# fuxiAIlab/RL4RS

Hardware: AMD Instinct MI355X
Metric: env-steps/s (batch=4096, 9-slot slate) (higher is better)
Workload: dtype f32 (scorer matrix operands as fp16 hi+lo pairs, three f16 MFMAs per product, fp32 accumulate)

## Files before the change

### include/rl4rs_hip.h

```cpp
#ifndef RL4RS_HIP_H
#define RL4RS_HIP_H

#include <stdint.h>

#ifdef __cplusplus
extern "C" {
#endif

#define RL4RS_ABI_VERSION 1

enum {
    RL4RS_OK = 0,
    RL4RS_EINVAL = -1,
    RL4RS_EHIP = -2,
    RL4RS_ESTATE = -3,
    RL4RS_ENOMEM = -4
};

const char* rl4rs_last_error(void);
int rl4rs_abi_version(void);
int rl4rs_device_count(void);

int rl4rs_copy_d2d(void* dst_dev, const void* src_dev, int64_t n_bytes, void* stream);

// ... 182 lines not shown
int rl4rs_dien_head_prob(rl4rs_dien* net, int32_t R, const float* obs_dev, float* prob_dev, void* stream);

enum {
    RL4RS_DIEN_ALL_FEATURE = 0,
    RL4RS_DIEN_SCORES = 1,
    RL4RS_DIEN_QUERY = 2,
    RL4RS_DIEN_H1 = 3,
    RL4RS_DIEN_N_ACTIVE = 4,
    RL4RS_DIEN_ROW_REP = 5,
    RL4RS_DIEN_ROW_ACTIVE = 6,
    RL4RS_DIEN_H1_FRAG = 7,
    RL4RS_DIEN_LEAD = 8
};
int rl4rs_dien_buffer(rl4rs_dien* net, int which, void** dev_ptr, int64_t* n_bytes);

int rl4rs_dien_set_row_order(rl4rs_dien* net, const int32_t* order_dev, int32_t n_groups);

int rl4rs_dien_set_profiling(rl4rs_dien* net, int enable);
int rl4rs_dien_kernel_count(void);
const char* rl4rs_dien_kernel_name(int which);
int rl4rs_dien_kernel_label(rl4rs_dien* net, int which, char* buf, int32_t cap);
int rl4rs_dien_profile_read(rl4rs_dien* net, int which, double* ms_total, int64_t* launches);
int rl4rs_dien_profile_reset(rl4rs_dien* net);

typedef struct rl4rs_simnet rl4rs_simnet;
enum { RL4RS_SIMNET_DNN = 1, RL4RS_SIMNET_WIDEDEEP = 2, RL4RS_SIMNET_LSTM = 3,
       RL4RS_SIMNET_ADVERSARIAL = 4  };

typedef struct rl4rs_simnet_cfg {
    int32_t algo;
    int32_t maxlen;
    int32_t emb_size;
    int32_t hidden_units;
    int32_t dense_feature_num;
    int32_t category_feature_num;
    int32_t category_hash_size;
    int32_t seq_num;
    int32_t class_num;
    int32_t max_rows;
    int32_t max_slots;
} rl4rs_simnet_cfg;

typedef struct rl4rs_simnet_weights {
    const float* cat_emb;
    const float* seq_emb;
    const float* dense_w1; const float* dense_b1;
    const float* dense_w2; const float* dense_b2;
    const float* fc_w; const float* fc_b;
    const float* obs_w; const float* obs_b;
    const float* out_w; const float* out_b;
    const float* cat_gru_kernel; const float* cat_gru_recurrent; const float* cat_gru_bias;
    const float* seq_gru_kernel[4]; const float* seq_gru_recurrent[4]; const float* seq_gru_bias[4];
} rl4rs_simnet_weights;

int rl4rs_simnet_create(const rl4rs_simnet_cfg* cfg, const rl4rs_simnet_weights* w, void* stream,
                        rl4rs_simnet** out);
int rl4rs_simnet_destroy(rl4rs_simnet* net);
int rl4rs_simnet_obs_dim(rl4rs_simnet* net, int32_t* dim);
int rl4rs_simnet_encode(rl4rs_simnet* net, int32_t s, const int32_t* ids_dev, int32_t n, int32_t slot_base,
                        void* stream);
int rl4rs_simnet_forward(rl4rs_simnet* net, int32_t R, int32_t group, const float* dense_dev,
                         const int32_t* cat_dev, const int32_t* slot_dev, float* obs_dev, float* prob_dev,
                         void* stream);
int rl4rs_simnet_head_prob(rl4rs_simnet* net, int32_t R, const float* obs_dev, float* prob_dev, void* stream);

typedef struct rl4rs_stepper rl4rs_stepper;
int rl4rs_env_attach_scorer(rl4rs_env* env, rl4rs_dien* net, const int32_t* slots_dev, int32_t seq_num,
                            rl4rs_stepper** out);
int rl4rs_env_attach_simnet(rl4rs_env* env, rl4rs_simnet* net, const int32_t* slots_dev, int32_t seq_num,
                            rl4rs_stepper** out);
int rl4rs_stepper_destroy(rl4rs_stepper* s);
int rl4rs_env_step_discrete(rl4rs_stepper* s, const int32_t* actions_dev, float* obs_dev, double* reward_dev,
                            uint8_t* done_dev, uint32_t* mask_bits_dev, void* stream);
int rl4rs_stepper_set_act_tail(rl4rs_stepper* s, int32_t on);
int rl4rs_stepper_set_obs_fold(rl4rs_stepper* s, int32_t on);
int rl4rs_stepper_set_distinct_hint(rl4rs_stepper* s, int32_t n_distinct);
int rl4rs_stepper_set_partition_carry(rl4rs_stepper* s, int32_t on);
int rl4rs_stepper_set_step_overlap(rl4rs_stepper* s, int32_t on);
int rl4rs_stepper_lane_stats(const rl4rs_stepper* s, int64_t* lane0, int64_t* lane1, int64_t* joins);
int rl4rs_stepper_observe(rl4rs_stepper* s, float* obs_dev, int32_t* taken, void* stream);
int rl4rs_stepper_set_reset_lane(rl4rs_stepper* s, int32_t on);
int rl4rs_stepper_set_reward_lane(rl4rs_stepper* s, int32_t on);
int rl4rs_stepper_lane_stats_ex(const rl4rs_stepper* s, int64_t* reset_runs, int64_t* reward_runs);
int rl4rs_stepper_click_probs(rl4rs_stepper* s, float* out_dev, void* stream);
int rl4rs_stepper_reward_rows(const rl4rs_stepper* s);
int rl4rs_stepper_next_offline_action(rl4rs_stepper* s, const int32_t** ids_dev, int32_t* step);
int rl4rs_env_step_conti(rl4rs_stepper* s, const void* actions_dev, int is_f64, int32_t* chosen_dev, float* obs_dev,
                         double* reward_dev, uint8_t* done_dev, uint32_t* mask_bits_dev, void* stream);

enum {
    RL4RS_STEP_WANT_MASK_I64 = 1, RL4RS_STEP_WANT_MASK_BITS = 2, RL4RS_STEP_WANT_D3RL_OBS = 4, RL4RS_STEP_WANT_CLICK_P = 8,
    RL4RS_STEP_WANT_OFFLINE_ACTION = 16, RL4RS_STEP_WANT_ALL = 31
};
typedef struct rl4rs_step_record {
    int64_t status, reward, done, chosen, obs, obs_d3rl, mask_i64, mask_bits, click_p, offline_action;
    int64_t host_bytes, total_bytes;
    int32_t obs_dim, d3rl_cols;
} rl4rs_step_record;
int rl4rs_stepper_record_layout(rl4rs_stepper* s, uint32_t want, int32_t conti, rl4rs_step_record* out);
int rl4rs_env_step_record(rl4rs_stepper* s, const void* actions_dev, int32_t action_kind, uint32_t want, void* record_dev,
                          void* stream);
int rl4rs_env_step_record_host(rl4rs_stepper* s, const void* actions_dev, int32_t action_kind, uint32_t want, void* record_dev,
                               void* record_host, void* stream);
int rl4rs_env_observe_record_host(rl4rs_stepper* s, int32_t conti, uint32_t want, void* record_dev, void* record_host,
                                  void* stream);
int rl4rs_set_host_mirror(int32_t on);

typedef struct rl4rs_policy rl4rs_policy;

int rl4rs_policy_param_count(int32_t obs_dim, int32_t hidden, int32_t action_size);
int rl4rs_policy_create(int32_t obs_dim, int32_t hidden, int32_t action_size, int32_t max_rows,
                        const float* params_host, void* stream, rl4rs_policy** out);
int rl4rs_policy_destroy(rl4rs_policy* pol);
int rl4rs_policy_params(rl4rs_policy* pol, float** params_dev, int32_t* count);

int rl4rs_policy_act(rl4rs_policy* pol, int32_t N, const float* obs_dev, const uint32_t* mask_bits_dev,
                     uint32_t seed, uint32_t step, int32_t* actions_dev, float* logp_dev, float* value_dev,
                     float* entropy_dev, float* logits_dev, void* stream);
int rl4rs_policy_evaluate(rl4rs_policy* pol, int32_t N, const float* obs_dev, const uint32_t* mask_bits_dev,
                          const int32_t* actions_dev, float* logp_dev, float* value_dev, float* entropy_dev,
                          float* logits_dev, void* stream);

int rl4rs_policy_loss_grad(rl4rs_policy* pol, int32_t algo, int32_t N, const float* obs_dev,
                           const uint32_t* mask_bits_dev, const int32_t* actions_dev, const float* adv_dev,
                           const float* ret_dev, const float* old_logp_dev, const float* old_value_dev,
                           const float* old_logits_dev, float vf_coeff, float ent_coeff, float clip,
                           float vf_clip, float kl_coeff, float* grad_dev, float* stats_dev, void* stream);
int rl4rs_policy_adam_step(rl4rs_policy* pol, const float* grad_dev, float lr, float beta1, float beta2,
                           float eps, float grad_clip, void* stream);
int rl4rs_policy_ppo_epoch(rl4rs_policy* pol, int32_t N, int32_t minibatch, const float* obs_dev,
                           const uint32_t* mask_bits_dev, const int32_t* actions_dev, const float* adv_dev,
                           const float* ret_dev, const float* old_logp_dev, const float* old_value_dev,
                           const float* old_logits_dev, float vf_coeff, float ent_coeff, float clip, float vf_clip,
                           float kl_coeff, float lr, float beta1, float beta2, float eps, float grad_clip,
                           float* grad_dev, float* stats_dev, void* stream);
int rl4rs_policy_ppo_minibatch_grad(rl4rs_policy* pol, int32_t N, int32_t minibatch, int32_t mb_index,
                                    const float* obs_dev, const uint32_t* mask_bits_dev, const int32_t* actions_dev,
                                    const float* adv_dev, const float* ret_dev, const float* old_logp_dev,
                                    const float* old_value_dev, const float* old_logits_dev, float vf_coeff,
                                    float ent_coeff, float clip, float vf_clip, float kl_coeff, float* grad_dev,
                                    float* stats_dev, void* stream);
enum { RL4RS_POLICY_STATUS_PASS_TIMEOUT = 1 };
int rl4rs_policy_status(rl4rs_policy* pol, int32_t* flags, void* stream);
int rl4rs_policy_status_words(rl4rs_policy* pol, uint32_t** words_dev);
enum { RL4RS_POLICY_OPT_TILE = 0, RL4RS_POLICY_OPT_PPO_FUSED = 1, RL4RS_POLICY_OPT_PPO_ROWS = 2, RL4RS_POLICY_OPT_RESIDENT_WGS = 3,
       RL4RS_POLICY_OPT_PPO_STD = 4 };
int rl4rs_policy_set_option(rl4rs_policy* pol, int32_t which, int32_t value);
int rl4rs_policy_adam_state(rl4rs_policy* pol, float** m_dev, float** v_dev, int64_t* step);
int rl4rs_policy_set_adam_step(rl4rs_policy* pol, int64_t step);

typedef struct rl4rs_replay rl4rs_replay;

int rl4rs_replay_create(int32_t obs_dim, int32_t action_size, int32_t max_steps, int32_t batch_size, int64_t buffer_size,
                        double alpha, rl4rs_replay** out);
int rl4rs_replay_destroy(rl4rs_replay* h);
int rl4rs_replay_rows(rl4rs_replay* h, int32_t* rows, int32_t* capacity_rows, int64_t* pushes);
enum { RL4RS_REPLAY_BUF_OBS = 0, RL4RS_REPLAY_BUF_MASK = 1, RL4RS_REPLAY_BUF_ACTION = 2, RL4RS_REPLAY_BUF_REWARD = 3,
       RL4RS_REPLAY_BUF_DONE = 4, RL4RS_REPLAY_BUF_PRIORITY = 5, RL4RS_REPLAY_BUF_MAX_PRIORITY = 6,
       RL4RS_REPLAY_BUF_ACTION_F32 = 7  };
int rl4rs_replay_buffer(rl4rs_replay* h, int32_t which, void** dev_out, int64_t* count_out);
int rl4rs_replay_push(rl4rs_replay* h, const float* obs_dev, const uint32_t* mask_bits_dev, const int32_t* action_dev,
                      const double* reward_dev, void* stream);
int rl4rs_replay_sample(rl4rs_replay* h, int32_t M, int32_t prioritized, double beta, uint32_t seed, uint32_t step,
                        float* obs_out, float* next_obs_out, uint32_t* next_mask_out, int32_t* action_out, float* reward_out,
                        int32_t* done_out, int32_t* idx_out, float* weight_out, float* u_out, void* stream);
int rl4rs_replay_update_priorities(rl4rs_replay* h, int32_t M, const int32_t* idx_dev, const float* td_dev, void* stream);
// ... 508 lines not shown
```

### rl4rs_amd/_lib.py

```python
import ctypes as C
import os

_HERE = os.path.dirname(os.path.abspath(__file__))
LIB_PATH = os.path.join(_HERE, 'csrc', 'librl4rs_hip.so')

OK = 0


class Rl4rsHipError(RuntimeError):
    pass


class EnvCfg(C.Structure):
    _fields_ = [(n, C.c_int32) for n in (
        'batch_size', 'max_steps', 'action_size', 'action_emb_size', 'page_items', 'item_dim',
        'user_dense_dim', 'user_cat_dim', 'maxlen', 'dense_feature_num', 'category_feature_num',
        'log_steps', 'is_seq', 'violation_zeroes_reward')]


class DienCfg(C.Structure):
    _fields_ = [(n, C.c_int32) for n in (
        'maxlen', 'emb_size', 'hidden_units', 'dense_feature_num', 'category_feature_num',
        'category_hash_size', 'seq_num', 'class_num', 'max_rows', 'max_slots', 'scorer_mode')] + [('kernel_opts', C.c_uint32)]

# ... 179 lines not shown
    'rl4rs_dien_kernel_count': (_I, []),
    'rl4rs_dien_kernel_name': (C.c_char_p, [_I]),
    'rl4rs_dien_kernel_label': (_I, [_P, _I, C.c_char_p, _I32]),
    'rl4rs_dien_profile_read': (_I, [_P, _I, C.POINTER(C.c_double), C.POINTER(_I64)]),
    'rl4rs_dien_profile_reset': (_I, [_P]),
    'rl4rs_policy_param_count': (_I, [_I32, _I32, _I32]),
    'rl4rs_policy_create': (_I, [_I32, _I32, _I32, _I32, _P, _P, C.POINTER(_P)]),
    'rl4rs_policy_destroy': (_I, [_P]),
    'rl4rs_policy_params': (_I, [_P, C.POINTER(_P), C.POINTER(_I32)]),
    'rl4rs_policy_act': (_I, [_P, _I32, _P, _P, C.c_uint32, C.c_uint32, _P, _P, _P, _P, _P, _P]),
    'rl4rs_policy_evaluate': (_I, [_P, _I32, _P, _P, _P, _P, _P, _P, _P, _P]),
    'rl4rs_policy_loss_grad': (_I, [_P, _I32, _I32, _P, _P, _P, _P, _P, _P, _P, _P, C.c_float, C.c_float, C.c_float,
                                    C.c_float, C.c_float, _P, _P, _P]),
    'rl4rs_policy_adam_step': (_I, [_P, _P, C.c_float, C.c_float, C.c_float, C.c_float, C.c_float, _P]),
    'rl4rs_simtrain_create': (_I, [C.POINTER(SimnetCfg), C.POINTER(SimnetWeights), _I32, _P, C.POINTER(_P)]),
    'rl4rs_simtrain_create_head': (_I, [C.POINTER(SimnetCfg), C.POINTER(SimnetWeights), _I32, _I32, _P, C.POINTER(_P)]),
    'rl4rs_simtrain_adam_state': (_I, [_P, C.POINTER(_P), C.POINTER(_P), C.POINTER(_I64)]),
    'rl4rs_simtrain_eval': (_I, [_P, _I32, _P, _P, C.POINTER(_P), _P, _P, _P, _P]),
    'rl4rs_simtrain_destroy': (_I, [_P]),
    'rl4rs_simtrain_params': (_I, [_P, C.POINTER(_P), C.POINTER(_P), C.POINTER(_I64)]),
    'rl4rs_simtrain_masks': (_I, [_P, C.POINTER(_P), C.POINTER(_P)]),
    'rl4rs_simtrain_grad': (_I, [_P, _I32, _P, _P, C.POINTER(_P), _P, C.c_float, C.c_uint32, C.c_uint32, _P, _P]),
    'rl4rs_simtrain_step': (_I, [_P, _I32, _P, _P, C.POINTER(_P), _P, C.c_float, C.c_float, C.c_float, C.c_float, C.c_float,
                                 C.c_uint32, C.c_uint32, _P, _P]),
    'rl4rs_recur_train_set_rows': (_I, [_I32]),
    'rl4rs_dientrain_create': (_I, [C.POINTER(DienCfg), C.POINTER(DienWeights), _I32, _P, C.POINTER(_P)]),
    'rl4rs_dientrain_create_head': (_I, [C.POINTER(DienCfg), C.POINTER(DienWeights), _I32, _I32, _P, C.POINTER(_P)]),
    'rl4rs_dientrain_adam_state': (_I, [_P, C.POINTER(_P), C.POINTER(_P), C.POINTER(_I64)]),
    'rl4rs_dientrain_eval': (_I, [_P, _I32, _P, _P, C.POINTER(_P), _P, _P, _P, _P]),
    'rl4rs_dientrain_destroy': (_I, [_P]),
    'rl4rs_clfmetrics_create': (_I, [_I32, _FP, _P, C.POINTER(_P)]),
    'rl4rs_clfmetrics_destroy': (_I, [_P]),
    'rl4rs_clfmetrics_reset': (_I, [_P, _P]),
    'rl4rs_clfmetrics_update_binary': (_I, [_P, _I64, _P, _P, _P]),
    'rl4rs_clfmetrics_update_multiclass': (_I, [_P, _I64, _I32, _P, _P, _P]),
    'rl4rs_clfmetrics_read': (_I, [_P, C.POINTER(_I64), _P]),
    'rl4rs_dientrain_set_fork': (_I, [_I32]),
    'rl4rs_dientrain_params': (_I, [_P, C.POINTER(_P), C.POINTER(_P), C.POINTER(_I64)]),
    'rl4rs_dientrain_masks': (_I, [_P, C.POINTER(_P), C.POINTER(_P)]),
    'rl4rs_dientrain_grad': (_I, [_P, _I32, _P, _P, C.POINTER(_P), _P, C.c_float, C.c_uint32, C.c_uint32, _P, _P]),
    'rl4rs_dientrain_step': (_I, [_P, _I32, _P, _P, C.POINTER(_P), _P, C.c_float, C.c_float, C.c_float, C.c_float, C.c_float,
                                  C.c_uint32, C.c_uint32, _P, _P]),
    'rl4rs_rawpolicy_create': (_I, [C.POINTER(RawPolicyCfg), C.POINTER(RawPolicyWeights), _P, C.POINTER(_P)]),
    'rl4rs_rawpolicy_destroy': (_I, [_P]),
    'rl4rs_rawpolicy_act': (_I, [_P, _I32, _P, _P, C.POINTER(_P), _P, C.c_uint32, C.c_uint32, _P, _P, _P, _P, _P, _P]),
    'rl4rs_rawpolicy_evaluate': (_I, [_P, _I32, _P, _P, C.POINTER(_P), _P, _P, _P, _P, _P, _P, _P]),
    'rl4rs_rawtrain_create': (_I, [C.POINTER(RawPolicyCfg), C.POINTER(RawPolicyWeights), _P, C.POINTER(_P)]),
    'rl4rs_rawtrain_destroy': (_I, [_P]),
    'rl4rs_rawtrain_params': (_I, [_P, C.POINTER(_P), C.POINTER(_P), C.POINTER(_I64)]),
    'rl4rs_rawtrain_act': (_I, [_P, _I32, _P, _P, C.POINTER(_P), _P, C.c_uint32, C.c_uint32, _P, _P, _P, _P, _P, _P]),
    'rl4rs_rawtrain_evaluate': (_I, [_P, _I32, _P, _P, C.POINTER(_P), _P, _P, _P, _P, _P, _P, _P]),
    'rl4rs_rawtrain_loss_grad': (_I, [_P, _I32, _I32, _P, _P, C.POINTER(_P), _P, _P, _P, _P, _P, _P, _P, C.c_float, C.c_float,
                                      C.c_float, C.c_float, C.c_float, _P, _P]),
    'rl4rs_rawtrain_adam_step': (_I, [_P, C.c_float, C.c_float, C.c_float, C.c_float, C.c_float, _P]),
    'rl4rs_policy_ppo_epoch': (_I, [_P, _I32, _I32, _P, _P, _P, _P, _P, _P, _P, _P] + [C.c_float] * 10 + [_P, _P, _P]),
    'rl4rs_dien_set_row_order': (_I, [_P, _P, _I32]),
    'rl4rs_dien_set_obs_last': (_I, [_P, _P]),
    'rl4rs_dien_set_row_partition': (_I, [_P, _P, _P, _P, _I32]),
    'rl4rs_dien_dedup_counts': (_I, [_P, C.POINTER(_I64), C.POINTER(_I64)]),
    'rl4rs_dien_set_augru_rows': (_I, [_P, _I32]),
    'rl4rs_dien_set_distinct_hint': (_I, [_P, _I32]),
    'rl4rs_dien_status_word': (_I, [_P, C.POINTER(_P)]),
    'rl4rs_stepper_record_layout': (_I, [_P, C.c_uint32, _I32, C.POINTER(StepRecord)]),
    'rl4rs_env_step_record': (_I, [_P, _P, _I32, C.c_uint32, _P, _P]),
    'rl4rs_env_step_record_host': (_I, [_P, _P, _I32, C.c_uint32, _P, _P, _P]),
    'rl4rs_env_observe_record_host': (_I, [_P, _I32, C.c_uint32, _P, _P, _P]),
    'rl4rs_set_host_mirror': (_I, [_I32]),
    'rl4rs_env_set_option': (_I, [_P, _I32, _I32]),
    'rl4rs_policy_set_option': (_I, [_P, _I32, _I32]),
    'rl4rs_env_get_cfg': (_I, [_P, _P]),
    'rl4rs_env_attach_scorer': (_I, [_P, _P, _P, _I32, _P]),
    'rl4rs_env_attach_simnet': (_I, [_P, _P, _P, _I32, _P]),
    'rl4rs_stepper_destroy': (_I, [_P]),
    'rl4rs_stepper_set_act_tail': (_I, [_P, _I32]),
    'rl4rs_stepper_set_obs_fold': (_I, [_P, _I32]),
    'rl4rs_stepper_set_partition_carry': (_I, [_P, _I32]),
    'rl4rs_stepper_set_distinct_hint': (_I, [_P, _I32]),
    'rl4rs_stepper_set_step_overlap': (_I, [_P, _I32]),
    'rl4rs_stepper_lane_stats': (_I, [_P, _P, _P, _P]),
    'rl4rs_stepper_observe': (_I, [_P, _P, _P, _P]),
    'rl4rs_stepper_set_reset_lane': (_I, [_P, _I32]),
    'rl4rs_stepper_set_reward_lane': (_I, [_P, _I32]),
    'rl4rs_stepper_lane_stats_ex': (_I, [_P, _P, _P]),
    'rl4rs_stepper_click_probs': (_I, [_P, _P, _P]),
    'rl4rs_stepper_reward_rows': (_I, [_P]),
    'rl4rs_stepper_next_offline_action': (_I, [_P, _P, _P]),
    'rl4rs_env_step_discrete': (_I, [_P, _P, _P, _P, _P, _P, _P]),
    'rl4rs_env_step_conti': (_I, [_P, _P, _I, _P, _P, _P, _P, _P, _P]),
    'rl4rs_policy_ppo_minibatch_grad': (_I, [_P, _I32, _I32, _I32, _P, _P, _P, _P, _P, _P, _P, _P] + [C.c_float] * 5 + [_P, _P, _P]),
    'rl4rs_policy_status': (_I, [_P, _P, _P]),
    'rl4rs_policy_status_words': (_I, [_P, _P]),
    'rl4rs_policy_adam_state': (_I, [_P, _P, _P, _P]),
    'rl4rs_policy_set_adam_step': (_I, [_P, C.c_int64]),
    'rl4rs_qnet_create': (_I, [_P, _FP, _P, _P, _P, _P]),
    'rl4rs_qnet_destroy': (_I, [_P]),
    'rl4rs_qnet_params': (_I, [_P, _P, _P, _P]),
    'rl4rs_qnet_copy_params': (_I, [_P, _P, _P]),
    'rl4rs_qnet_adam_state': (_I, [_P, _P, _P, _P]),
    'rl4rs_qnet_set_adam_step': (_I, [_P, _I64]),
    'rl4rs_qnet_status': (_I, [_P, C.POINTER(_I32), _P]),
    'rl4rs_qnet_forward': (_I, [_P, _I32, _P, _P, _P]),
    'rl4rs_qnet_backward': (_I, [_P, _I32, _P, _P, _P]),
    'rl4rs_qnet_adam_step': (_I, [_P, C.c_float, C.c_float, C.c_float, C.c_float, _P]),
    'rl4rs_q_best_action': (_I, [_I32, _I32, _P, _P, C.c_float, _P, _P]),
    'rl4rs_qloss_imitation': (_I, [_P, _I32, _P, _P, C.c_float, _P, _P, _P, _P]),
    'rl4rs_qloss_dqn': (_I, [_P, _I32, _P, _P, _P, _P, _P, _P, _P, C.c_float, C.c_float, C.c_float, _P, _P, _P, _P, _P]),
    'rl4rs_amlp_create': (_I, [_P, _FP, _P, _P]),
    'rl4rs_amlp_destroy': (_I, [_P]),
    'rl4rs_amlp_params': (_I, [_P, _P, _P, _P]),
    'rl4rs_amlp_copy_params': (_I, [_P, _P, _P]),
    'rl4rs_amlp_adam_state': (_I, [_P, _P, _P, _P]),
    'rl4rs_amlp_set_adam_step': (_I, [_P, _I64]),
    'rl4rs_amlp_soft_update': (_I, [_P, _P, C.c_float, _P]),
    'rl4rs_amlp_forward': (_I, [_P, _I32, _I32, _P, _P, _P, _P]),
    'rl4rs_amlp_h16_ok': (_I, [_P]),
    'rl4rs_pack_h16_selftest': (_I, [_P, _I64, _I32, _I32, _P, _P]),
    'rl4rs_amlp_forward_h16': (_I, [_P, _I32, _I32, _P, _P, _P, _P]),
    'rl4rs_amlp_backward': (_I, [_P, _I32, _I32, _P, _P, _P, _P, _I32, _P]),
    'rl4rs_amlp_adam_step': (_I, [_P, C.c_float, C.c_float, C.c_float, C.c_float, _P]),
    'rl4rs_amlp_adam_multi': (_I, [_I32, C.POINTER(_P), C.POINTER(C.c_float), C.POINTER(_I32), C.POINTER(_P), C.c_float, C.c_float, C.c_float,
                                   C.c_float, _P]),
    'rl4rs_amlp_set_fused': (_I, [_I32]),
    'rl4rs_cql_workspace_floats': (_I64, [_I32, _I32, _I32]),
    'rl4rs_cql_update': (_I, [C.POINTER(CqlStep), _P]),
    'rl4rs_bcq_workspace_floats': (_I64, [_I32, _I32, _I32, _I32]),
    'rl4rs_amlp_grad_stash': (_I, [_I32, _P, _P, _I32, _P]),
    'rl4rs_combo_critic_loss': (_I, [_I32, _I32, _I32, _P, _P, _P, _P, _P, _P, _P, _P, _P, _P, _P, _P, _P, _P]),
    'rl4rs_combo_workspace_floats': (_I64, [_I32, _I32, _I32, _I32]),
    'rl4rs_combo_workspace_offset': (_I64, [_I32, _I32, _I32, _I32, _I32]),
    'rl4rs_combo_update': (_I, [C.POINTER(ComboStep), _P]),
    'rl4rs_bcq_update': (_I, [C.POINTER(BcqStep), _P]),
    'rl4rs_amlp_forward_multi': (_I, [_I32, C.POINTER(_P), _I32, _P, _P, C.POINTER(_P), _P]),
    'rl4rs_amlp_backward_multi': (_I, [_I32, C.POINTER(_P), _I32, _P, _P, C.POINTER(_P), C.POINTER(_P), _I32, _P]),
    'rl4rs_cvae_sample': (_I, [_I32, _I32, _P, _P, C.c_float, C.c_float, _P, _P]),
    'rl4rs_cvae_loss': (_I, [_I32, _I32, _I32, _P, _P, _P, C.c_float, C.c_float, _P, _P, _P, _P]),
    'rl4rs_cvae_encoder_grad': (_I, [_I32, _I32, _P, _P, _P, C.c_float, C.c_float, C.c_float, _P, _P]),
    'rl4rs_residual_action': (_I, [_I32, _I32, _P, _P, C.c_float, _P, _P]),
    'rl4rs_residual_grad': (_I, [_I32, _I32, _P, _P, C.c_float, _P, _P, _P]),
    'rl4rs_bcq_target': (_I, [_I32, _I32, _P, _P, C.c_float, _P, _P, C.c_float, _P, _P, _P]),
    'rl4rs_pick_rows': (_I, [_I32, _I32, _I32, _P, _P, _P, _P]),
    'rl4rs_critic_mse': (_I, [_I32, _P, _P, _P, _P, _P, _P, _P]),
    'rl4rs_squashed_sample': (_I, [_I32, _I32, _I32, _P, _P, C.c_float, C.c_float, _I32, _I32, _P, _P, _P]),
    'rl4rs_sac_actor_grad': (_I, [_I32, _I32, _P, _P, _P, _P, _P, C.c_float, C.c_float, _P, _P]),
    'rl4rs_twin_min': (_I, [_I32, _P, _P, _P, _P, _P, _P]),
    'rl4rs_cql_critic_loss': (_I, [_I32, _I32, _P, _P, _P, _P, _P, _P, _P, _P, _P, _P]),
    'rl4rs_gemm_f32_packed': (_I, [_P, _I64, _P, _I64, _P, _P, _I64, _I32, _I32, _I32, _I, _P]),
    'rl4rs_gemm_h16_packed': (_I, [_P, _I64, _P, _I64, _P, _P, _I64, _I32, _I32, _I32, _I, _P]),
    'rl4rs_gemm_f32': (_I, [_P, _I64, _P, _I64, _P, _P, _I64, _I32, _I32, _I32, _I, _P]),
    'rl4rs_student_t_ppf': (C.c_double, [C.c_double, C.c_double]),
    'rl4rs_ope_create': (_I, [_I32, _I32, C.POINTER(_P)]),
    'rl4rs_ope_destroy': (_I, [_P]),
    'rl4rs_ope_begin': (_I, [_P, _I32, _I32]),
    'rl4rs_ope_record_policy': (_I, [_P, _I32, _P, _I32, _I64, _P, _I32, _P]),
    'rl4rs_ope_record_behavior': (_I, [_P, _I32, _P, _I32, _I64, _I32, _I32, _P, _I32, _P]),
    'rl4rs_ope_record_column': (_I, [_P, _I32, _I32, _P, _I32, _P]),
    'rl4rs_ope_record_q': (_I, [_P, _I32, _P, _I32, _I64, _P, _P]),
    'rl4rs_ope_log': (_I, [_P, _I32, C.POINTER(_P), C.POINTER(_I64)]),
    'rl4rs_ope_mark_recorded': (_I, [_P, _I32, _I32]),
    'rl4rs_ope_estimate': (_I, [_P, C.c_double, C.POINTER(C.c_double), _P]),
    'rl4rs_ope_episode_stats': (_I, [_I32, _P, _P, _P, _P, _P, C.POINTER(C.c_double), _P]),
    'rl4rs_ope_step_stats': (_I, [_I32, _I32, _P, _P, _P, _P, _P, C.c_double, C.POINTER(C.c_double), _P]),
    'rl4rs_replay_create': (_I, [_I32, _I32, _I32, _I32, _I64, C.c_double, C.POINTER(_P)]),
    'rl4rs_replay_destroy': (_I, [_P]),
    'rl4rs_replay_rows': (_I, [_P, C.POINTER(_I32), C.POINTER(_I32), C.POINTER(_I64)]),
    'rl4rs_replay_buffer': (_I, [_P, _I32, C.POINTER(_P), C.POINTER(_I64)]),
    'rl4rs_replay_push': (_I, [_P, _P, _P, _P, _P, _P]),
# ... 136 lines not shown
```

### rl4rs_amd/csrc/common.hpp

```cpp
#pragma once
#include <hip/hip_runtime.h>
#include <cmath>
#include <cstdarg>
#include <cstdint>
#include <cstdio>
#include <cstring>
#include <string>
#include <vector>

#include "../../include/rl4rs_hip.h"
#include "step_lanes.hpp"

namespace rl4rs {

void set_error(const char* fmt, ...);

#define RL4RS_HIP_TRY(expr)                                                              \
    do {                                                                                 \
        hipError_t _e = (expr);                                                          \
        if (_e != hipSuccess) {                                                          \
            ::rl4rs::set_error("%s failed: %s (%s:%d)", #expr, hipGetErrorString(_e),    \
                               __FILE__, __LINE__);                                      \
            return RL4RS_EHIP;                                                           \
        }                                                                                \
// ... 29 lines not shown
    uint32_t h = mix32(seed ^ mix32(step * 0x9E3779B9U + 0x85EBCA6BU) ^ mix32(row * 0xC2B2AE35U + a * 0x27D4EB2FU + 1U));
    h = mix32(h + a);
    return ((float)(h >> 9) + 0.5f) * (1.0f / 8388608.0f);
}
__device__ __forceinline__ float normal01(uint32_t seed, uint32_t step, uint32_t row, uint32_t col) {
    const float u1 = uniform01(seed, step, row, 2u * col);
    const float u2 = uniform01(seed, step, row, 2u * col + 1u);
    return sqrtf(-2.f * logf(u1)) * cosf(6.28318530717958647692f * u2);
}

inline int ceil_div(int a, int b) { return (a + b - 1) / b; }

enum { ACT_NONE = 0, ACT_ELU = 1, ACT_SIGMOID = 2, ACT_TANH = 3, ACT_RELU = 4 };

int launch_gemm_f32(const float* a, int64_t lda, const float* w, int64_t ldw, const float* bias,
                    float* c, int64_t ldc, int M, int N, int K, int act, hipStream_t st, const float* addend = nullptr,
                    int64_t ldadd = 0, int add_div = 1);

int launch_gemm_small(const float* a, int64_t lda, const float* w, int64_t ldw, int K, const float* a2, int64_t lda2, const float* w2,
                      int64_t ldw2, int K2, const float* bias, float* c, int64_t ldc, int M, int N, int act, hipStream_t st,
                      const float* addend = nullptr, int64_t ldadd = 0, int add_div = 1);
int launch_gemm_nt(const float* dy, int64_t ldy, const float* w, int64_t ldw, float* dx, int64_t ldx, int M, int Kin, int Nout,
                   hipStream_t st, const float* relu_of = nullptr, int64_t ldr = 0);

int launch_gemm_tn(const float* A, int lda, int M, const float* B, int ldb, int Nc, int Ns, int chunk, float* part, float* part_b,
                   float* dW, float* db, hipStream_t st);

int launch_gemm_packed(const float* a, int64_t lda, const float* wp, const float* bias, float* c, int64_t ldc,
                       int M, int N, int K, int act, hipStream_t st, const float* addend = nullptr, int64_t ldadd = 0);
std::vector<float> pack_gemm_weight(const float* w, int64_t ldw, int K, int N);
struct G16RowMap { const int32_t* active; const int32_t* n_active; int group; };
int launch_gemm_h16(const float* a, int64_t lda, const float* wp16, const float* bias, float* c, int64_t ldc,
                    int M, int N, int K, int act, hipStream_t st, const float* addend = nullptr, int64_t ldadd = 0,
                    float* mirror = nullptr, int64_t ldm = 0, const G16RowMap* map = nullptr);
int launch_gemm_h16_gather(const float* a, int64_t lda, const float* wp16, float* c, int64_t ldc, int M, int N, int K, int act,
                           hipStream_t st, const float* addend, int64_t ldadd, const int32_t* rep);
std::vector<float> pack_gemm_weight_h16(const float* w, int64_t ldw, int K, int N);
int launch_gemm_h16_chain(const float* a, int64_t lda, const float* wp1, const float* bias1, int N1, int K1, int act1,
                          const float* wp2, const float* bias2, float* c2, int64_t ldc2, int N2, int act2, int M, hipStream_t st,
                          const G16RowMap* map = nullptr);
struct GemmH16Desc {
    const float* a; int64_t lda; const float* wp; const float* bias; float* c; int64_t ldc; int M, N, K, act;
    const float* addend; int64_t ldadd;
    const float* wp2; const float* bias2; float* c2; int64_t ldc2; int N2, act2;
};
int launch_gemm_h16_pair(const GemmH16Desc& x, const GemmH16Desc& y, hipStream_t st, const G16RowMap* map = nullptr);

struct PackH16Desc { const float* w; float* out; int ldw, K, N; };
struct PackH16Args { PackH16Desc d[4]; };
int launch_pack_h16_dev(const PackH16Desc* d, int n, hipStream_t st);
struct AmlpFwdH16 {
    const float* act; const float* proj; const char* w1p; const char* w2p; const char* w3p;
    const float* b2; const float* b3; float* out;
    int N, E, rep, K3, head_act;
};
int launch_amlp_fwd_h16(const AmlpFwdH16& a, hipStream_t st);

int raise_dyn_smem(const void* fn, size_t bytes);
int current_device();

struct ActTail {
    uint8_t* done; uint8_t done_v;
    double* zero_reward;
    int32_t* next_action; int next_cur;
};
struct RowRefineArgs;
int env_act_discrete_tail(rl4rs_env* e, const int32_t* actions, const ActTail& tail, void* stream, const RowRefineArgs* rf = nullptr);
int env_act_conti_refine(rl4rs_env* e, const void* actions, int is_f64, int32_t* chosen, void* stream, const RowRefineArgs* rf);
bool env_refine_fits(const rl4rs_env* e);
uint64_t next_stamp();
uint64_t env_rows_stamp(const rl4rs_env* e);
struct DienPartition {
    uint64_t stamp;
    int n_groups, group;
    const float* dense; const int32_t* cat; const int32_t* slots; const int32_t* order;
    const int32_t* rep; const int32_t* active; const int32_t* n_active;
};
void dien_last_partition(const rl4rs_dien* n, DienPartition* out);
bool dien_takes_partition(const rl4rs_dien* n);
const int32_t* dien_row_order(const rl4rs_dien* n, int n_groups);

void dien_set_obs_mirror(rl4rs_dien* n, float* host_visible);
bool dien_obs_mirror_used(const rl4rs_dien* n);
void dien_drop_pending_expand(rl4rs_dien* n);
int64_t dien_augru_rounds(const rl4rs_dien* n, int B, int live, int group);
bool dien_augru_rows64(const rl4rs_dien* n, int B, int group);

const LaneHook** env_lane_slot(rl4rs_env* e);
const LaneHook** dien_lane_slot(rl4rs_dien* n);
void env_flip_rows(rl4rs_env* e);
void env_rows_current(const rl4rs_env* e, const float** dense, const int32_t** cat);
int dien_reserve_lane_scratch(rl4rs_dien* n, int rows);
int dien_forward_lane(rl4rs_dien* n, int set, int32_t R, const float* dense, const int32_t* cat, const int32_t* slots, float* obs,
                      void* stream, void* home);
int dien_forward_lane_full(rl4rs_dien* n, int set, int32_t R, int32_t group, const float* dense, const int32_t* cat, const int32_t* slots,
                           float* obs, float* prob, void* stream, void* home, void* after_dedup, void* before_augru);
int env_build_complete_rows_lane(rl4rs_env* e, int32_t rows_per_env, void* stream);
int env_reward_split_lane(rl4rs_env* e, const float* probs, const float* p_last, double* reward, void* stream);
bool dien_lane_path(const rl4rs_dien* n, int rows);
int dien_n_cu(const rl4rs_dien* n);

struct RecurTrainFwd {
    int N, L, S, Hd;
    const int32_t* iota;
    const float* a1[4];
    const float* wg[4]; const float* wc[4];
    const float* att[4];
    float *R[4], *U[4], *C[4], *H[4], *RH[4];
    int hard;
    int xblk[3];
};
struct RecurTrainBwd {
    int N, L, S, Hd;
    const float *R[4], *U[4], *C[4], *H[4];
    const float* att[4];
    const float* up_last[4]; int64_t ld_up;
    const float* up_all[4];
    const float* wcT[4]; const float* wgT[4];
    float *dr[4], *du[4], *dc[4];
    int64_t ld_g, ld_c;
    float* d_score[4];
    int hard;
};
int launch_recur_train_fwd(const RecurTrainFwd& f, hipStream_t st);
int launch_recur_train_bwd(const RecurTrainBwd& b, hipStream_t st);
int launch_pack_frag(const float* w, int64_t ld, int k_off, int K, int N, int transpose, float* out, hipStream_t st);
int launch_pack_frag_slice(const float* w, int64_t ld, int k_off, int K, int N, int transpose, float* out, int K_total, int k_dst,
                           hipStream_t st);

inline float pow2_prescale(float maxabs) {
    if (!(maxabs > 0.f) || !(maxabs < 3.0e38f)) return 1.f;
    int e = 0;
    (void)frexpf(maxabs, &e);
    int k = 14 - e;
#ifndef RL4RS_PRESCALE_UP
    if (e <= 14 && e > -6) k = 0;
#endif
    if (k > 100) k = 100;
    if (k < -100) k = -100;
    return ldexpf(1.f, k);
}

inline uint16_t f32_to_f16(float f) {
    uint32_t x;
    memcpy(&x, &f, 4);
    const uint32_t sign = (x >> 16) & 0x8000u;
    x &= 0x7fffffffu;
    if (x >= 0x7f800000u) return (uint16_t)(sign | 0x7c00u | (x > 0x7f800000u ? 0x200u : 0));
    if (x >= 0x477ff000u) return (uint16_t)(sign | 0x7c00u);
    if (x < 0x38800000u) {
        if (x < 0x33000000u) return (uint16_t)sign;
        const int e = (int)(x >> 23);
        uint32_t m = (x & 0x7fffffu) | 0x800000u;
        const int shift = 126 - e;
        uint32_t r = m >> shift;
        const uint32_t rem = m & ((1u << shift) - 1), halfway = 1u << (shift - 1);
        if (rem > halfway || (rem == halfway && (r & 1))) ++r;
        return (uint16_t)(sign | r);
    }
    uint32_t r = ((x - 0x38000000u) >> 13);
    const uint32_t rem = x & 0x1fffu;
    if (rem > 0x1000u || (rem == 0x1000u && (r & 1))) ++r;
    return (uint16_t)(sign | r);
}
inline float f16_to_f32(uint16_t h) {
    const uint32_t sign = (uint32_t)(h & 0x8000u) << 16;
    uint32_t e = (h >> 10) & 0x1f, m = h & 0x3ffu, x;
    if (e == 0) {
        if (m == 0) x = sign;
        else { int s = 0; while (!(m & 0x400u)) { m <<= 1; ++s; } m &= 0x3ffu; x = sign | ((uint32_t)(113 - s) << 23) | (m << 13); }
    } else if (e == 31) x = sign | 0x7f800000u | (m << 13);
    else x = sign | ((e + 112) << 23) | (m << 13);
    float f;
    memcpy(&f, &x, 4);
    return f;
}

}
```

### rl4rs_amd/csrc/dien.hip

```cpp
#include <cstdlib>
#include <vector>

#include "common.hpp"
#include "recur_args.hpp"
#include "cat_attn2_row.hpp"
#include "dien_plan.hpp"
#include "augru_xs.hpp"

namespace rl4rs {


__device__ __forceinline__ float sigmoidf_(float x) { return 1.f / (1.f + expf(-x)); }
__device__ __forceinline__ float eluf_(float x) { return x > 0.f ? x : expm1f(x); }



#ifndef RL4RS_AUGRU_U
#define RL4RS_AUGRU_U 2
#endif
constexpr int AUGRU_U = RL4RS_AUGRU_U, GRU_U = 2;
#ifndef RL4RS_H16_NLDS
#define RL4RS_H16_NLDS 5
#endif
#ifndef RL4RS_H16_NRES
// ... 1354 lines not shown
        int id = min(max(crowp[j], 0), H - 1);
        const float4 v = reinterpret_cast<const float4*>(ptab + ((size_t)j * H + id) * OBS_DIM)[lane];
        acc.x += v.x; acc.y += v.y; acc.z += v.z; acc.w += v.w;
    }
    acc.x = eluf_(acc.x); acc.y = eluf_(acc.y); acc.z = eluf_(acc.z); acc.w = eluf_(acc.w);
    *o = acc;
}

}

using namespace rl4rs;

namespace {
enum { KID_CAT = 0, KID_DENSE, KID_DIN, KID_AUGRU, KID_HEAD, KID_PROB, KID_GRU1, KID_PROJ, KID_DEDUP, KID_COUNT };
const char* kKernelNames[KID_COUNT] = {"k_cat_attn", "k_gemm_f32(dense tower)", "k_din_scores",
                                       "augru", "k_gemm_f32(simulator_obs)", "k_head_prob",
                                       "k_recur<128,gru>", "k_gemm_f32(seq projections)", "k_row_dedup"};
struct EvPair { int id; hipEvent_t a, b; };
}

static size_t augru_h16_smem(int mt, int nh2, int L) {
    return (size_t)4 * mt * 32 * (nh2 + 8) * 2 + (size_t)(mt * 32 * (L + 1) + mt * 32) * 4 + (size_t)8 * RL4RS_H16_NLDS * 2048;
}

struct rl4rs_dien {
    rl4rs_dien_cfg c;
    DienTraits t;
    int n_cu;
    int E, U, L, S, Cn, Dn, H, K, F, PLD, NH2;
    int Fld;
    float *cat_emb, *seq_emb, *dense_w1, *dense_b1, *dense_w2, *dense_b2, *obs_w, *obs_b, *out_w, *out_b;
    float* ptab;
    float* embw1[4];
    float* gru_wg[4];
    float* gru_wc[4];
    float* wproj[4];
    float* bproj[4];
    float* w1ac[4];
    float* w1ac_all;
    float* qa;
    float* w1d[4];
    float* w1d16[4];
    float *att_w2[4], *att_b2[4], *att_w3[4], *att_b3[4];
    float* augru_wg16[4];
    float* augru_wc16[4];
    float* gru_wg16[4];
    float* gru_pad[4];
    int32_t* lead[4];
    float* gru_wc16[4];
    bool gru16, gru16_attr;
    bool gru_roles;
    int augru_rows;
    float augru_s[4][3][8];
    float* tsum;
    hipStream_t side_stream; hipEvent_t ev_fork, ev_join;
    int* range_flag;
    const int32_t* row_order; int row_order_n;
    DienPlan last_plan;
    int distinct_hint;
    int32_t *dd_dstart, *dd_dlist, *dd_dcur;
    int32_t* dd_rep;
    int32_t* dd_active;
    int32_t* dd_nact;
    const int32_t* part_rep; const int32_t* part_active; const int32_t* part_nact; int part_groups;
    const int32_t* last_rep; const int32_t* last_active; const int32_t* last_nact; int last_groups;
    DienPartition dd_info;
    int64_t dedup_launched, dedup_carried;
    struct LazyExpand { bool pending; hipStream_t st; int R, group, n_groups, ncol; const int32_t* rep; const int32_t* nact; int set; } lazy;
    float* augru_wg[4];
    float* augru_wc[4];
    float* h1[4];
    float* h1f[4];
    float* proj[4];
    float *allf, *dh, *q, *scores, *obs_tmp;
    int srows;
    struct ScratchSet { float *allf, *dh, *q, *scores, *qa, *tsum; int rows; } alt;
    int last_set;
    int last_rows;
    hipStream_t last_home;
    const LaneHook* lanes;
    float* obs_mirror;
    bool obs_mirror_used;
    float* obs_last;
    std::vector<void*> owned;
    int profiling;
    std::vector<EvPair> pending;
    std::vector<hipEvent_t> pool;
    double ms_total[KID_COUNT];
    long launches[KID_COUNT];
};

namespace {

int upload(rl4rs_dien* n, float** dst, const float* src, size_t count, hipStream_t st) {
    int rc = dev_alloc(dst, count);
    if (rc) return rc;
    n->owned.push_back(*dst);
    RL4RS_HIP_TRY(hipMemcpyAsync(*dst, src, count * 4, hipMemcpyHostToDevice, st));
    return RL4RS_OK;
}
int alloc_f(rl4rs_dien* n, float** dst, size_t count) {
    int rc = dev_alloc(dst, count);
    if (rc) return rc;
    n->owned.push_back(*dst);
    return RL4RS_OK;
}

int launch_gru16(rl4rs_dien* n, const RecurArgs& a, hipStream_t st) {
    const size_t smem_v1 = (((size_t)4 * 32 * (128 + 8) * 2 + (size_t)32 * (a.L + 1) * 4 + 15) & ~(size_t)15) + (size_t)4 * 8 * 2048;
    const size_t smem = n->gru_roles ? gru_h16r_smem(a.L) : smem_v1;
    const void* fn = n->gru_roles ? reinterpret_cast<const void*>(&k_gru_h16r) : reinterpret_cast<const void*>(&k_gru_h16);
    if (!n->gru16_attr) {
        const int rc = raise_dyn_smem(fn, smem);
        if (rc) return rc;
        n->gru16_attr = true;
    }
    if (n->gru_roles) hipLaunchKernelGGL(k_gru_h16r, dim3((a.n_rows + 31) / 32, 1), dim3(512), smem, st, a);
    else hipLaunchKernelGGL(k_gru_h16, dim3((a.n_rows + 31) / 32, 1), dim3(256), smem, st, a);
    return RL4RS_OK;
}

std::vector<float> pack_frag(const float* w, int ld, int k_off, int K, int N) {
    const int KB = K / 8, NT = N / 32;
    std::vector<float> out((size_t)K * N);
    for (int nt = 0; nt < NT; ++nt)
        for (int kb = 0; kb < KB; ++kb)
            for (int lane = 0; lane < 64; ++lane)
                for (int i = 0; i < 4; ++i) {
                    int k = kb * 8 + (lane >> 5) * 4 + i;
                    int j = nt * 32 + (lane & 31);
                    out[(((size_t)nt * KB + kb) * 64 + lane) * 4 + i] = w[(size_t)(k_off + k) * ld + j];
                }
    return out;
}

std::vector<float> pack_frag_h16(const float* w, int ld, int k_off, int K, int N) {
    const int KB = K / 16, NT = N / 32;
    std::vector<uint16_t> out((size_t)NT * KB * 2 * 64 * 8);
    for (int nt = 0; nt < NT; ++nt)
        for (int kb = 0; kb < KB; ++kb)
            for (int lane = 0; lane < 64; ++lane)
                for (int i = 0; i < 8; ++i) {
                    const float v = w[(size_t)(k_off + kb * 16 + (lane >> 5) * 8 + i) * ld + nt * 32 + (lane & 31)];
                    const uint16_t hi = f32_to_f16(v);
                    const uint16_t lo = f32_to_f16(v - f16_to_f32(hi));
                    const size_t base = (((size_t)nt * KB + kb) * 2) * 512 + (size_t)lane * 8 + i;
                    out[base] = hi;
                    out[base + 512] = lo;
                }
    std::vector<float> f(out.size() / 2);
    memcpy(f.data(), out.data(), out.size() * 2);
    return f;
}

static int scorer_gemm(rl4rs_dien* n, const float* a, int64_t lda, const float* wp, const float* bias, float* c, int64_t ldc,
                       int M, int N, int K, int act, hipStream_t st) {
    return n->t.gemm16 ? launch_gemm_h16(a, lda, wp, bias, c, ldc, M, N, K, act, st)
                     : launch_gemm_packed(a, lda, wp, bias, c, ldc, M, N, K, act, st);
}

struct Prof {
    rl4rs_dien* n; int id; hipStream_t st; hipEvent_t a, b; bool on;
    Prof(rl4rs_dien* n_, int id_, hipStream_t st_) : n(n_), id(id_), st(st_), on(n_->profiling == 1 || (n_->profiling == 2 && id_ == KID_AUGRU)) {
        if (!on) return;
        auto get = [&]() {
            hipEvent_t e;
// ... 684 lines not shown
            augru_xs_launch(S, f.st, a, sh);
            break;
        }
        case PlanAugru::X32: augru_x_launch(32, S, f.st, a); break;
        case PlanAugru::X64: augru_x_launch(64, S, f.st, a); break;
        default: hipLaunchKernelGGL((k_augru_h16<1, RL4RS_H16_RING1, RL4RS_H16_NRES>), grid, block, augru_h16_smem(1, NH2, L), f.st, a); break;
    }
    RL4RS_LAUNCH_CHECK();
    return RL4RS_OK;
}

static int stage_expand(rl4rs_dien* n, const DienPlan& p, const DienFwd& f) {
    Prof pr(n, KID_DEDUP, f.st);
    if (p.expand == PlanExpand::Lazy) {
        n->lazy = rl4rs_dien::LazyExpand{true, f.home, f.R, f.group, f.n_groups, p.expand_ncol, f.rep, f.nact, f.set};
        return RL4RS_OK;
    }
    RowExpandArgs a;
    memset(&a, 0, sizeof(a));
    a.R = f.R; a.group = f.group; a.n_groups = f.n_groups; a.S = n->S; a.L = n->L; a.ncol = p.expand_ncol;
    a.rep = f.rep; a.n_active = f.nact;
    a.allf = n->allf; a.ld = n->Fld; a.scores = n->scores; a.scores_stride = (int64_t)n->srows * n->L;
    if (p.expand == PlanExpand::Behind) { a.q = n->q; a.E = n->E; a.obs = f.obs_out; a.obs_dim = OBS_DIM; }
    hipLaunchKernelGGL(k_row_expand, dim3((f.R + 3) / 4), dim3(256), 0, f.st, a);
    RL4RS_LAUNCH_CHECK();
    return RL4RS_OK;
}

static int stage_head(rl4rs_dien* n, const DienPlan& p, const DienFwd& f) {
    Prof pr(n, KID_HEAD, f.st);
    const int F = n->Fld, R = f.R, Kh = n->S * n->NH2 + n->U + n->E;
    int rc;
    switch (p.head) {
        case PlanHead::TsumH16:
        case PlanHead::TsumH16Mirror: {
            if (p.expand == PlanExpand::Lazy && f.group == 1)
                return launch_gemm_h16_gather(n->allf, F, n->obs_w, f.obs_out, OBS_DIM, R, OBS_DIM, Kh, 1, f.st, n->tsum, OBS_DIM, f.rep);
            float* const mirror = p.head == PlanHead::TsumH16Mirror ? n->obs_mirror : nullptr;
            rc = launch_gemm_h16(n->allf, F, n->obs_w, nullptr, f.obs_out, OBS_DIM, R, OBS_DIM, Kh, 1, f.st, n->tsum, OBS_DIM, mirror, OBS_DIM, f.map2);
            n->obs_mirror_used = mirror != nullptr;
            return rc;
        }
        case PlanHead::TsumPacked:
            return launch_gemm_packed(n->allf, F, n->obs_w, nullptr, f.obs_out, OBS_DIM, R, OBS_DIM, Kh, 1, f.st, n->tsum, OBS_DIM);
        case PlanHead::TablesFinish:
            if ((rc = scorer_gemm(n, n->allf, F, n->obs_w, nullptr, f.obs_out, OBS_DIM, R, OBS_DIM, Kh, 0, f.st))) return rc;
            hipLaunchKernelGGL(k_head_finish, dim3((R + 3) / 4), dim3(256), 0, f.st, f.obs_out, R, f.cat, n->Cn, n->H, n->ptab, n->obs_b);
            RL4RS_LAUNCH_CHECK();
            return RL4RS_OK;
        case PlanHead::Plain: break;
    }
    return scorer_gemm(n, n->allf, F, n->obs_w, n->obs_b, f.obs_out, OBS_DIM, R, OBS_DIM, n->F, 1, f.st);
}

static int stage_prob(rl4rs_dien* n, const DienPlan& p, const DienFwd& f) {
    Prof pr(n, KID_PROB, f.st);
    if (p.expand == PlanExpand::Lazy && f.group > 1)
        hipLaunchKernelGGL(k_head_prob_rep, dim3((f.R + 3) / 4), dim3(256), 0, f.st, f.obs_out, f.R, OBS_DIM, n->K, n->out_w, n->out_b, f.prob, f.group,
                           n->obs_last, f.rep);
    else
        hipLaunchKernelGGL(k_head_prob, dim3((f.R + 3) / 4), dim3(256), 0, f.st, f.obs_out, f.R, OBS_DIM, n->K, n->out_w, n->out_b, f.prob, f.group, n->obs_last);
    RL4RS_LAUNCH_CHECK();
    return RL4RS_OK;
}

static void swap_scratch(rl4rs_dien* n) {
    rl4rs_dien::ScratchSet& a = n->alt;
    std::swap(n->allf, a.allf); std::swap(n->dh, a.dh); std::swap(n->q, a.q); std::swap(n->scores, a.scores);
    std::swap(n->qa, a.qa); std::swap(n->tsum, a.tsum); std::swap(n->srows, a.rows);
}

static int dien_forward_on(rl4rs_dien* n, int set, hipStream_t home, int32_t R, int32_t group, const float* dense, const int32_t* cat,
                           const int32_t* slots, float* obs, float* prob, void* stream, hipEvent_t after_dedup = nullptr,
                           hipEvent_t before_augru = nullptr) {
    RL4RS_REQUIRE(n && dense && cat && slots, "dien_forward: null argument");
    RL4RS_REQUIRE(R > 0 && R <= n->c.max_rows, "dien_forward: R=%d exceeds max_rows=%d", R, n->c.max_rows);
    RL4RS_REQUIRE(group >= 1 && R % group == 0, "dien_forward: R=%d is not a multiple of group=%d", R, group);
    const int ngroups = R / group;
    n->obs_mirror_used = false;
    n->lazy.pending = false;
    struct SetGuard { rl4rs_dien* n; bool on; ~SetGuard() { if (on) swap_scratch(n); } } set_guard{n, set == 1};
    if (set == 1) swap_scratch(n);
    n->last_set = set; n->last_rows = R; n->last_home = home;
    struct MirrorOnce { rl4rs_dien* n; ~MirrorOnce() { n->obs_mirror = nullptr; n->obs_last = nullptr; n->part_rep = nullptr; } } mirror_once{n};
    DienCall c{};
    c.R = R; c.group = group; c.obs = obs != nullptr; c.prob = prob != nullptr;
    c.mirror = n->obs_mirror != nullptr; c.obs_last = n->obs_last != nullptr;
    c.carried = n->part_rep != nullptr; c.part_groups = n->part_groups;
    c.row_order = n->row_order && n->row_order_n == ngroups;
    c.augru_rows = n->augru_rows; c.distinct_hint = n->distinct_hint;
    c.dense_vec = (n->Dn & 3) == 0 && (reinterpret_cast<uintptr_t>(dense) & 15) == 0;
    RL4RS_REQUIRE(!c.carried || (dien_takes_partition(n) && c.part_groups == ngroups),
                  "dien_forward: the row partition set for this forward is for %d groups with the row dedup on (forward: %d groups)", n->part_groups, ngroups);
    RL4RS_REQUIRE(!c.obs_last || c.prob, "dien_forward: rl4rs_dien_set_obs_last needs a forward that returns probabilities");
    const DienPlan p = dien_plan(n->t, c);
    DienFwd f;
    f.R = R; f.group = group; f.n_groups = ngroups; f.dense = dense; f.cat = cat; f.slots = slots;
    f.obs_out = obs ? obs : n->obs_tmp; f.prob = prob; f.st = (hipStream_t)stream;
    f.set = set; f.home = home;
    f.order_in = c.row_order ? n->row_order : nullptr;
    f.rep = c.carried ? n->part_rep : n->dd_rep;
    f.active = c.carried ? n->part_active : n->dd_active;
    f.nact = c.carried ? n->part_nact : n->dd_nact;
    f.rmap = G16RowMap{f.active, f.nact, group};
    f.map2 = p.tier2 ? &f.rmap : nullptr;
    int rc;
    if (p.dense_side && (rc = stage_dense_fork(n, p, f))) return rc;
    if ((rc = stage_dedup(n, p, f))) return rc;
    if (after_dedup) RL4RS_HIP_TRY(hipEventRecord(after_dedup, f.st));
    n->last_plan = p;
    if ((rc = stage_cat(n, p, f))) return rc;
    if ((rc = stage_dense(n, p, f))) return rc;
    if ((rc = stage_din(n, p, f))) return rc;
    if (before_augru) RL4RS_HIP_TRY(hipStreamWaitEvent(f.st, before_augru, 0));
    if ((rc = stage_augru(n, p, f))) return rc;
    if (p.expand == PlanExpand::Front && (rc = stage_expand(n, p, f))) return rc;
    if (p.dense_side) RL4RS_HIP_TRY(hipStreamWaitEvent(f.st, n->ev_join, 0));
    if ((rc = stage_head(n, p, f))) return rc;
    if ((p.expand == PlanExpand::Behind || p.expand == PlanExpand::Lazy) && (rc = stage_expand(n, p, f))) return rc;
    if (p.prob && (rc = stage_prob(n, p, f))) return rc;
    return RL4RS_OK;
}

int rl4rs_dien_forward(rl4rs_dien* n, int32_t R, int32_t group, const float* dense, const int32_t* cat,
                       const int32_t* slots, float* obs, float* prob, void* stream) {
    RL4RS_REQUIRE(n, "dien_forward: null argument");
    const int rc = lanes_join(n->lanes, stream);
    if (rc) return rc;
    return dien_forward_on(n, 0, (hipStream_t)stream, R, group, dense, cat, slots, obs, prob, stream);
}

int rl4rs_dien_head_prob(rl4rs_dien* n, int32_t R, const float* obs, float* prob, void* stream) {
    RL4RS_REQUIRE(n && obs && prob && R > 0, "dien_head_prob: bad argument");
    hipStream_t st = (hipStream_t)stream;
    Prof p(n, KID_PROB, st);
    hipLaunchKernelGGL(k_head_prob, dim3((R + 3) / 4), dim3(256), 0, st, obs, R, OBS_DIM, n->K, n->out_w, n->out_b, prob, 1, nullptr);
    RL4RS_LAUNCH_CHECK();
    return RL4RS_OK;
}

static int dien_settle_set(rl4rs_dien* n) {
    if (n->last_set != 1) return RL4RS_OK;
    n->last_set = 0;
    const rl4rs_dien::ScratchSet& a = n->alt;
    const size_t R = (size_t)n->last_rows;
    hipStream_t st = n->last_home;
    RL4RS_HIP_TRY(hipMemcpyAsync(n->allf, a.allf, R * n->Fld * 4, hipMemcpyDeviceToDevice, st));
    RL4RS_HIP_TRY(hipMemcpyAsync(n->q, a.q, R * n->E * 4, hipMemcpyDeviceToDevice, st));
    for (int s = 0; s < n->S; ++s)
        RL4RS_HIP_TRY(hipMemcpyAsync(n->scores + (size_t)s * n->srows * n->L, a.scores + (size_t)s * a.rows * n->L, R * n->L * 4,
                                     hipMemcpyDeviceToDevice, st));
    return RL4RS_OK;
}

static int dien_settle_expand(rl4rs_dien* n) {
    if (!n->lazy.pending) return RL4RS_OK;
    n->lazy.pending = false;
    const rl4rs_dien::LazyExpand& z = n->lazy;
    struct SetGuard { rl4rs_dien* n; bool on; ~SetGuard() { if (on) swap_scratch(n); } } set_guard{n, z.set == 1};
    if (z.set == 1) swap_scratch(n);
    RowExpandArgs a;
    memset(&a, 0, sizeof(a));
    a.R = z.R; a.group = z.group; a.n_groups = z.n_groups; a.S = n->S; a.L = n->L; a.ncol = z.ncol;
    a.rep = z.rep; a.n_active = z.nact;
    a.allf = n->allf; a.ld = n->Fld; a.scores = n->scores; a.scores_stride = (int64_t)n->srows * n->L;
    a.q = n->q; a.E = n->E;
    hipLaunchKernelGGL(k_row_expand, dim3((z.R + 3) / 4), dim3(256), 0, z.st, a);
    RL4RS_LAUNCH_CHECK();
    return RL4RS_OK;
}

int rl4rs_dien_buffer(rl4rs_dien* n, int which, void** p, int64_t* bytes) {
    RL4RS_REQUIRE(n && p, "dien_buffer: null argument");
    {
        const int rc = lanes_join(n->lanes, nullptr, false);
        if (rc) return rc;
    }
    if (which == RL4RS_DIEN_ALL_FEATURE || which == RL4RS_DIEN_SCORES || which == RL4RS_DIEN_QUERY) {
        int rc = dien_settle_expand(n);
        if (rc) return rc;
        if ((rc = dien_settle_set(n))) return rc;
// ... 10 lines not shown
            ptr = n->h1f[0]; b = ((int64_t)n->c.max_slots + 1) * ((n->L + 31) / 32) * 32 * n->E * 4; break;
        case RL4RS_DIEN_LEAD:
            if (!n->lead[0]) { set_error("dien_buffer: this handle keeps no pad table (no lead[])"); return RL4RS_EINVAL; }
            ptr = n->lead[0]; b = ((int64_t)n->c.max_slots + 1) * 4; break;
        case RL4RS_DIEN_N_ACTIVE:
        case RL4RS_DIEN_ROW_REP:
        case RL4RS_DIEN_ROW_ACTIVE: {
            if (!n->t.row_dedup) { set_error("dien_buffer: row dedup is off on this handle"); return RL4RS_EINVAL; }
            const int64_t groups = n->last_rep ? n->last_groups : n->c.max_rows;
            if (which == RL4RS_DIEN_N_ACTIVE) { ptr = const_cast<int32_t*>(n->last_rep ? n->last_nact : n->dd_nact); b = 4; }
            else if (which == RL4RS_DIEN_ROW_REP) { ptr = const_cast<int32_t*>(n->last_rep ? n->last_rep : n->dd_rep); b = groups * 4; }
            else { ptr = const_cast<int32_t*>(n->last_rep ? n->last_active : n->dd_active); b = groups * 4; }
            break;
        }
        default: set_error("dien_buffer: unknown buffer id %d", which); return RL4RS_EINVAL;
    }
    *p = ptr;
    if (bytes) *bytes = b;
    return RL4RS_OK;
}

int rl4rs_dien_set_row_order(rl4rs_dien* n, const int32_t* order_dev, int32_t n_groups) {
    RL4RS_REQUIRE(n && n_groups >= 0, "dien_set_row_order: bad argument");
    n->row_order = order_dev;
    n->row_order_n = order_dev ? n_groups : 0;
    return RL4RS_OK;
}

int rl4rs_dien_set_augru_rows(rl4rs_dien* n, int32_t rows) {
    RL4RS_REQUIRE(n && (rows == 0 || rows == 32 || rows == 64), "dien_set_augru_rows: rows must be 0, 32 or 64");
    n->augru_rows = rows;
    return RL4RS_OK;
}

int rl4rs_dien_set_distinct_hint(rl4rs_dien* n, int32_t n_groups) {
    RL4RS_REQUIRE(n && n_groups >= 0, "dien_set_distinct_hint: bad argument");
    n->distinct_hint = n_groups;
    return RL4RS_OK;
}

static_assert(rl4rs::ROW_REFINE_CAP == rl4rs::ROW_DEDUP_CAP, "the carried partition's search window is k_row_dedup's");
int rl4rs_dien_set_row_partition(rl4rs_dien* n, const int32_t* rep_dev, const int32_t* active_dev, const int32_t* n_active_dev, int32_t n_groups) {
    RL4RS_REQUIRE(n, "dien_set_row_partition: null handle");
    if (!rep_dev) { n->part_rep = nullptr; return RL4RS_OK; }
    RL4RS_REQUIRE(active_dev && n_active_dev && n_groups > 0 && n_groups <= n->c.max_rows, "dien_set_row_partition: bad argument");
    RL4RS_REQUIRE(n->t.row_dedup && !n->t.dup_store, "dien_set_row_partition: this handle's forward does not take a partition (row dedup off, or dup_store)");
    n->part_rep = rep_dev; n->part_active = active_dev; n->part_nact = n_active_dev; n->part_groups = n_groups;
    return RL4RS_OK;
}

int rl4rs_dien_set_obs_last(rl4rs_dien* n, float* obs_last_dev) {
    RL4RS_REQUIRE(n, "dien_set_obs_last: null handle");
    n->obs_last = obs_last_dev;
    return RL4RS_OK;
}

int rl4rs_dien_set_profiling(rl4rs_dien* n, int enable) {
    RL4RS_REQUIRE(n, "dien_set_profiling: null handle");
    n->profiling = enable == 2 ? 2 : (enable != 0 ? 1 : 0);
    return RL4RS_OK;
}
int rl4rs_dien_scorer_mode(rl4rs_dien* n, int32_t* mode) {
    RL4RS_REQUIRE(n && mode, "dien_scorer_mode: null argument");
    *mode = n->t.fp16x2 ? RL4RS_SCORER_FP16X2 : RL4RS_SCORER_FP32;
    return RL4RS_OK;
}
int rl4rs_dien_status(rl4rs_dien* n, int32_t* flags, void* stream) {
    RL4RS_REQUIRE(n && flags, "dien_status: null argument");
    hipStream_t st = (hipStream_t)stream;
    int v = 0;
    {
        const int rc = lanes_join(n->lanes, stream);
        if (rc) return rc;
    }
    RL4RS_HIP_TRY(hipMemcpyAsync(&v, n->range_flag, 4, hipMemcpyDeviceToHost, st));
    RL4RS_HIP_TRY(hipStreamSynchronize(st));
    if (v) RL4RS_HIP_TRY(hipMemsetAsync(n->range_flag, 0, 4, st));
    *flags = v ? RL4RS_DIEN_STATUS_FP16_RANGE : 0;
    return RL4RS_OK;
}
}
namespace rl4rs {
void dien_set_obs_mirror(rl4rs_dien* n, float* host_visible) { if (n) n->obs_mirror = host_visible; }
void dien_last_partition(const rl4rs_dien* n, DienPartition* out) { *out = n->dd_info; }
bool dien_takes_partition(const rl4rs_dien* n) { return n && n->t.row_dedup && !n->t.dup_store; }
const int32_t* dien_row_order(const rl4rs_dien* n, int n_groups) { return (n->row_order && n->row_order_n == n_groups) ? n->row_order : nullptr; }
bool dien_obs_mirror_used(const rl4rs_dien* n) { return n && n->obs_mirror_used; }
void dien_drop_pending_expand(rl4rs_dien* n) { if (n) n->lazy.pending = false; }
const LaneHook** dien_lane_slot(rl4rs_dien* n) { return &n->lanes; }
int dien_n_cu(const rl4rs_dien* n) { return n ? n->n_cu : 0; }
bool dien_lane_path(const rl4rs_dien* n, int rows) {
    return n && n->t.fp16x2 && n->t.augru_x && n->t.row_dedup && n->alt.allf && n->alt.rows >= rows;
}
int dien_reserve_lane_scratch(rl4rs_dien* n, int rows) {
    RL4RS_REQUIRE(n && rows > 0 && rows <= n->c.max_rows, "dien_reserve_lane_scratch: bad argument");
    if (n->alt.allf && n->alt.rows >= rows) return RL4RS_OK;
    rl4rs_dien::ScratchSet a;
    memset(&a, 0, sizeof(a));
    const int padded = (rows + 63) / 64 * 64 + 64;
    const size_t R = (size_t)padded;
    int rc;
    if ((rc = alloc_f(n, &a.allf, R * n->Fld)) || (rc = alloc_f(n, &a.dh, R * n->U)) || (rc = alloc_f(n, &a.q, R * n->E)) ||
        (rc = alloc_f(n, &a.qa, (size_t)n->S * R * ATT_H1)) || (rc = alloc_f(n, &a.scores, (size_t)n->S * R * n->L))) return rc;
    if (n->tsum && (rc = alloc_f(n, &a.tsum, R * OBS_DIM))) return rc;
    a.rows = padded;
    n->alt = a;
    return RL4RS_OK;
}
int dien_forward_lane(rl4rs_dien* n, int set, int32_t R, const float* dense, const int32_t* cat, const int32_t* slots, float* obs,
                      void* stream, void* home) {
    RL4RS_REQUIRE(n && (set == 0 || (set == 1 && n->alt.allf && R <= n->alt.rows)), "dien_forward_lane: no second scratch set of %d rows", R);
    return dien_forward_on(n, set, (hipStream_t)home, R, 1, dense, cat, slots, obs, nullptr, stream);
}
int dien_forward_lane_full(rl4rs_dien* n, int set, int32_t R, int32_t group, const float* dense, const int32_t* cat, const int32_t* slots,
                           float* obs, float* prob, void* stream, void* home, void* after_dedup, void* before_augru) {
    RL4RS_REQUIRE(n && (set == 0 || (set == 1 && n->alt.allf && R <= n->alt.rows)), "dien_forward_lane: no second scratch set of %d rows", R);
    return dien_forward_on(n, set, (hipStream_t)home, R, group, dense, cat, slots, obs, prob, stream, (hipEvent_t)after_dedup, (hipEvent_t)before_augru);
}
bool dien_augru_rows64(const rl4rs_dien* n, int B, int group) {
    return n && n->t.fp16x2 && n->t.augru_x && (int64_t)B * group <= n->c.max_rows && augru_rows64(n->augru_rows, B * group, group, n->S, n->n_cu);
}
int64_t dien_augru_rounds(const rl4rs_dien* n, int B, int live, int group) {
    if (!n || !n->t.fp16x2 || !n->t.augru_x || (int64_t)B * group > n->c.max_rows) return -1;
    const int64_t G = n->t.row_dedup ? (live < B ? live : B) : B;
    const int64_t tiles = augru_tiles(augru_rows64(n->augru_rows, B * group, group, n->S, n->n_cu), G * group, group);
    return (tiles * n->S + n->n_cu - 1) / n->n_cu;
}
}
extern "C" {
int rl4rs_dien_status_word(rl4rs_dien* n, int32_t** word_dev) {
    RL4RS_REQUIRE(n && word_dev, "dien_status_word: null argument");
    *word_dev = n->range_flag;
    return RL4RS_OK;
}
int rl4rs_dien_last_plan(rl4rs_dien* n, char* buf, int32_t cap) {
    RL4RS_REQUIRE(n && buf && cap > 0, "dien_last_plan: bad argument");
    buf[0] = 0;
    if (n->last_plan.din_waves) dien_plan_str(n->last_plan, buf, (size_t)cap);
    return RL4RS_OK;
}
int rl4rs_dien_kernel_count(void) { return KID_COUNT; }
int rl4rs_dien_kernel_label(rl4rs_dien* n, int which, char* buf, int32_t cap) {
    RL4RS_REQUIRE(n && buf && cap > 0 && which >= 0 && which < KID_COUNT, "dien_kernel_label: bad argument");
    const char* gemm = n->t.gemm16 ? "k_gemm_h16" : "k_gemm_pk";
    const DienTraits& t = n->t;
    std::string s;
    switch (which) {
        case KID_CAT: s = t.cat_v2_shape() ? (t.cat_group ? "k_cat_attn2 / k_cat_attn2g (grouped rows)" : "k_cat_attn2") : "k_cat_attn"; break;
        case KID_DENSE:
            s = t.dense_grouped() ? "k_gemm_h16_pair(dense tower, both layers + q-side term of the DIN scores)"
                : t.dense_chained() ? "k_gemm_h16<chain>(dense tower, both layers)" : std::string(gemm) + " x2 (dense tower)";
            break;
        case KID_DIN:
            s = std::string(t.din_x_selected() ? "k_din_x" : (t.din_h16() ? "k_din_scores<h16>" : "k_din_scores"));
            if (!t.dense_grouped()) s += std::string(" + ") + gemm + "(q-side term)";
            break;
        case KID_AUGRU:
            s = !t.fp16x2 ? "k_recur<256,augru>" : (t.augru_x ? "k_augru_x" : "k_augru_h16");
            if (n->last_plan.shadow) s = "k_augru_xs (last forward: category branch and dense tower in the shadow plane)";
            break;
        case KID_HEAD:
            s = std::string(gemm) + "(simulator_obs)" + ((n->ptab && !n->tsum) ? " + k_head_finish" : "");
            break;
        case KID_PROB: s = "k_head_prob"; break;
        case KID_GRU1:
            s = n->gru16 ? (n->gru_roles ? "k_gru_h16r" : "k_gru_h16") : "k_recur<128,gru>";
            if (n->h1f[0] && !(n->gru16 && n->gru_roles)) s += " + k_h1_frag";
            break;
        case KID_DEDUP: s = n->t.row_dedup ? "k_row_dedup + k_row_expand" : "k_row_dedup (off)"; break;
        case KID_PROJ: s = n->t.gemm16 ? "k_gemm_h16 / k_gemm_h16_wres(seq projections)" : "k_gemm_pk(seq projections)"; break;
    }
    snprintf(buf, (size_t)cap, "%s", s.c_str());
    return RL4RS_OK;
}
const char* rl4rs_dien_kernel_name(int which) {
    return (which >= 0 && which < KID_COUNT) ? kKernelNames[which] : "";
}
int rl4rs_dien_profile_read(rl4rs_dien* n, int which, double* ms_total, int64_t* launches) {
    RL4RS_REQUIRE(n && which >= 0 && which < KID_COUNT, "dien_profile_read: bad argument");
    {
        const int rc = lanes_join(n->lanes, nullptr, false);
        if (rc) return rc;
    }
    for (auto& e : n->pending) {
        RL4RS_HIP_TRY(hipEventSynchronize(e.b));
        float ms = 0.f;
        RL4RS_HIP_TRY(hipEventElapsedTime(&ms, e.a, e.b));
        n->ms_total[e.id] += ms;
        n->launches[e.id] += 1;
        n->pool.push_back(e.a);
        n->pool.push_back(e.b);
    }
    n->pending.clear();
    if (ms_total) *ms_total = n->ms_total[which];
    if (launches) *launches = n->launches[which];
    return RL4RS_OK;
}
int rl4rs_dien_profile_reset(rl4rs_dien* n) {
    RL4RS_REQUIRE(n, "dien_profile_reset: null handle");
    double d; int64_t l;
    int rc = rl4rs_dien_profile_read(n, 0, &d, &l);
    for (int i = 0; i < KID_COUNT; ++i) { n->ms_total[i] = 0; n->launches[i] = 0; }
    n->dedup_launched = n->dedup_carried = 0;
// ... 14 lines not shown
```

### rl4rs_amd/csrc/dien_plan.hpp

```cpp
#pragma once
#include <stdint.h>
#include <stdio.h>

namespace rl4rs {

inline int64_t augru_tiles(bool rows64, int64_t rows, int group) {
    if (!rows64) return (rows + 31) / 32;
    return group == 9 ? (rows / 9 + 6) / 7 : (rows + 63) / 64;
}
inline bool augru_rows64(int pin, int R, int group, int S, int n_cu) {
    if (pin == 32 || !(group == 9 || (group % 8 == 0 && R % 64 == 0))) return false;
    return pin == 64 || augru_tiles(true, R, group) * S >= 2 * (int64_t)n_cu;
}
inline bool augru_shadow_room(int hint, int n_groups, int S, int n_cu) {
    const int g = hint > 0 && hint < n_groups ? hint : n_groups;
    return augru_tiles(false, g, 1) * (S + 1) <= n_cu;
}
inline bool g16_shadow_fits(int R, int Dn, int F, int U) {
    return ((int64_t)R - 1) * Dn + Dn < ((int64_t)1 << 29) && ((int64_t)R - 1) * F + U < ((int64_t)1 << 29);
}
inline bool g16_gather_fits(int R, int F, int Kh) {
    return ((int64_t)R - 1) * F + Kh < ((int64_t)1 << 29) && (int64_t)R * 256 < ((int64_t)1 << 29);
}

struct DienTraits {
    bool fp16x2;
    bool gemm16;
    bool din16;
    bool cat16;
    bool augru_x;
    bool din_x;
    bool din_rows_auto;
    bool cat_v2;
    bool cat_group;
    bool dense_chain;
    bool gemm_group;
    bool dense_fork;
    bool row_dedup;
    bool dup_store;
    bool tier2_rows;
    bool augru_shadow;
    bool h1f;
    bool lazy_expand;
    bool ptab, tsum;
    int E, U, L, S, Cn, Dn, Fld, NH2, n_cu, max_rows;

    bool dense_chained() const { return gemm16 && dense_chain && U <= 128 && U % 16 == 0; }
    bool dense_grouped() const { return fp16x2 && dense_chained() && gemm_group && !dense_fork; }
    bool din_h16() const { return fp16x2 && din16; }
    bool din_x_selected() const { return din_h16() && h1f; }
    bool cat_v2_shape() const { return cat_v2 && E == 128 && Cn <= 24; }
    bool head_tsum() const { return ptab && tsum; }
};

struct DienCall {
    int R, group;
    bool obs, prob;
    bool mirror, obs_last;
    bool carried;
    int part_groups;
    bool row_order;
    int augru_rows;
    int distinct_hint;
    bool dense_vec;
};

enum class PlanDedup { None, Launch, Carried };
enum class PlanCat { Shadow, V1, V2_21, V2_24, G8, G9 };
enum class PlanDense { Shadow, Pair, Chain, TwoGemm };
enum class PlanQside { InPair, InDinXq, MappedH16, ScorerGemm };
enum class PlanDin { Xq, XAuto, X16, Scores };
enum class PlanAugru { Xs, X32, X64, H16, Recur32 };
enum class PlanExpand { None, Front, Behind, Lazy };
enum class PlanHead { TsumH16, TsumH16Mirror, TsumPacked, TablesFinish, Plain };

struct DienPlan {
    bool tier2;
    bool shadow;
    PlanDedup dedup;
    bool dup_lists;
    PlanCat cat;
    bool cat_h16;
    PlanDense dense;
    bool dense_side;
    bool dense_vec;
    PlanQside qside;
    PlanDin din;
    bool din_stage, din_h16; int din_waves;
    PlanAugru augru;
    PlanExpand expand; int expand_ncol;
    PlanHead head;
    bool prob;
};

inline DienPlan dien_plan(const DienTraits& t, const DienCall& c) {
    DienPlan p{};
    const int n_groups = c.R / c.group;
    const bool rows64 = augru_rows64(c.augru_rows, c.R, c.group, t.S, t.n_cu);
    p.dedup = !t.row_dedup ? PlanDedup::None : (c.carried ? PlanDedup::Carried : PlanDedup::Launch);
    p.dup_lists = t.dup_store;
    p.tier2 = t.row_dedup && t.tier2_rows && !t.dup_store && !t.dense_fork && !(c.obs && c.mirror) && t.gemm16 && t.head_tsum() &&
              t.cat_v2_shape() && t.dense_chained();
    p.shadow = p.tier2 && t.augru_shadow && c.group == 1 && t.Cn == 21 && t.S <= 2 && t.din_rows_auto && t.dense_grouped() && !rows64 &&
               c.augru_rows != 64 && augru_shadow_room(c.distinct_hint, n_groups, t.S, t.n_cu) && g16_shadow_fits(c.R, t.Dn, t.Fld, t.U);
    p.cat_h16 = t.fp16x2 && t.cat16;
    if (p.shadow) p.cat = PlanCat::Shadow;
    else if (t.cat_v2_shape() && t.cat_group && t.Cn >= 11 && (c.group == 8 || c.group == 9)) p.cat = c.group == 8 ? PlanCat::G8 : PlanCat::G9;
    else if (t.cat_v2_shape()) p.cat = t.Cn == 21 ? PlanCat::V2_21 : PlanCat::V2_24;
    else p.cat = PlanCat::V1;
    p.dense_side = t.dense_fork;
    p.dense_vec = c.dense_vec;
    if (p.shadow) p.dense = PlanDense::Shadow;
    else if (t.dense_grouped()) p.dense = PlanDense::Pair;
    else p.dense = t.dense_chained() ? PlanDense::Chain : PlanDense::TwoGemm;
    if (p.shadow) p.qside = PlanQside::InDinXq;
    else if (p.dense == PlanDense::Pair) p.qside = PlanQside::InPair;
    else p.qside = p.tier2 ? PlanQside::MappedH16 : PlanQside::ScorerGemm;
    p.din_h16 = t.din_h16();
    p.din_stage = c.group != 1;
    p.din_waves = c.group == 1 ? 4 : (c.group % 4 == 0 ? 4 : (c.group % 3 == 0 ? 3 : (c.group % 2 == 0 ? 2 : (c.group < 4 ? c.group : 4))));
    if (p.shadow) p.din = PlanDin::Xq;
    else if (t.din_x_selected()) p.din = (c.group == 1 && t.din_rows_auto) ? PlanDin::XAuto : PlanDin::X16;
    else p.din = PlanDin::Scores;
    if (!t.fp16x2) p.augru = PlanAugru::Recur32;
    else if (p.shadow) p.augru = PlanAugru::Xs;
    else if (t.augru_x) p.augru = rows64 ? PlanAugru::X64 : PlanAugru::X32;
    else p.augru = PlanAugru::H16;
    if (p.dedup == PlanDedup::None || t.dup_store) p.expand = PlanExpand::None;
    else p.expand = p.tier2 ? PlanExpand::Behind : PlanExpand::Front;
    p.expand_ncol = p.expand == PlanExpand::None ? 0 : (p.tier2 ? t.S * t.NH2 + t.U + t.E : t.S * t.NH2);
    if (p.expand == PlanExpand::Behind && t.lazy_expand &&
        (c.group == 1 ? g16_gather_fits(c.R, t.Fld, p.expand_ncol) : !c.obs))
        p.expand = PlanExpand::Lazy;
    if (t.head_tsum()) p.head = !t.gemm16 ? PlanHead::TsumPacked : ((c.obs && c.mirror) ? PlanHead::TsumH16Mirror : PlanHead::TsumH16);
    else p.head = t.ptab ? PlanHead::TablesFinish : PlanHead::Plain;
    p.prob = c.prob;
    return p;
}

inline int dien_plan_str(const DienPlan& p, char* buf, size_t cap) {
    static const char* const dd[] = {"none", "k_row_dedup", "carried"};
    static const char* const ct[] = {"shadow", "k_cat_attn", "k_cat_attn2<21,true>", "k_cat_attn2<24,false>", "k_cat_attn2g<8,8>", "k_cat_attn2g<9>"};
    static const char* const dn[] = {"shadow", "pair", "chain", "two_gemms"};
    static const char* const qs[] = {"in_pair", "in_k_din_xq", "mapped_k_gemm_h16", "scorer_gemm"};
    static const char* const di[] = {"k_din_xq", "k_din_x_auto", "k_din_x_16", "k_din_scores"};
    static const char* const au[] = {"k_augru_xs", "k_augru_x_32", "k_augru_x_64", "k_augru_h16", "k_recur_fp32"};
    static const char* const ex[] = {"none", "front", "behind", "lazy"};
    static const char* const hd[] = {"tsum+k_gemm_h16", "tsum+k_gemm_h16+mirror", "tsum+packed", "tables+k_head_finish", "plain"};
    char din[48];
    if (p.din == PlanDin::Scores) snprintf(din, sizeof(din), "k_din_scores<%d,%d>x%d", (int)p.din_stage, (int)p.din_h16, p.din_waves);
    else snprintf(din, sizeof(din), "%s", di[(int)p.din]);
    return snprintf(buf, cap, "tier2=%d shadow=%d dedup=%s%s cat=%s dense=%s%s qside=%s din=%s augru=%s expand=%s:%d head=%s prob=%d",
                    (int)p.tier2, (int)p.shadow, dd[(int)p.dedup], p.dup_lists ? "+dup_lists" : "", ct[(int)p.cat], dn[(int)p.dense],
                    p.dense_side ? "@side" : "", qs[(int)p.qside], din, au[(int)p.augru], ex[(int)p.expand], p.expand_ncol,
                    hd[(int)p.head], (int)p.prob);
}

}
```

### rl4rs_amd/csrc/env.hip

```cpp
#include <atomic>
#include <cstdlib>
#include <mutex>

#include "common.hpp"
#include "row_refine.hpp"

namespace rl4rs {

static thread_local std::string g_err;
void set_error(const char* fmt, ...) {
    char buf[1024];
    va_list ap;
    va_start(ap, fmt);
    vsnprintf(buf, sizeof(buf), fmt, ap);
    va_end(ap);
    g_err = buf;
}

struct EnvDev {
    int B, T, A, W, E, P, D, UD, UC, L, Dn, Cn, logT, is_seq;
    const float* item_vec;
    const double* price;
    const double* action_emb;
    const uint32_t* special_bits;
// ... 43 lines not shown
                if (j < npage) id = s_prev[page_init + j];
                else if (j == npage) id = a;
                if (id >= 0) v = *reinterpret_cast<const float4*>(s_item + id * D + d);
                else v = make_float4(0.f, 0.f, 0.f, 0.f);
            }
            out4[q] = v;
        }
    } else {
        for (int x = lane; x < e.Dn; x += 64) {
            float v = 0.f;
            if (x < UD) {
                v = e.ud[(size_t)b * UD + x];
            } else {
                int r = x - UD;
                int j = r / D;
                int d = r - j * D;
                int id = -1;
                if (j < npage) id = s_prev[page_init + j];
                else if (j == npage) id = a;
                if (id >= 0) v = s_item[id * D + d];
            }
            drow[x] = v;
        }
    }
    for (int c = lane; c < e.Cn; c += 64) {
        int v = 0;
        if (c < e.UC) v = e.ucat[(size_t)b * e.UC + c];
        else if (c == e.UC) v = seq_id;
        else {
            int j = c - e.UC - 1;
            if (j < npage) v = s_prev[page_init + j];
            else if (j == npage) v = a;
        }
        crow[c] = v;
    }
}

__device__ __forceinline__ void stage_items(const EnvDev& e, float* s_item) {
    const int n = e.A * e.D;
    if ((n & 3) == 0) {
        const float4* src = reinterpret_cast<const float4*>(e.item_vec);
        float4* dst = reinterpret_cast<float4*>(s_item);
        for (int i = threadIdx.x; i < (n >> 2); i += blockDim.x) dst[i] = src[i];
    } else {
        for (int i = threadIdx.x; i < n; i += blockDim.x) s_item[i] = e.item_vec[i];
    }
}

#ifndef RL4RS_ROWS_PER_ENV
#define RL4RS_ROWS_PER_ENV 1
#endif

__device__ __forceinline__ int offline_action_id(const EnvDev& e, int b, int cur) {
    return (cur < e.T && cur < e.logT) ? e.exposed[(size_t)b * e.logT + cur] : 0;
}

#define ENV_ROWS_BEGIN(b)
#define ENV_ROWS_ACTED(b, a, lane)
#define ENV_ROWS_BUILT(b, a, lane)
#define ENV_ROWS_DONE(smem)
template <int MODE, bool USE_LDS>
__global__ __launch_bounds__(1024) void k_env_rows(EnvDev e, const int32_t* __restrict__ actions,
                                                   int cur, int n_complete, int j_base, ActTail tail) {
#include "env_rows_body.inc"
}
#undef ENV_ROWS_BEGIN
#undef ENV_ROWS_ACTED
#undef ENV_ROWS_BUILT
#undef ENV_ROWS_DONE
#define ENV_ROWS_BEGIN(b) const int rf_r = rf.rep_prev[b]; int rf_ar = 0
#define ENV_ROWS_ACTED(b, a, lane) rf_ar = row_refine_key(actions, e.A, rf_r)
#define ENV_ROWS_BUILT(b, a, lane) row_refine_env(rf, b, a, rf_r, rf_ar, lane)
#define ENV_ROWS_DONE(smem) row_refine_finish(rf, actions, e.A, smem)
template <bool USE_LDS>
__global__ __launch_bounds__(1024) void k_env_rows_refine(EnvDev e, const int32_t* __restrict__ actions, int cur, ActTail tail, RowRefineArgs rf) {
    constexpr int MODE = 1;
    const int n_complete = 0, j_base = 0;
#include "env_rows_body.inc"
}
#undef ENV_ROWS_BEGIN
#undef ENV_ROWS_ACTED
#undef ENV_ROWS_BUILT
#undef ENV_ROWS_DONE

template <typename TA>
__global__ __launch_bounds__(256) void k_knn(const TA* __restrict__ actions, int n, const double* __restrict__ emb,
                                             int A, int E, const uint32_t* __restrict__ amask,
                                             const uint32_t* __restrict__ smask, const uint32_t* __restrict__ loc,
                                             int W, const uint8_t* __restrict__ dense_mask,
                                             int32_t* __restrict__ out) {
    extern __shared__ __attribute__((aligned(16))) char smem[];
    double* s_act = reinterpret_cast<double*>(smem);
    const int wave = threadIdx.x >> 6, lane = threadIdx.x & 63, nw = blockDim.x >> 6;
    double* my = s_act + wave * E;
    const int b = blockIdx.x * nw + wave;
    if (b < n)
        for (int j = lane; j < E; j += 64) my[j] = (double)actions[(size_t)b * E + j];
    __syncthreads();
    if (b >= n) return;
    double best = -1.0e308;
    int best_k = 0x7fffffff;
    for (int k = lane; k < A; k += 64) {
        double s = 0.0;
        const double* row = emb + (size_t)k * E;
        for (int j = 0; j < E; ++j) s = __dadd_rn(s, __dmul_rn(my[j], row[j]));
        if (amask) {
            uint32_t m = amask[(size_t)b * W + (k >> 5)] & smask[(size_t)b * W + (k >> 5)] & loc[k >> 5];
            if (!((m >> (k & 31)) & 1u)) s = -2147483648.0;
        }
        if (dense_mask && !dense_mask[(size_t)b * A + k]) s = -2147483648.0;
        if (best_k == 0x7fffffff || s > best) { best = s; best_k = k; }
    }
    for (int off = 32; off > 0; off >>= 1) {
        double os = __shfl_xor(best, off);
        int ok = __shfl_xor(best_k, off);
        if (ok != 0x7fffffff && (best_k == 0x7fffffff || os > best || (os == best && ok < best_k))) {
            best = os;
            best_k = ok;
        }
    }
    if (lane == 0) out[b] = best_k;
}

template <typename TA>
__global__ __launch_bounds__(1024) void k_knn_lds(const TA* __restrict__ actions, int n, const double* __restrict__ emb,
                                                  int A, int E, const uint32_t* __restrict__ amask,
                                                  const uint32_t* __restrict__ smask, const uint32_t* __restrict__ loc,
                                                  int W, const uint8_t* __restrict__ dense_mask,
                                                  int32_t* __restrict__ out) {
    extern __shared__ __attribute__((aligned(16))) char smem[];
    const int LDE = E + 1;
    double* s_emb = reinterpret_cast<double*>(smem);
    double* s_act = s_emb + (size_t)A * LDE;
    const int wave = threadIdx.x >> 6, lane = threadIdx.x & 63, nw = blockDim.x >> 6;
    for (int i = threadIdx.x; i < A * E; i += blockDim.x) s_emb[(i / E) * LDE + (i % E)] = emb[i];
    double* my = s_act + wave * E;
    const int b = blockIdx.x * nw + wave;
    if (b < n)
        for (int j = lane; j < E; j += 64) my[j] = (double)actions[(size_t)b * E + j];
    __syncthreads();
    if (b >= n) return;
    double best = -1.0e308;
    int best_k = 0x7fffffff;
    for (int k = lane; k < A; k += 64) {
        double s = 0.0;
        const double* row = s_emb + (size_t)k * LDE;
        for (int j = 0; j < E; ++j) s = __dadd_rn(s, __dmul_rn(my[j], row[j]));
        if (amask) {
            uint32_t m = amask[(size_t)b * W + (k >> 5)] & smask[(size_t)b * W + (k >> 5)] & loc[k >> 5];
            if (!((m >> (k & 31)) & 1u)) s = -2147483648.0;
        }
        if (dense_mask && !dense_mask[(size_t)b * A + k]) s = -2147483648.0;
        if (best_k == 0x7fffffff || s > best) { best = s; best_k = k; }
    }
    for (int off = 32; off > 0; off >>= 1) {
        double os = __shfl_xor(best, off);
        int ok = __shfl_xor(best_k, off);
        if (ok != 0x7fffffff && (best_k == 0x7fffffff || os > best || (os == best && ok < best_k))) {
            best = os;
            best_k = ok;
        }
    }
    if (lane == 0) out[b] = best_k;
}

__global__ __launch_bounds__(256) void k_predict_with_mask(EnvDev e, int N, const float* __restrict__ scores,
// ... 538 lines not shown
    }
    dim3 grid((n + 3) / 4), block(256);
    size_t smem = (size_t)4 * E * sizeof(double);
    if (is_f64)
        hipLaunchKernelGGL(k_knn<double>, grid, block, smem, st, (const double*)actions, n, emb, A, E, amask, smask, loc, W, dense_mask, out);
    else
        hipLaunchKernelGGL(k_knn<float>, grid, block, smem, st, (const float*)actions, n, emb, A, E, amask, smask, loc, W, dense_mask, out);
    RL4RS_LAUNCH_CHECK();
    return RL4RS_OK;
}

int rl4rs_env_act_conti(rl4rs_env* e, const void* actions, int is_f64, int32_t* chosen, void* stream) {
    RL4RS_REQUIRE(e, "act_conti: null argument");
    ENV_JOIN(e, stream);
    return rl4rs::env_act_conti_refine(e, actions, is_f64, chosen, stream, nullptr);
}
}
int rl4rs::env_act_conti_refine(rl4rs_env* e, const void* actions, int is_f64, int32_t* chosen, void* stream, const RowRefineArgs* rf) {
    RL4RS_REQUIRE(e && actions, "act_conti: null argument");
    if (e->cur_steps >= e->d.T) {
        set_error("act at cur_steps=%d >= max_steps=%d", e->cur_steps, e->d.T);
        return RL4RS_ESTATE;
    }
    hipStream_t st = (hipStream_t)stream;
    const EnvDev& d = e->d;
    int layer = d.is_seq ? (e->cur_steps % d.P) / 3 : e->cur_steps / 3;
    RL4RS_REQUIRE(layer < 4, "location layer %d out of range (cur_steps=%d)", layer, e->cur_steps);
    int rc = knn_launch(actions, is_f64, d.B, d.action_emb, d.A, d.E, d.amask, d.smask, d.loc_bits + layer * d.W,
                        d.W, nullptr, e->knn_tmp, st);
    if (rc) return rc;
    if (chosen) RL4RS_HIP_TRY(hipMemcpyAsync(chosen, e->knn_tmp, (size_t)d.B * 4, hipMemcpyDeviceToDevice, st));
    return rl4rs::env_act_discrete_tail(e, e->knn_tmp, ActTail(), stream, rf);
}
extern "C" {

int rl4rs_knn(const void* actions, int is_f64, int32_t n, const double* emb, int32_t A, int32_t E,
              const uint8_t* mask, int32_t* out, void* stream) {
    RL4RS_REQUIRE(actions && emb && out && n > 0 && A > 0 && E > 0, "rl4rs_knn: bad argument");
    return knn_launch(actions, is_f64, n, emb, A, E, nullptr, nullptr, nullptr, 0, mask, out, (hipStream_t)stream);
}

int rl4rs_env_get_cfg(const rl4rs_env* e, rl4rs_env_cfg* out) {
    RL4RS_REQUIRE(e && out, "env_get_cfg: null argument");
    *out = e->cfg;
    return RL4RS_OK;
}
int rl4rs_env_complete_rows(const rl4rs_env* e) { return e ? e->n_complete : RL4RS_EINVAL; }
int rl4rs_env_cur_steps(const rl4rs_env* e) { return e ? e->cur_steps : RL4RS_EINVAL; }
int rl4rs_env_is_reward_step(const rl4rs_env* e) {
    if (!e) return RL4RS_EINVAL;
    if (e->d.is_seq) return (e->cur_steps % e->d.P == 0) ? 1 : 0;
    return (e->cur_steps >= e->d.T) ? 1 : 0;
}

static int complete_base(const rl4rs_env* e) {
    return e->d.is_seq ? e->cur_steps - e->d.P : 0;
}

int rl4rs_env_build_complete_rows(rl4rs_env* e, int32_t rows_per_env, void* stream);
int rl4rs_env_build_complete(rl4rs_env* e, void* stream) {
    RL4RS_REQUIRE(e, "build_complete: null env");
    return rl4rs_env_build_complete_rows(e, e->n_complete, stream);
}

int rl4rs_env_build_complete_rows(rl4rs_env* e, int32_t rows_per_env, void* stream) {
    RL4RS_REQUIRE(e, "build_complete: null env");
    ENV_JOIN(e, stream);
    return rl4rs::env_build_complete_rows_lane(e, rows_per_env, stream);
}
}
int rl4rs::env_build_complete_rows_lane(rl4rs_env* e, int32_t rows_per_env, void* stream) {
    RL4RS_REQUIRE(e, "build_complete: null env");
    RL4RS_REQUIRE(rows_per_env >= 1 && rows_per_env <= e->n_complete, "build_complete: rows_per_env=%d not in 1..%d",
                  rows_per_env, e->n_complete);
    int jb = complete_base(e);
    if (jb < 0 || jb + e->n_complete > e->d.T) {
        set_error("build_complete: cur_steps=%d has no complete page", e->cur_steps);
        return RL4RS_ESTATE;
    }
    hipStream_t st = (hipStream_t)stream;
    int R = e->d.B * rows_per_env;
    return launch_rows<2>(e, R, nullptr, e->cur_steps, rows_per_env, jb, st);
}
extern "C" {

int rl4rs_env_reward_split(rl4rs_env* e, const float* probs, const float* p_last, double* reward, void* stream);
int rl4rs_env_reward(rl4rs_env* e, const float* probs, double* reward, void* stream) {
    return rl4rs_env_reward_split(e, probs, nullptr, reward, stream);
}

int rl4rs_env_reward_split(rl4rs_env* e, const float* probs, const float* p_last, double* reward, void* stream) {
    RL4RS_REQUIRE(e && probs && reward, "reward: null argument");
    ENV_JOIN(e, stream);
    return rl4rs::env_reward_split_lane(e, probs, p_last, reward, stream);
}
}
int rl4rs::env_reward_split_lane(rl4rs_env* e, const float* probs, const float* p_last, double* reward, void* stream) {
    RL4RS_REQUIRE(e && probs && reward, "reward: null argument");
    int jb = complete_base(e);
    if (jb < 0 || jb + e->n_complete > e->d.T) {
        set_error("reward: cur_steps=%d has no complete page", e->cur_steps);
        return RL4RS_ESTATE;
    }
    hipLaunchKernelGGL(k_reward, dim3((e->d.B + 127) / 128), dim3(128), 0, (hipStream_t)stream, e->d,
                       e->cur_steps, e->n_complete, jb, e->cfg.violation_zeroes_reward, probs, p_last, reward);
    RL4RS_LAUNCH_CHECK();
    return RL4RS_OK;
}
extern "C" {

int rl4rs_env_violation(rl4rs_env* e, int32_t* out, void* stream) {
    RL4RS_REQUIRE(e && out, "violation: null argument");
    ENV_JOIN(e, stream);
    hipLaunchKernelGGL(k_violation, dim3((e->d.B + 127) / 128), dim3(128), 0, (hipStream_t)stream, e->d,
                       e->cur_steps, out);
    RL4RS_LAUNCH_CHECK();
    return RL4RS_OK;
}

int rl4rs_env_obs_mask(rl4rs_env* e, void* out, int dtype, void* stream) {
    RL4RS_REQUIRE(e && out && dtype >= 0 && dtype <= 4, "obs_mask: bad argument");
    ENV_JOIN(e, stream);
    const EnvDev& d = e->d;
    int layer = d.is_seq ? (e->cur_steps % d.P) / 3 : e->cur_steps / 3;
    RL4RS_REQUIRE(layer < 4, "location layer %d out of range (cur_steps=%d)", layer, e->cur_steps);
    if (dtype == 4) {
        hipLaunchKernelGGL(k_obs_mask_bits, dim3((unsigned)((d.B * d.W + 255) / 256)), dim3(256), 0, (hipStream_t)stream, e->d, layer,
                           reinterpret_cast<uint32_t*>(out));
        RL4RS_LAUNCH_CHECK();
        return RL4RS_OK;
    }
    size_t total = (size_t)d.B * d.A;
    hipLaunchKernelGGL(k_obs_mask, dim3((unsigned)((total + 255) / 256)), dim3(256), 0, (hipStream_t)stream, e->d,
                       layer, out, dtype);
    RL4RS_LAUNCH_CHECK();
    return RL4RS_OK;
}

int rl4rs_env_offline_action(rl4rs_env* e, int32_t* ids, double* emb, void* stream) {
    RL4RS_REQUIRE(e && (ids || emb), "offline_action: null argument");
    ENV_JOIN(e, stream);
    hipLaunchKernelGGL(k_offline_action, dim3((e->d.B + 127) / 128), dim3(128), 0, (hipStream_t)stream, e->d,
                       e->cur_steps, ids, emb);
    RL4RS_LAUNCH_CHECK();
    return RL4RS_OK;
}

int rl4rs_env_offline_reward(rl4rs_env* e, double* out, void* stream) {
    RL4RS_REQUIRE(e && out, "offline_reward: null argument");
    ENV_JOIN(e, stream);
    hipLaunchKernelGGL(k_offline_reward, dim3((e->d.B + 127) / 128), dim3(128), 0, (hipStream_t)stream, e->d,
                       e->cur_steps, out);
    RL4RS_LAUNCH_CHECK();
    return RL4RS_OK;
}

int rl4rs_env_predict_with_mask(rl4rs_env* e, int32_t N, const float* scores, const int32_t* prev, int32_t prev_cols,
                                const int32_t* cur_step, int32_t* out, void* stream) {
    RL4RS_REQUIRE(e && scores && prev && cur_step && out && N > 0 && prev_cols > 0, "predict_with_mask: bad argument");
    ENV_JOIN(e, stream);
    if (!e->catalog_set) {
        set_error("predict_with_mask: catalogue not loaded");
        return RL4RS_ESTATE;
    }
    hipLaunchKernelGGL(k_predict_with_mask, dim3((N + 3) / 4), dim3(256), 0, (hipStream_t)stream, e->d, N, scores, prev,
                       prev_cols, cur_step, out);
// ... 33 lines not shown
```

### rl4rs_amd/csrc/step.hip

```cpp
#include "common.hpp"
#include "row_refine.hpp"
#include "step_lanes.hpp"

using namespace rl4rs;

struct StepLane {
    hipStream_t st;
    hipEvent_t act_done;
    hipEvent_t done;
    hipEvent_t handed;
    float* obs;
    double* reward;
};

struct rl4rs_stepper {
    rl4rs_env* env;
    rl4rs_dien* dien;
    rl4rs_simnet* simnet;
    const int32_t* slots;
    int32_t seq_num;
    rl4rs_env_cfg cfg;
    int n_complete;
    float* probs;
    float* p_last;
    const float* dense; const int32_t* cat; const int32_t* seq1; const float* c_dense; const int32_t* c_cat;
    bool act_tail;
    bool obs_fold;
    int distinct_hint;
    int probs_rows;
    int32_t* next_off;
    int next_off_cur;
    bool carry;
    bool part_valid;
    bool part_now;
    int part_cur;
    int32_t* part_rep[2];
    int32_t* part_active;
    int32_t* part_cnt;
    const int32_t* part_order;
    uint64_t part_stamp;
    bool overlap;
    bool reset_lane;
    bool reward_lane;
    bool lanes_made;
    StepLane lane[2];
    hipEvent_t ev_entry;
    LaneState lstate;
    LaneHook hook;
    LaneLinks links;
    int32_t* part_active_alt;
    int32_t* part_cnt_alt;
    hipStream_t copy_stream;
    hipEvent_t ev_ready, ev_copied;
};

namespace {

int scorer_forward(rl4rs_stepper* s, int R, int group, const float* dense, const int32_t* cat, float* obs, float* prob, void* stream) {
    if (s->part_now && s->dien) {
        int rc = rl4rs_dien_set_row_partition(s->dien, s->part_rep[s->part_cur], s->part_active, s->part_cnt, s->cfg.batch_size);
        if (rc) return rc;
    }
    return s->dien ? rl4rs_dien_forward(s->dien, R, group, dense, cat, s->slots, obs, prob, stream)
                   : rl4rs_simnet_forward(s->simnet, R, group, dense, cat, s->slots, obs, prob, stream);
}
int scorer_head_prob(rl4rs_stepper* s, int R, const float* obs, float* prob, void* stream) {
    return s->dien ? rl4rs_dien_head_prob(s->dien, R, obs, prob, stream) : rl4rs_simnet_head_prob(s->simnet, R, obs, prob, stream);
}
int scorer_encode(rl4rs_stepper* s, int q, const int32_t* ids, int n, void* stream) {
    return s->dien ? rl4rs_dien_encode(s->dien, q, ids, n, 0, stream) : rl4rs_simnet_encode(s->simnet, q, ids, n, 0, stream);
}

int g_host_mirror = 0;

int ensure_copy_stream(rl4rs_stepper* s) {
    if (!s->copy_stream) {
        RL4RS_HIP_TRY(hipStreamCreateWithFlags(&s->copy_stream, hipStreamNonBlocking));
        RL4RS_HIP_TRY(hipEventCreateWithFlags(&s->ev_ready, hipEventDisableTiming));
        RL4RS_HIP_TRY(hipEventCreateWithFlags(&s->ev_copied, hipEventDisableTiming));
    }
    return RL4RS_OK;
}

__global__ void k_step_tail(uint8_t* done, uint8_t v, double* zero_reward, int n) {
    const int i = blockIdx.x * blockDim.x + threadIdx.x;
    if (i < n) {
        if (done) done[i] = v;
        if (zero_reward) zero_reward[i] = 0.0;
    }
}

__global__ void k_lane_handout(const float* __restrict__ obs_src, float* __restrict__ obs_dst, int64_t n_obs,
                               const double* __restrict__ reward_src, double* __restrict__ reward_dst, int B) {
    const int64_t i = (int64_t)blockIdx.x * blockDim.x + threadIdx.x;
    if (i < n_obs) obs_dst[i] = obs_src[i];
    if (reward_dst && i < B) reward_dst[i] = reward_src[i];
}

int lanes_wait(rl4rs_stepper* s, void* stream, int have_stream) {
    const bool used[2] = {s->lstate.used[0], s->lstate.used[1]};
    if (!lane_join(s->lstate)) return RL4RS_OK;
    for (int i = 0; i < 2; ++i) {
        if (!used[i]) continue;
        if (have_stream) RL4RS_HIP_TRY(hipStreamWaitEvent((hipStream_t)stream, s->lane[i].done, 0));
        else RL4RS_HIP_TRY(hipStreamSynchronize(s->lane[i].st));
    }
    return RL4RS_OK;
}
int hook_join(void* ctx, void* stream, int have_stream) { return lanes_wait(reinterpret_cast<rl4rs_stepper*>(ctx), stream, have_stream); }
void hook_gone(void* ctx, int which) {
    rl4rs_stepper* s = reinterpret_cast<rl4rs_stepper*>(ctx);
    lane_links_gone(s->links, which);
    s->overlap = false;
}

int make_lanes(rl4rs_stepper* s) {
    const size_t B = (size_t)s->cfg.batch_size;
    RL4RS_HIP_TRY(hipEventCreateWithFlags(&s->ev_entry, hipEventDisableTiming));
    for (int i = 0; i < 2; ++i) {
        StepLane& l = s->lane[i];
        RL4RS_HIP_TRY(hipStreamCreateWithFlags(&l.st, hipStreamNonBlocking));
        RL4RS_HIP_TRY(hipEventCreateWithFlags(&l.act_done, hipEventDisableTiming));
        RL4RS_HIP_TRY(hipEventCreateWithFlags(&l.done, hipEventDisableTiming));
        RL4RS_HIP_TRY(hipEventCreateWithFlags(&l.handed, hipEventDisableTiming));
        int rc;
        if ((rc = dev_alloc(&l.obs, B * 256)) || (rc = dev_alloc(&l.reward, B))) return rc;
    }
    s->lanes_made = true;
    return RL4RS_OK;
}

struct NoHook { int operator()() const { return RL4RS_OK; } };

bool plan_refine(rl4rs_stepper* s, int cur, RowRefineArgs* rf) {
    s->part_now = false;
    env_rows_current(s->env, &s->dense, &s->cat);
    const int B = s->cfg.batch_size;
    const bool was_valid = s->part_valid;
    s->part_valid = false;
    if (!s->carry || !s->dien || !s->part_cnt || !dien_takes_partition(s->dien) || !env_refine_fits(s->env)) return false;
    if (s->cfg.is_seq && cur > 0 && cur % s->cfg.page_items == 0) return false;
    const int32_t* order = dien_row_order(s->dien, B);
    memset(rf, 0, sizeof(*rf));
    if (was_valid && s->part_stamp == env_rows_stamp(s->env) && s->part_order == order) {
        rf->rep_prev = s->part_rep[s->part_cur];
    } else {
        DienPartition d;
        dien_last_partition(s->dien, &d);
        if (!(d.stamp > env_rows_stamp(s->env) && d.n_groups == B && d.group == 1 && d.dense == s->dense && d.cat == s->cat &&
              d.slots == s->slots && d.order == order)) return false;
        rf->rep_prev = d.rep;
        rf->active_src = d.active;
        rf->n_active_src = d.n_active;
    }
    dien_drop_pending_expand(s->dien);
    rf->n = B;
    rf->rep = s->part_rep[s->part_cur ^ 1];
    rf->active = s->part_active;
    rf->cnt = s->part_cnt;
    rf->order = order;
    return true;
}
void refined(rl4rs_stepper* s) {
    s->part_cur ^= 1;
    s->part_order = dien_row_order(s->dien, s->cfg.batch_size);
    s->part_stamp = env_rows_stamp(s->env);
    s->part_valid = s->part_now = true;
}

bool fold_obs(const rl4rs_stepper* s) {
    const int n = s->n_complete, B = s->cfg.batch_size;
    if (!s->obs_fold || !s->dien || n < 2) return false;
    if (!rl4rs::dien_augru_rows64(s->dien, B, n)) return false;
    const int64_t with = rl4rs::dien_augru_rounds(s->dien, B, s->distinct_hint, n);
    const int64_t without = rl4rs::dien_augru_rounds(s->dien, B, s->distinct_hint, n - 1);
    return with > 0 && without > 0 && with <= without;
}

template <typename Hook = NoHook>
int after_act(rl4rs_stepper* s, int cur_before, float* obs, double* reward, uint8_t* done, uint32_t* mask_bits, void* stream,
              Hook on_obs = Hook(), bool tail_done = false, bool may_fold = false) {
    hipStream_t st = (hipStream_t)stream;
// ... 49 lines not shown
__global__ void k_record_d3rl(const float* obs, int obs_dim, const int32_t* prev, int T, int c0, int ncols, int cur, double* out, int B) {
    const int w = obs_dim + ncols + 1;
    const int64_t i = (int64_t)blockIdx.x * blockDim.x + threadIdx.x;
    if (i >= (int64_t)B * w) return;
    const int b = (int)(i / w), c = (int)(i - (int64_t)b * w);
    double v;
    if (c < obs_dim) v = (double)obs[(size_t)b * obs_dim + c];
    else if (c < obs_dim + ncols) v = (double)prev[(size_t)b * T + c0 + (c - obs_dim)];
    else v = (double)cur;
    out[i] = v;
}
__global__ void k_record_click(const float* probs, const float* p_last, int m, float* out, int B) {
    const int i = blockIdx.x * blockDim.x + threadIdx.x;
    if (i >= B * (m + 1)) return;
    const int b = i / (m + 1), j = i - b * (m + 1);
    out[i] = j < m ? probs[(size_t)b * m + j] : p_last[b];
}
__global__ void k_record_status(const int32_t* env_err, int32_t* range_flag, int32_t* out) {
    if (threadIdx.x == 0 && blockIdx.x == 0) {
        out[0] = env_err ? *env_err : 0;
        out[1] = range_flag ? atomicExch(range_flag, 0) : 0;
    }
}

int lane_transition(rl4rs_stepper* s, const LanePlan& lp, const LaneState& before, int cur, RowRefineArgs* rf, const int32_t* actions_dev, float* obs_dev,
                    double* reward_dev, void* stream) {
    hipStream_t home = (hipStream_t)stream;
    StepLane& l = s->lane[lp.on];
    const int B = s->cfg.batch_size;
    if (lp.wait_entry) {
        RL4RS_HIP_TRY(hipEventRecord(s->ev_entry, home));
        RL4RS_HIP_TRY(hipStreamWaitEvent(l.st, s->ev_entry, 0));
    }
    if (lp.wait_act) RL4RS_HIP_TRY(hipStreamWaitEvent(l.st, s->lane[lp.on ^ 1].act_done, 0));
    if (lp.wait_handout) RL4RS_HIP_TRY(hipStreamWaitEvent(l.st, l.handed, 0));
    if (!rf->active_src) { rf->active_src = s->part_active; rf->n_active_src = s->part_cnt; }
    rf->active = s->part_active_alt;
    rf->cnt = s->part_cnt_alt;
    env_flip_rows(s->env);
    ActTail tail;
    tail.done = nullptr; tail.done_v = 0;
    tail.zero_reward = (reward_dev && !lp.reward) ? l.reward : nullptr;
    tail.next_action = s->next_off + (size_t)(cur + 1) * B;
    tail.next_cur = cur + 1;
    int rc = rl4rs::env_act_discrete_tail(s->env, actions_dev, tail, l.st, rf);
    if (rc) {
        env_flip_rows(s->env);
        env_rows_current(s->env, &s->dense, &s->cat);
        lane_undo(s->lstate, before);
        return rc;
    }
    std::swap(s->part_active, s->part_active_alt);
    std::swap(s->part_cnt, s->part_cnt_alt);
    env_rows_current(s->env, &s->dense, &s->cat);
    refined(s);
    s->next_off_cur = cur + 1;
    RL4RS_HIP_TRY(hipEventRecord(l.act_done, l.st));
    if (lp.reward) {
        const int n = s->n_complete;
        if ((rc = rl4rs::env_build_complete_rows_lane(s->env, n, l.st)) ||
            (rc = rl4rs_dien_set_obs_last(s->dien, l.obs)) ||
            (rc = rl4rs_dien_set_row_partition(s->dien, s->part_rep[s->part_cur], s->part_active, s->part_cnt, B)) ||
            (rc = dien_forward_lane_full(s->dien, 0, B * n, n, s->c_dense, s->c_cat, s->slots, nullptr, s->probs, l.st, stream, nullptr,
                                         s->lane[1].done)) ||
            (rc = rl4rs::env_reward_split_lane(s->env, s->probs, nullptr, l.reward, l.st))) {
            (void)hipEventRecord(l.done, l.st);
            return rc;
        }
        s->probs_rows = n;
    } else if ((rc = rl4rs_dien_set_row_partition(s->dien, s->part_rep[s->part_cur], s->part_active, s->part_cnt, B)) ||
        (rc = dien_forward_lane(s->dien, lp.on, B, s->dense, s->cat, s->slots, l.obs, l.st, stream))) {
        (void)hipEventRecord(l.done, l.st);
        return rc;
    }
    RL4RS_HIP_TRY(hipEventRecord(l.done, l.st));
    RL4RS_HIP_TRY(hipStreamWaitEvent(home, l.done, 0));
    const int64_t n_obs = (int64_t)B * 256;
    hipLaunchKernelGGL(k_lane_handout, dim3((unsigned)((n_obs + 255) / 256)), dim3(256), 0, home, l.obs, obs_dev, n_obs, l.reward, reward_dev, B);
    RL4RS_LAUNCH_CHECK();
    RL4RS_HIP_TRY(hipEventRecord(l.handed, home));
    return RL4RS_OK;
}

int reward_act(const rl4rs_stepper* s, int cur) {
    const int T = s->cfg.max_steps;
    if (!s->cfg.is_seq) return T - 1;
    const int d = cur / s->cfg.page_items * s->cfg.page_items + s->cfg.page_items - 1;
    return d < T - 1 ? d : T - 1;
}

int attach(rl4rs_env* env, rl4rs_dien* dien, rl4rs_simnet* simnet, const int32_t* slots_dev, int32_t seq_num, rl4rs_stepper** out) {
    RL4RS_REQUIRE(env && (dien || simnet) && slots_dev && out && seq_num >= 1 && seq_num <= 4, "env_attach_scorer: bad argument");
    rl4rs_stepper* s = new rl4rs_stepper();
    memset(s, 0, sizeof(*s));
    s->env = env; s->dien = dien; s->simnet = simnet; s->slots = slots_dev; s->seq_num = seq_num;
    int rc = rl4rs_env_get_cfg(env, &s->cfg);
    if (rc) { delete s; return rc; }
    s->n_complete = rl4rs_env_complete_rows(env);
    const size_t B = (size_t)s->cfg.batch_size;
    float* ring = nullptr;
    if ((rc = dev_alloc(&s->probs, B * (size_t)s->n_complete)) || (rc = dev_alloc(&s->p_last, B)) ||
        (rc = dev_alloc(&ring, B * (size_t)(s->cfg.max_steps + 1)))) {
        if (s->probs) (void)hipFree(s->probs);
        if (s->p_last) (void)hipFree(s->p_last);
        delete s;
        return rc;
    }
    s->next_off = reinterpret_cast<int32_t*>(ring);
    s->next_off_cur = -1;
    if (dien) {
        float* part = nullptr;
        if ((rc = dev_alloc(&part, 4 * B + 8))) { rl4rs_stepper_destroy(s); return rc; }
        s->part_rep[0] = reinterpret_cast<int32_t*>(part);
        s->part_rep[1] = s->part_rep[0] + B;
        s->part_active = s->part_rep[1] + B;
        s->part_active_alt = s->part_active + B;
        s->part_cnt = s->part_active_alt + B;
        s->part_cnt_alt = s->part_cnt + 4;
        if (hipMemset(s->part_cnt, 0, 32) != hipSuccess) { rl4rs_stepper_destroy(s); set_error("env_attach_scorer: hipMemset failed"); return RL4RS_EHIP; }
        s->carry = true;
    }
    s->hook.ctx = s;
    s->hook.join = hook_join;
    s->hook.gone = hook_gone;
    lane_links_attach(s->links, LANE_LINK_ENV, env_lane_slot(env), &s->hook);
    if (dien) {
        lane_links_attach(s->links, LANE_LINK_SCORER, dien_lane_slot(dien), &s->hook);
        if (dien_takes_partition(dien) && ((rc = make_lanes(s)) || (rc = dien_reserve_lane_scratch(dien, s->cfg.batch_size)))) {
            rl4rs_stepper_destroy(s);
            return rc;
        }
        s->overlap = s->reset_lane = s->reward_lane = s->lanes_made;
    }
    s->act_tail = true;
    s->obs_fold = true;
    s->distinct_hint = s->cfg.batch_size;
    void* p;
    int64_t nb;
#define BUF(which, field, type) if ((rc = rl4rs_env_buffer(env, which, &p, &nb))) { rl4rs_stepper_destroy(s); return rc; } s->field = reinterpret_cast<type>(p)
    BUF(RL4RS_BUF_DENSE, dense, const float*);
    BUF(RL4RS_BUF_CATEGORY, cat, const int32_t*);
    BUF(RL4RS_BUF_SEQ1, seq1, const int32_t*);
    BUF(RL4RS_BUF_C_DENSE, c_dense, const float*);
    BUF(RL4RS_BUF_C_CATEGORY, c_cat, const int32_t*);
#undef BUF
    *out = s;
    return RL4RS_OK;
}

}

extern "C" {

int rl4rs_env_attach_scorer(rl4rs_env* env, rl4rs_dien* net, const int32_t* slots_dev, int32_t seq_num, rl4rs_stepper** out) {
    return attach(env, net, nullptr, slots_dev, seq_num, out);
}
int rl4rs_env_attach_simnet(rl4rs_env* env, rl4rs_simnet* net, const int32_t* slots_dev, int32_t seq_num, rl4rs_stepper** out) {
    return attach(env, nullptr, net, slots_dev, seq_num, out);
}

int rl4rs_stepper_destroy(rl4rs_stepper* s) {
    if (!s) return RL4RS_OK;
    (void)lanes_wait(s, nullptr, 0);
    lane_links_release(s->links, &s->hook);
    if (s->lanes_made || s->ev_entry) {
        if (s->ev_entry) (void)hipEventDestroy(s->ev_entry);
        for (int i = 0; i < 2; ++i) {
            StepLane& l = s->lane[i];
            if (l.st) { (void)hipStreamSynchronize(l.st); (void)hipStreamDestroy(l.st); }
            if (l.act_done) (void)hipEventDestroy(l.act_done);
            if (l.done) (void)hipEventDestroy(l.done);
            if (l.handed) (void)hipEventDestroy(l.handed);
            if (l.obs) (void)hipFree(l.obs);
            if (l.reward) (void)hipFree(l.reward);
        }
    }
    if (s->probs) (void)hipFree(s->probs);
    if (s->p_last) (void)hipFree(s->p_last);
    if (s->next_off) (void)hipFree(s->next_off);
    if (s->part_rep[0]) (void)hipFree(s->part_rep[0]);
    if (s->ev_ready) (void)hipEventDestroy(s->ev_ready);
    if (s->ev_copied) (void)hipEventDestroy(s->ev_copied);
    if (s->copy_stream) (void)hipStreamDestroy(s->copy_stream);
    delete s;
    return RL4RS_OK;
}

int rl4rs_env_step_discrete(rl4rs_stepper* s, const int32_t* actions_dev, float* obs_dev, double* reward_dev, uint8_t* done_dev,
                            uint32_t* mask_bits_dev, void* stream) {
    RL4RS_REQUIRE(s && actions_dev && obs_dev, "env_step_discrete: null argument");
    const int cur = rl4rs_env_cur_steps(s->env);
    const bool own_row = s->next_off_cur == cur && cur >= 0 && actions_dev == s->next_off + (size_t)cur * s->cfg.batch_size;
    s->next_off_cur = -1;
    RowRefineArgs rf;
    const bool refine = plan_refine(s, cur, &rf);
    {
        const int T = s->cfg.max_steps;
        LaneCall c;
        memset(&c, 0, sizeof(c));
        c.overlap = s->overlap && s->act_tail && cur < T && lane_links_mine(s->links, LANE_LINK_ENV, &s->hook) &&
                    lane_links_mine(s->links, LANE_LINK_SCORER, &s->hook);
        c.dien_x = s->dien && dien_lane_path(s->dien, s->cfg.batch_size);
        c.carried = refine;
        c.reward_due = s->cfg.is_seq ? (cur + 1) % s->cfg.page_items == 0 : cur + 1 >= T;
        c.extra_outputs = mask_bits_dev != nullptr || done_dev != nullptr;
        c.own_row = own_row;
        c.seq_num = s->seq_num; c.distinct_hint = s->distinct_hint; c.n_cu = s->dien ? dien_n_cu(s->dien) : 0;
        c.to_reward = (c.reward_due || !(s->reset_lane || s->reward_lane)) ? 0 : reward_act(s, cur) - cur;
        c.no_reward_lane = !s->reward_lane;
        c.reward_fold = c.reward_due && reward_dev && c.overlap && c.dien_x && refine && fold_obs(s);
        const LaneState before = s->lstate;
        const LanePlan lp = lane_decide(s->lstate, c);
        if (lp.lane) return lane_transition(s, lp, before, cur, &rf, actions_dev, obs_dev, reward_dev, stream);
        if (lp.join) {
            for (int i = 0; i < 2; ++i) RL4RS_HIP_TRY(hipStreamWaitEvent((hipStream_t)stream, s->lane[i].done, 0));
        }
    }
    if (!s->act_tail) {
        int rc = rl4rs::env_act_discrete_tail(s->env, actions_dev, ActTail(), stream, refine ? &rf : nullptr);
        if (rc) return rc;
        if (refine) refined(s);
        return after_act(s, cur, obs_dev, reward_dev, done_dev, mask_bits_dev, stream, NoHook(), false, true);
    }
    const int T = s->cfg.max_steps;
    const int due = s->cfg.is_seq ? ((cur + 1) % s->cfg.page_items == 0 ? 1 : 0) : (cur + 1 >= T ? 1 : 0);
    ActTail tail;
    tail.done = done_dev; tail.done_v = (uint8_t)(cur >= T - 1 ? 1 : 0);
    tail.zero_reward = (reward_dev && !due) ? reward_dev : nullptr;
    tail.next_action = (cur + 1 <= T) ? s->next_off + (size_t)(cur + 1) * s->cfg.batch_size : nullptr;
    tail.next_cur = cur + 1;
    int rc = rl4rs::env_act_discrete_tail(s->env, actions_dev, tail, stream, refine ? &rf : nullptr);
    if (rc) return rc;
    if (refine) refined(s);
    if (tail.next_action) s->next_off_cur = cur + 1;
    const bool covered = rl4rs_env_is_reward_step(s->env) == due;
    return after_act(s, cur, obs_dev, reward_dev, done_dev, mask_bits_dev, stream, NoHook(), covered, true);
}

int rl4rs_stepper_set_act_tail(rl4rs_stepper* s, int32_t on) {
    RL4RS_REQUIRE(s, "stepper_set_act_tail: null argument");
    s->act_tail = on != 0;
    s->next_off_cur = -1;
    return RL4RS_OK;
}

int rl4rs_stepper_set_obs_fold(rl4rs_stepper* s, int32_t on) {
    RL4RS_REQUIRE(s, "stepper_set_obs_fold: null argument");
    s->obs_fold = on != 0;
    return RL4RS_OK;
}

int rl4rs_stepper_set_partition_carry(rl4rs_stepper* s, int32_t on) {
    RL4RS_REQUIRE(s, "stepper_set_partition_carry: null argument");
    s->carry = on != 0 && s->part_cnt != nullptr;
    s->part_valid = s->part_now = false;
    return RL4RS_OK;
}

int rl4rs_stepper_set_step_overlap(rl4rs_stepper* s, int32_t on) {
    RL4RS_REQUIRE(s, "stepper_set_step_overlap: null argument");
    s->overlap = on != 0 && s->lanes_made;
    return RL4RS_OK;
}

int rl4rs_stepper_set_reset_lane(rl4rs_stepper* s, int32_t on) {
    RL4RS_REQUIRE(s, "stepper_set_reset_lane: null argument");
    s->reset_lane = on != 0 && s->lanes_made;
    return RL4RS_OK;
}

int rl4rs_stepper_set_reward_lane(rl4rs_stepper* s, int32_t on) {
    RL4RS_REQUIRE(s, "stepper_set_reward_lane: null argument");
    s->reward_lane = on != 0 && s->lanes_made;
    return RL4RS_OK;
}

int rl4rs_stepper_lane_stats_ex(const rl4rs_stepper* s, int64_t* reset_runs, int64_t* reward_runs) {
    RL4RS_REQUIRE(s, "stepper_lane_stats_ex: null argument");
    if (reset_runs) *reset_runs = s->lstate.ran_reset;
    if (reward_runs) *reward_runs = s->lstate.ran_reward;
    return RL4RS_OK;
}

int rl4rs_stepper_observe(rl4rs_stepper* s, float* obs_dev, int32_t* taken, void* stream) {
    RL4RS_REQUIRE(s && obs_dev && taken, "stepper_observe: null argument");
    *taken = 0;
    const int cur = rl4rs_env_cur_steps(s->env);
    const int B = s->cfg.batch_size;
    LaneCall c;
    memset(&c, 0, sizeof(c));
    c.overlap = s->overlap && s->act_tail && cur == 0 && lane_links_mine(s->links, LANE_LINK_ENV, &s->hook) &&
                lane_links_mine(s->links, LANE_LINK_SCORER, &s->hook);
    c.dien_x = s->dien && dien_lane_path(s->dien, B);
    c.seq_num = s->seq_num; c.distinct_hint = s->distinct_hint; c.n_cu = s->dien ? dien_n_cu(s->dien) : 0;
    c.observe = true;
    c.no_reset_lane = !s->reset_lane;
    c.to_reward = 1 + reward_act(s, cur) - cur;
    if (!lane_observe_eligible(c)) return RL4RS_OK;
    hipStream_t home = (hipStream_t)stream;
    int rc = lanes_wait(s, stream, 1);
    if (rc) return rc;
    s->next_off_cur = -1;
    if ((rc = rl4rs_env_offline_action(s->env, s->next_off, nullptr, stream))) return rc;
    const LanePlan lp = lane_decide(s->lstate, c);
    StepLane& l = s->lane[lp.on];
    s->part_now = false;
    env_rows_current(s->env, &s->dense, &s->cat);
    RL4RS_HIP_TRY(hipEventRecord(s->ev_entry, home));
    RL4RS_HIP_TRY(hipStreamWaitEvent(l.st, s->ev_entry, 0));
    if ((rc = dien_forward_lane_full(s->dien, lp.on, B, 1, s->dense, s->cat, s->slots, l.obs, nullptr, l.st, stream, l.act_done, nullptr))) {
        (void)hipEventRecord(l.act_done, l.st);
        (void)hipEventRecord(l.done, l.st);
        return rc;
    }
    RL4RS_HIP_TRY(hipEventRecord(l.done, l.st));
    RL4RS_HIP_TRY(hipStreamWaitEvent(home, l.done, 0));
    const int64_t n_obs = (int64_t)B * 256;
    hipLaunchKernelGGL(k_lane_handout, dim3((unsigned)((n_obs + 255) / 256)), dim3(256), 0, home, l.obs, obs_dev, n_obs, l.reward, (double*)nullptr, B);
    RL4RS_LAUNCH_CHECK();
    RL4RS_HIP_TRY(hipEventRecord(l.handed, home));
    s->next_off_cur = 0;
    *taken = 1;
    return RL4RS_OK;
}

int rl4rs_stepper_lane_stats(const rl4rs_stepper* s, int64_t* lane0, int64_t* lane1, int64_t* joins) {
    RL4RS_REQUIRE(s, "stepper_lane_stats: null argument");
    if (lane0) *lane0 = s->lstate.ran[0];
    if (lane1) *lane1 = s->lstate.ran[1];
    if (joins) *joins = s->lstate.joins;
    return RL4RS_OK;
}

int rl4rs_stepper_reward_rows(const rl4rs_stepper* s) { return s ? s->probs_rows : RL4RS_EINVAL; }

int rl4rs_stepper_click_probs(rl4rs_stepper* s, float* out_dev, void* stream) {
    RL4RS_REQUIRE(s && out_dev, "stepper_click_probs: null argument");
    { const int rcj = lanes_wait(s, stream, 1); if (rcj) return rcj; }
    RL4RS_REQUIRE(s->n_complete >= 2 && s->probs_rows > 0, "stepper_click_probs: no reward step yet");
    const int B = s->cfg.batch_size, n = s->n_complete;
    hipStream_t st = (hipStream_t)stream;
    if (s->probs_rows == n) {
        RL4RS_HIP_TRY(hipMemcpyAsync(out_dev, s->probs, (size_t)B * n * 4, hipMemcpyDeviceToDevice, st));
    } else {
        hipLaunchKernelGGL(k_record_click, dim3((B * n + 255) / 256), dim3(256), 0, st, s->probs, s->p_last, n - 1, out_dev, B);
        RL4RS_LAUNCH_CHECK();
    }
    return RL4RS_OK;
}

int rl4rs_stepper_set_distinct_hint(rl4rs_stepper* s, int32_t n_distinct) {
    RL4RS_REQUIRE(s && n_distinct >= 1, "stepper_set_distinct_hint: bad argument");
    s->distinct_hint = n_distinct < s->cfg.batch_size ? n_distinct : s->cfg.batch_size;
    if (s->dien) return rl4rs_dien_set_distinct_hint(s->dien, s->distinct_hint);
    return RL4RS_OK;
}
// ... 199 lines not shown
```

### rl4rs_amd/csrc/step_lanes.hpp

```cpp
#pragma once
#include <stdint.h>

namespace rl4rs {

inline int64_t lane_pair_workgroups(int seq_num, int distinct_hint) { return 2 * (int64_t)seq_num * ((distinct_hint + 31) / 32); }

struct LaneCall {
    bool overlap;
    bool dien_x;
    bool carried;
    bool reward_due;
    bool extra_outputs;
    bool own_row;
    int seq_num, distinct_hint, n_cu;
    bool observe;
    bool no_reset_lane;
    bool reward_fold;
    bool no_reward_lane;
    int to_reward;
};

inline bool lane_room(const LaneCall& c) {
    return c.overlap && c.dien_x && !c.extra_outputs && lane_pair_workgroups(c.seq_num, c.distinct_hint) <= c.n_cu;
}
// ... 30 lines not shown
}

inline void lane_undo(LaneState& s, const LaneState& before) { s = before; }

enum { LANE_LINK_ENV = 0, LANE_LINK_SCORER = 1 };
struct LaneHook {
    void* ctx;
    int (*join)(void* ctx, void* stream, int have_stream);
    void (*gone)(void* ctx, int which);
};
inline int lanes_join(const LaneHook* h, void* stream, bool have_stream = true) {
    return h ? h->join(h->ctx, stream, have_stream ? 1 : 0) : 0;
}
inline void lanes_gone(const LaneHook* h, int which) {
    if (h && h->gone) h->gone(h->ctx, which);
}
struct LaneLinks { const LaneHook** slot[2]; };
inline void lane_links_attach(LaneLinks& l, int which, const LaneHook** slot, const LaneHook* hook) {
    if (*slot && *slot != hook) {
        (void)lanes_join(*slot, nullptr, false);
        lanes_gone(*slot, which);
    }
    *slot = hook;
    l.slot[which] = slot;
}
inline void lane_links_gone(LaneLinks& l, int which) { l.slot[which] = nullptr; }
inline bool lane_links_mine(const LaneLinks& l, int which, const LaneHook* hook) { return l.slot[which] && *l.slot[which] == hook; }
inline void lane_links_release(LaneLinks& l, const LaneHook* hook) {
    for (int w = 0; w < 2; ++w) {
        if (lane_links_mine(l, w, hook)) *l.slot[w] = nullptr;
        l.slot[w] = nullptr;
    }
}

inline int lane_first(int to_reward) { return 1 ^ ((to_reward - 1) & 1); }

inline bool lane_reward_eligible(const LaneState& s, const LaneCall& c) {
    return lane_room(c) && !c.observe && c.carried && c.reward_due && c.reward_fold && !c.no_reward_lane && s.in_flight && s.last == 1;
}

inline LanePlan lane_decide(LaneState& s, const LaneCall& c) {
    LanePlan p = {};
    if (lane_reward_eligible(s, c)) {
        p.lane = p.reward = true;
        p.on = 0;
        p.wait_act = true;
        p.wait_entry = !c.own_row;
        p.wait_handout = !p.wait_entry && s.used[0];
        s.used[0] = true;
        s.last = 0;
        s.ran_reward += 1;
        s.next = 1;
        return p;
    }
    if (lane_observe_eligible(c)) {
        p.join = lane_join(s);
        p.lane = p.observe = true;
        p.on = c.to_reward > 0 ? lane_first(c.to_reward) : s.next;
        p.wait_entry = true;
        s.in_flight = true;
        s.used[p.on] = true;
        s.last = p.on;
        s.ran_reset += 1;
        s.next = p.on ^ 1;
        return p;
    }
    if (!lane_eligible(c)) {
        p.join = lane_join(s);
        return p;
    }
    p.lane = true;
    p.on = (!s.in_flight && c.to_reward > 0) ? lane_first(c.to_reward) : s.next;
    p.wait_act = s.in_flight;
    p.wait_entry = !s.in_flight || !c.own_row;
    p.wait_handout = !p.wait_entry && s.used[p.on];
    s.in_flight = true;
    s.used[p.on] = true;
    s.last = p.on;
    s.ran[p.on] += 1;
    s.next = p.on ^ 1;
    return p;
}

}
```

### rl4rs_amd/device.py

```python
import ctypes as C
import os

import numpy as np
import torch

from . import _lib
from ._lib import check

BUF_PREV_ACTIONS, BUF_ACTION_MASK, BUF_SPECIAL_MASK, BUF_DENSE, BUF_CATEGORY, BUF_SEQ0, BUF_SEQ1, \
    BUF_C_DENSE, BUF_C_CATEGORY, BUF_ERROR_FLAG = range(10)
DIEN_ALL_FEATURE, DIEN_SCORES, DIEN_QUERY, DIEN_H1, DIEN_N_ACTIVE, DIEN_ROW_REP, DIEN_ROW_ACTIVE = range(7)
DIEN_H1_FRAG, DIEN_LEAD = 7, 8

_MASK_DTYPES = {torch.uint8: 0, torch.int32: 1, torch.int64: 2, torch.float32: 3}


def _stream():
    return C.c_void_p(torch.cuda.current_stream().cuda_stream)


def _ptr(t):
    return C.c_void_p(t.data_ptr()) if t is not None else C.c_void_p(0)


# ... 116 lines not shown
        assert ex.shape == (self.B, self.log_steps) and fb.shape == ex.shape, (ex.shape, self.log_steps)
        assert hi.shape == (self.B, self.L) and ud.shape == (self.B, 32) and uc.shape == (self.B, 10)
        check(self.lib.rl4rs_env_load_batch(self.h, _ptr(ex), _ptr(fb), _ptr(hi), _ptr(ud), _ptr(uc), _stream()))
        self._keep = (ex, fb, hi, ud, uc)

    def load_lines(self, tables, n_lines, line_idx, uniq_idx=None, hist_unique=None):
        assert line_idx.dtype == torch.int32 and line_idx.numel() == self.B and line_idx.is_contiguous()
        n_uniq = 0 if uniq_idx is None else int(uniq_idx.numel())
        if n_uniq:
            assert uniq_idx.dtype == torch.int32 and uniq_idx.is_contiguous()
            assert hist_unique.dtype == torch.int32 and tuple(hist_unique.shape) == (n_uniq, self.L) and hist_unique.is_contiguous()
        ex = tables['exposed']
        assert ex.shape[1] == self.log_steps and tables['history'].shape[1] == self.L
        check(self.lib.rl4rs_env_load_lines(self.h, _ptr(ex), _ptr(tables['feedback']), _ptr(tables['history']),
                                            _ptr(tables['user_dense']), _ptr(tables['user_cat']), int(n_lines), int(ex.shape[1]),
                                            _ptr(line_idx), _ptr(uniq_idx), n_uniq, _ptr(hist_unique), _stream()))
        self._keep = (line_idx, uniq_idx, hist_unique)

    def reset(self):
        check(self.lib.rl4rs_env_reset(self.h, _stream()))

    def act_discrete(self, actions):
        a = _dev_tensor(actions, torch.int32, self.device).reshape(-1)
        assert a.numel() == self.B, (a.shape, self.B)
        check(self.lib.rl4rs_env_act_discrete(self.h, _ptr(a), _stream()))
        return a

    def act_conti(self, actions):
        if isinstance(actions, torch.Tensor):
            a = actions.to(self.device)
            if a.dtype not in (torch.float32, torch.float64):
                a = a.to(torch.float64)
            a = a.contiguous()
        else:
            a = np.asarray(actions)
            a = a.astype(np.float32 if a.dtype == np.float32 else np.float64)
            a = torch.from_numpy(np.ascontiguousarray(a)).to(self.device)
        assert a.shape == (self.B, self.E), (a.shape, (self.B, self.E))
        chosen = torch.empty(self.B, dtype=torch.int32, device=self.device)
        check(self.lib.rl4rs_env_act_conti(self.h, _ptr(a), 1 if a.dtype == torch.float64 else 0,
                                           _ptr(chosen), _stream()))
        return chosen

    @property
    def cur_steps(self):
        return self.lib.rl4rs_env_cur_steps(self.h)

    def is_reward_step(self):
        return bool(self.lib.rl4rs_env_is_reward_step(self.h))

    def buffer_ptr(self, which):
        p = C.c_void_p()
        n = C.c_int64()
        check(self.lib.rl4rs_env_buffer(self.h, which, C.byref(p), C.byref(n)))
        return p, n.value

    def snapshot(self, which):
        p, n = self.buffer_ptr(which)
        B, nc = self.B, self.n_complete
        shapes = {
            BUF_PREV_ACTIONS: ((B, self.T), torch.int32), BUF_ACTION_MASK: ((B, self.W), torch.int32),
            BUF_SPECIAL_MASK: ((B, self.W), torch.int32), BUF_DENSE: ((B, self.Dn), torch.float32),
            BUF_CATEGORY: ((B, self.Cn), torch.int32), BUF_SEQ0: ((B, self.L), torch.int32),
            BUF_SEQ1: ((B, self.L), torch.int32), BUF_C_DENSE: ((B * nc, self.Dn), torch.float32),
            BUF_C_CATEGORY: ((B * nc, self.Cn), torch.int32), BUF_ERROR_FLAG: ((1,), torch.int32),
        }
        shape, dt = shapes[which]
        out = torch.empty(shape, dtype=dt, device=self.device)
        assert out.numel() * out.element_size() == n, (which, shape, n)
        check(self.lib.rl4rs_copy_d2d(_ptr(out), p, n, _stream()))
        return out

    def bits_to_mask(self, bits):
        b = bits.cpu().numpy().view(np.uint32)
        k = np.arange(self.A)
        return ((b[:, k >> 5] >> (k & 31).astype(np.uint32)) & 1).astype(np.int64)

    def build_complete(self, rows_per_env=None):
        if rows_per_env is None:
            check(self.lib.rl4rs_env_build_complete(self.h, _stream()))
        else:
            check(self.lib.rl4rs_env_build_complete_rows(self.h, rows_per_env, _stream()))

    def reward(self, probs, p_last=None):
        out = torch.empty(self.B, dtype=torch.float64, device=self.device)
        m = self.n_complete - (1 if p_last is not None else 0)
        assert probs.dtype == torch.float32 and probs.numel() == self.B * m
        assert p_last is None or (p_last.dtype == torch.float32 and p_last.numel() == self.B)
        check(self.lib.rl4rs_env_reward_split(self.h, _ptr(probs), _ptr(p_last), _ptr(out), _stream()))
        return out

    def violation(self):
        out = torch.empty(self.B, dtype=torch.int32, device=self.device)
        check(self.lib.rl4rs_env_violation(self.h, _ptr(out), _stream()))
        return out

    def obs_mask(self, dtype=torch.int64):
        out = torch.empty((self.B, self.A), dtype=dtype, device=self.device)
        check(self.lib.rl4rs_env_obs_mask(self.h, _ptr(out), _MASK_DTYPES[dtype], _stream()))
        return out

    def obs_mask_bits(self, out=None):
        if out is None:
            out = torch.empty((self.B, (self.A + 31) // 32), dtype=torch.int32, device=self.device)
        assert out.dtype == torch.int32 and tuple(out.shape) == (self.B, (self.A + 31) // 32) and out.is_contiguous()
        check(self.lib.rl4rs_env_obs_mask(self.h, _ptr(out), 4, _stream()))
        return out

    def offline_action(self, conti=False):
        ids = torch.empty(self.B, dtype=torch.int32, device=self.device)
        emb = torch.empty((self.B, self.E), dtype=torch.float64, device=self.device) if conti else None
        check(self.lib.rl4rs_env_offline_action(self.h, _ptr(ids), _ptr(emb), _stream()))
        return emb if conti else ids

    def offline_reward(self):
        out = torch.empty(self.B, dtype=torch.float64, device=self.device)
        check(self.lib.rl4rs_env_offline_reward(self.h, _ptr(out), _stream()))
        return out

    def predict_with_mask(self, scores, obs_tail):
        scores = scores.to(device=self.device, dtype=torch.float32).contiguous()
        tail = obs_tail.to(device=self.device)
        prev = tail[:, :-1].to(torch.int32).contiguous()
        cur = tail[:, -1].to(torch.int32).contiguous()
        N = scores.shape[0]
        out = torch.empty(N, dtype=torch.int32, device=self.device)
        check(self.lib.rl4rs_env_predict_with_mask(self.h, N, _ptr(scores), _ptr(prev), prev.shape[1], _ptr(cur),
                                                   _ptr(out), _stream()))
        return out

    def check_error_flag(self):
        flag = int(self.snapshot(BUF_ERROR_FLAG).item())
        if flag:
            raise IndexError("an action id outside [0, action_size) was passed to act() "
                             "(numpy would raise at rl4rs/env/slate.py:199)")


def knn(actions, action_emb_dev, mask=None):
    lib = _lib.load()
    dev = action_emb_dev.device
    a = actions if isinstance(actions, torch.Tensor) else torch.from_numpy(np.ascontiguousarray(np.asarray(actions)))
    if a.dtype not in (torch.float32, torch.float64):
        a = a.to(torch.float64)
    a = a.to(dev).contiguous()
    n, E = a.shape
    out = torch.empty(n, dtype=torch.int32, device=dev)
    m = None
    if mask is not None:
        m = (torch.as_tensor(np.asarray(mask) >= 0.5) if not isinstance(mask, torch.Tensor) else (mask >= 0.5))
        m = m.to(device=dev, dtype=torch.uint8).contiguous()
        assert m.shape == (n, action_emb_dev.shape[0])
    check(lib.rl4rs_knn(_ptr(a), 1 if a.dtype == torch.float64 else 0, n, _ptr(action_emb_dev),
                        action_emb_dev.shape[0], E, _ptr(m), _ptr(out), _stream()))
    return out


SCORER_MODES = {'auto': 0, 'fp32': 1, 'fp16x2': 2}
class DeviceStepper(object):

    def __init__(self, env, net, slots, act_tail=True, obs_fold=True, partition_carry=True, step_overlap=True, reset_lane=True,
                 reward_lane=True):
        self.lib = _lib.load()
        self.env, self.net, self.slots = env, net, slots
        assert slots.dtype == torch.int32 and slots.is_contiguous() and slots.shape[1] == env.B
        h = C.c_void_p()
        attach = self.lib.rl4rs_env_attach_simnet if isinstance(net, DeviceSimnet) else self.lib.rl4rs_env_attach_scorer
        check(attach(env.h, net.h, _ptr(slots), int(slots.shape[0]), C.byref(h)))
        self.h = h
        self.act_tail = bool(act_tail)
        if not self.act_tail:
            check(self.lib.rl4rs_stepper_set_act_tail(self.h, 0))
        if not obs_fold:
            check(self.lib.rl4rs_stepper_set_obs_fold(self.h, 0))
        if not partition_carry:
            check(self.lib.rl4rs_stepper_set_partition_carry(self.h, 0))
        if not step_overlap:
            check(self.lib.rl4rs_stepper_set_step_overlap(self.h, 0))
        if not reset_lane:
            check(self.lib.rl4rs_stepper_set_reset_lane(self.h, 0))
        if not reward_lane:
            check(self.lib.rl4rs_stepper_set_reward_lane(self.h, 0))
        self.reset_lane = bool(step_overlap and reset_lane)
        self._distinct_hint = None
        self.B, self.A, self.E, self.W, self.device = env.B, env.A, env.E, env.W, env.device
        self.obs_dim = int(getattr(net, 'obs_dim', 256))

    def close(self):
        if getattr(self, 'h', None) is not None and self.h:
            self.lib.rl4rs_stepper_destroy(self.h)
            self.h = None

    def __del__(self):
        try:
            self.close()
        except Exception:
            pass

    def set_distinct_hint(self, n):
        n = self.B if n is None else max(1, min(int(n), self.B))
        if n != self._distinct_hint:
            check(self.lib.rl4rs_stepper_set_distinct_hint(self.h, n))
            self._distinct_hint = n

    def lane_stats(self):
        a, b, j = C.c_int64(0), C.c_int64(0), C.c_int64(0)
        check(self.lib.rl4rs_stepper_lane_stats(self.h, C.byref(a), C.byref(b), C.byref(j)))
        return int(a.value), int(b.value), int(j.value)

    def lane_stats_ex(self):
        a, b = C.c_int64(0), C.c_int64(0)
        check(self.lib.rl4rs_stepper_lane_stats_ex(self.h, C.byref(a), C.byref(b)))
        return int(a.value), int(b.value)

    def observe(self):
        if not self.reset_lane or not self.act_tail:
            return None
        obs = torch.empty((self.B, self.obs_dim), dtype=torch.float32, device=self.device)
        taken = C.c_int32(0)
        check(self.lib.rl4rs_stepper_observe(self.h, _ptr(obs), C.byref(taken), _stream()))
        return obs if taken.value else None

    def reward_rows(self):
        return int(self.lib.rl4rs_stepper_reward_rows(self.h))

    def click_probs(self):
        out = torch.empty((self.B, self.env.n_complete), dtype=torch.float32, device=self.device)
        check(self.lib.rl4rs_stepper_click_probs(self.h, _ptr(out), _stream()))
        return out

    def step(self, actions, conti=False, want_reward=True, want_mask_bits=False):
        obs = torch.empty((self.B, self.obs_dim), dtype=torch.float32, device=self.device)
        reward = torch.empty(self.B, dtype=torch.float64, device=self.device) if want_reward else None
        bits = torch.empty((self.B, self.W), dtype=torch.int32, device=self.device) if want_mask_bits else None
        if conti:
            a = actions.to(self.device) if isinstance(actions, torch.Tensor) else torch.from_numpy(np.ascontiguousarray(actions)).to(self.device)
            if a.dtype not in (torch.float32, torch.float64):
                a = a.to(torch.float64)
            a = a.contiguous()
            assert a.shape == (self.B, self.E), (a.shape, (self.B, self.E))
            chosen = torch.empty(self.B, dtype=torch.int32, device=self.device)
            check(self.lib.rl4rs_env_step_conti(self.h, _ptr(a), 1 if a.dtype == torch.float64 else 0, _ptr(chosen), _ptr(obs),
                                                _ptr(reward), None, _ptr(bits), _stream()))
        else:
            chosen = _dev_tensor(actions, torch.int32, self.device).reshape(-1)
            assert chosen.numel() == self.B, (chosen.shape, self.B)
            check(self.lib.rl4rs_env_step_discrete(self.h, _ptr(chosen), _ptr(obs), _ptr(reward), None, _ptr(bits), _stream()))
        return obs, reward, bits, chosen

    def next_offline_action(self, rows=None):
        if not self.act_tail:
            return None
        ptr, step = C.c_void_p(), C.c_int32(-1)
        check(self.lib.rl4rs_stepper_next_offline_action(self.h, C.byref(ptr), C.byref(step)))
        if step.value < 0 or not ptr.value:
            return None
        t = None if rows is None else rows.get(ptr.value)
        if t is None:
            t = _alias_i32(ptr.value, self.B, self.device, self)
            if rows is not None:
                rows[ptr.value] = t
        return int(step.value), t

    def offline_action_view(self):
        last = getattr(self, '_last_record', None)
        if last is None or last[0].offline_action < 0:
            return None
        L, rec = last
        off = int(L.offline_action)
        return rec[off:off + self.B * 4].view(torch.int32)

    def _layout(self, want, conti):
        key = (want, bool(conti))
        cache = self.__dict__.setdefault('_layouts', {})
        if key not in cache:
            L = _lib.StepRecord()
            check(self.lib.rl4rs_stepper_record_layout(self.h, want, 1 if conti else 0, C.byref(L)))
            rec = torch.empty(int(L.total_bytes), dtype=torch.uint8, device=self.device)
            cache[key] = (L, rec)
        return cache[key]

    def step_record(self, actions, conti=False, want=(), shadow=None):
        bits = 0
        for name in want:
            bits |= _lib.STEP_WANT[name]
        L, rec = self._layout(bits, conti)
        if actions is None:
            a = None
        elif conti:
            a = actions
            if not (isinstance(a, torch.Tensor) and a.is_cuda):
                a = np.asarray(a.detach().cpu().numpy() if isinstance(a, torch.Tensor) else a)
                a = to_device_async(a, torch.float32 if a.dtype == np.float32 else torch.float64, self.device)
            elif a.dtype not in (torch.float32, torch.float64):
                a = a.to(torch.float64)
            a = a.contiguous()
# ... 2145 lines not shown
```

### rl4rs_amd/env/slate.py

```python
import os

import numpy as np

from .base import RecSimBase, RecState, RecordBatch
from ..data import CatalogTables, RecordColumns
from ..utils.datautil import FeatureUtil
from .. import device as D

_CATALOG_CACHE = {}


def _catalog(iteminfo_file, action_size, action_emb_size, onehot):
    key = (iteminfo_file, action_size, action_emb_size, bool(onehot))
    if key not in _CATALOG_CACHE:
        _CATALOG_CACHE[key] = CatalogTables(iteminfo_file, action_size, action_emb_size, onehot)
    return _CATALOG_CACHE[key]


class StateRows(object):

    def __init__(self, owner, kind):
        self.owner = owner
        self.kind = kind

# ... 456 lines not shown
        masked = self.config.get("support_rllib_mask", False)
        d3rl = self.config.get("support_d3rl_mask", False)
        rows = state["state"] if (masked or d3rl) else state
        samples = rows.owner
        tensor_mode = samples._tensor_mode()
        B = self.batch_size
        if self.config.get("rawstate_as_obs", False) and tensor_mode:
            env = samples._live()
            seq0, seq1 = env.snapshot(D.BUF_SEQ0), env.snapshot(D.BUF_SEQ1)
            obs = {"category_feature": env.snapshot(D.BUF_CATEGORY), "dense_feature": env.snapshot(D.BUF_DENSE),
                   "sequence_feature": [seq0] + [seq1] * (self.config['seq_num'] - 1)}
            if masked:
                obs["action_mask"] = state["action_mask"]
            return obs
        if self.config.get("rawstate_as_obs", False):
            feat, _ = self.FeatureUtil.feature_extraction(rows)
            obs = [{"category_feature": feat[2][i], "dense_feature": feat[1][i], "sequence_feature": feat[0][i]}
                   for i in range(B)]
            if masked:
                am = state["action_mask"]
                am = am.cpu().numpy() if hasattr(am, 'cpu') else am
                return [dict(action_mask=am[i], **obs[i]) for i in range(B)]
            return obs
        env = samples._live()
        net, slots = self._net_for(samples)
        dp, _ = env.buffer_ptr(D.BUF_DENSE)
        cp, _ = env.buffer_ptr(D.BUF_CATEGORY)
        obs, _ = net.forward(B, 1, dp, cp, slots, want_obs=True, want_prob=False)
        self._last_obs = (samples._batch_version, env.cur_steps, obs if not tensor_mode else obs.clone())
        if tensor_mode:
            if masked:
                return {"action_mask": state["action_mask"], "obs": obs}
            if d3rl:
                import torch
                return torch.cat([obs.double(), state["masked_actions"].double(), state["cur_steps"].double()], dim=-1)
            return obs
        obs = D.to_host(obs)
        if masked:
            return [{"action_mask": m, "obs": o} for m, o in zip(state["action_mask"], obs)]
        if d3rl:
            return np.concatenate([obs, state["masked_actions"], state["cur_steps"]], axis=-1)
        return obs

    def _stock_methods(self, samples):
        from .seqslate import SeqSlateState, SeqSlateRecEnv
        st, ev = type(samples), type(self)
        stock_state = SeqSlateState if samples.is_seq else SlateState
        stock_env = SeqSlateRecEnv if samples.is_seq else SlateRecEnv
        return (st.act is stock_state.act and st.state is stock_state.state and st.get_complete_states is SlateState.get_complete_states
                and st._masked_actions is stock_state._masked_actions
                and ev.obs_fn is SlateRecEnv.obs_fn and ev.forward is SlateRecEnv.forward and ev._reward_due is stock_env._reward_due)

    def _fused_ok(self, samples):
        cfg = self.config
        return (not cfg.get("rawstate_as_obs", False) and not cfg.get('no_state_row_reuse', False)
                and not cfg.get('no_fused_step', False) and samples._env.n_complete > 1
                and not (samples._tensor_mode() and (cfg.get("support_d3rl_mask", False) or cfg.get("simulator_info_fetch", False)))
                and self._stock_methods(samples))

    def _lane_switch(self, name):
        key = 'no_' + name
        return not self.config.get(key, os.environ.get('RL4RS_' + key.upper(), '') not in ('', '0'))

    def _reset_lane_ok(self, samples):
        cfg = self.config
        off = any(cfg.get(k, os.environ.get(v, '') not in ('', '0'))
                  for k, v in (('no_step_overlap', 'RL4RS_NO_STEP_OVERLAP'), ('no_act_tail', 'RL4RS_NO_ACT_TAIL')))
        return (not off and self._lane_switch('reset_lane') and self._fused_ok(samples) and not cfg.get("support_conti_env", False)
                and not cfg.get("support_rllib_mask", False) and not cfg.get("support_d3rl_mask", False))

    def _stepper_for(self, samples):
        env = samples._live()
        net, slots = self._net_for(samples)
        key = (id(env), id(net), slots.data_ptr())
        if getattr(self, '_stepper_key', None) != key:
            self._stepper = None
            self._next_rows = {}
            no_tail = self.config.get('no_act_tail', os.environ.get('RL4RS_NO_ACT_TAIL', '') not in ('', '0'))
            no_fold = self.config.get('no_reward_obs_fold', os.environ.get('RL4RS_NO_REWARD_OBS_FOLD', '') not in ('', '0'))
            no_carry = self.config.get('no_partition_carry', os.environ.get('RL4RS_NO_PARTITION_CARRY', '') not in ('', '0'))
            no_overlap = self.config.get('no_step_overlap', os.environ.get('RL4RS_NO_STEP_OVERLAP', '') not in ('', '0'))
            self._stepper = D.DeviceStepper(env, net, slots, act_tail=not no_tail, obs_fold=not no_fold, partition_carry=not no_carry,
                                            step_overlap=not no_overlap, reset_lane=self._lane_switch('reset_lane'),
                                            reward_lane=self._lane_switch('reward_lane'))
            self._stepper_key = key
        own = samples.is_seq and env.cur_steps >= samples.page_items
        self._stepper.set_distinct_hint(None if own else getattr(samples, '_n_lines', None))
        return env, net, self._stepper

    def _mask_dicts(self, rec):
        import gc
        keep = self.__dict__.setdefault('_obs_keep', [])
        while len(keep) >= 2:
            keep.pop(0)
        was_on = gc.isenabled()
        gc.disable()
        try:
            out = [{"action_mask": m, "obs": o} for m, o in zip(rec.mask, rec.obs)]
        finally:
            if was_on:
                gc.enable()
        keep.append(out)
        return out

    def _copied_obs(self, rec, masked):
        if not masked:
            return np.array(rec.obs)
        m, o = np.array(rec.mask), np.array(rec.obs)
        return [{"action_mask": mi, "obs": oi} for mi, oi in zip(m, o)]

    def sample(self, batch_size):
        samples = self._recData.sample(batch_size)
        if samples._tensor_mode() and self._reset_lane_ok(samples):
            env, net, stepper = self._stepper_for(samples)
            obs = stepper.observe()
            if obs is not None:
                nxt = stepper.next_offline_action(self.__dict__.setdefault('_next_rows', {}))
                samples._next_offline_dev = None if nxt is None else ((samples._batch_version, nxt[0]), nxt[1])
                self._last_obs = None
                return samples, obs
        if samples._tensor_mode() or not self._fused_ok(samples):
            return samples, self.obs_fn(samples.state)
        env, net, stepper = self._stepper_for(samples)
        conti = bool(self.config.get("support_conti_env", False))
        masked = self.config.get("support_rllib_mask", False)
        d3rl = (not masked) and self.config.get("support_d3rl_mask", False)
        want = ['offline_action'] + (['mask_i64'] if masked else []) + (['d3rl_obs'] if d3rl else [])
        built = {}

        def in_the_gpu_shadow(rec):
            if masked:
                built['obs'] = self._mask_dicts(rec)
            samples.infos
            if env.cur_steps < self.max_steps and env.cur_steps < samples._exposed_len_min:
                samples._next_offline = ((samples._batch_version, env.cur_steps),
                                         samples._offline_from_host(env.cur_steps, conti, None if conti else stepper.offline_action_view()))

        r = stepper.observe_record(conti=conti, want=want, shadow=in_the_gpu_shadow)
        samples._range_seen = getattr(samples, '_range_seen', 0) | int(r.status[1])
        self._last_obs = None
        if self.config.get('copy_outputs', False):
            return samples, self._copied_obs(r, masked)
        return samples, (built['obs'] if masked else r.obs)

    def _step(self, samples, action, **kwargs):
        if not self._fused_ok(samples):
            return RecSimBase._step(self, samples, action, **kwargs)
        env, net, stepper = self._stepper_for(samples)
        first_of_page = samples.is_seq and env.cur_steps > 0 and env.cur_steps % samples.page_items == 0
        if first_of_page:
            self._seq_slots_own(env, self.batch_size)
        conti = bool(self.config.get("support_conti_env", False))
        last = kwargs['step'] >= self.max_steps - 1
        masked = self.config.get("support_rllib_mask", False)
        if samples._tensor_mode():
            obs, reward, _, chosen = stepper.step(action, conti=conti)
            samples.last_actions = chosen
            nxt = None if conti else stepper.next_offline_action(self.__dict__.setdefault('_next_rows', {}))
            samples._next_offline_dev = None if nxt is None else ((samples._batch_version, nxt[0]), nxt[1])
            if masked:
                obs = {"action_mask": samples._obs_mask(), "obs": obs}
        else:
            d3rl = (not masked) and self.config.get("support_d3rl_mask", False)
            fetch = bool(self.config.get("simulator_info_fetch", False))
            want = ['offline_action']
            if masked:
                want.append('mask_i64')
# ... 83 lines not shown
```

Baseline: 6.446 million.

## Precompute remaining slate-step rows ahead and hand out cached observations

Adds a replay-ahead path for slate envs. Once the remaining steps follow logged offline actions, it builds the DIEN input rows for all remaining 8 or 9 steps in one kernel and runs one grouped forward over them. Later steps then copy cached observations per representative row through a small handout kernel instead of running a scorer forward each step. The partition of representative rows is refined ahead as well. This adds extra buffers and a state machine that cancels the prefetch when the actions diverge, which costs wasted work on a drop. It also disables the G8/G9 cat-group plan when rows differ.

```diff
diff --git a/include/rl4rs_hip.h b/include/rl4rs_hip.h
--- a/include/rl4rs_hip.h
+++ b/include/rl4rs_hip.h
@@ -288,6 +288,10 @@
 int rl4rs_stepper_set_reset_lane(rl4rs_stepper* s, int32_t on);
 int rl4rs_stepper_set_reward_lane(rl4rs_stepper* s, int32_t on);
 int rl4rs_stepper_lane_stats_ex(const rl4rs_stepper* s, int64_t* reset_runs, int64_t* reward_runs);
+int rl4rs_stepper_set_replay_ahead(rl4rs_stepper* s, int32_t on);
+int rl4rs_env_build_ahead_rows(rl4rs_env* e, int32_t n, float* dense_out, int32_t* cat_out, const int32_t* rep, const int32_t* active,
+                               const int32_t* n_active, int32_t* rep_out, int32_t* active_out, int32_t* n_active_out, void* stream);
+int rl4rs_stepper_replay_stats(const rl4rs_stepper* s, int64_t* started, int64_t* handed, int64_t* dropped);
 int rl4rs_stepper_click_probs(rl4rs_stepper* s, float* out_dev, void* stream);
 int rl4rs_stepper_reward_rows(const rl4rs_stepper* s);
 int rl4rs_stepper_next_offline_action(rl4rs_stepper* s, const int32_t** ids_dev, int32_t* step);
diff --git a/rl4rs_amd/_lib.py b/rl4rs_amd/_lib.py
--- a/rl4rs_amd/_lib.py
+++ b/rl4rs_amd/_lib.py
@@ -285,6 +285,9 @@
     'rl4rs_stepper_set_reset_lane': (_I, [_P, _I32]),
     'rl4rs_stepper_set_reward_lane': (_I, [_P, _I32]),
     'rl4rs_stepper_lane_stats_ex': (_I, [_P, _P, _P]),
+    'rl4rs_stepper_set_replay_ahead': (_I, [_P, _I32]),
+    'rl4rs_env_build_ahead_rows': (_I, [_P, _I32, _P, _P, _P, _P, _P, _P, _P, _P, _P]),
+    'rl4rs_stepper_replay_stats': (_I, [_P, _P, _P, _P]),
     'rl4rs_stepper_click_probs': (_I, [_P, _P, _P]),
     'rl4rs_stepper_reward_rows': (_I, [_P]),
     'rl4rs_stepper_next_offline_action': (_I, [_P, _P, _P]),
diff --git a/rl4rs_amd/csrc/common.hpp b/rl4rs_amd/csrc/common.hpp
--- a/rl4rs_amd/csrc/common.hpp
+++ b/rl4rs_amd/csrc/common.hpp
@@ -135,9 +135,11 @@
 
 void dien_set_obs_mirror(rl4rs_dien* n, float* host_visible);
 bool dien_obs_mirror_used(const rl4rs_dien* n);
+void dien_set_group_rows(rl4rs_dien* n, float* head_out);
 void dien_drop_pending_expand(rl4rs_dien* n);
 int64_t dien_augru_rounds(const rl4rs_dien* n, int B, int live, int group);
 bool dien_augru_rows64(const rl4rs_dien* n, int B, int group);
+bool dien_augru_rows64_auto(const rl4rs_dien* n, int B, int group);
 
 const LaneHook** env_lane_slot(rl4rs_env* e);
 const LaneHook** dien_lane_slot(rl4rs_dien* n);
@@ -150,6 +152,11 @@
                            float* obs, float* prob, void* stream, void* home, void* after_dedup, void* before_augru);
 int env_build_complete_rows_lane(rl4rs_env* e, int32_t rows_per_env, void* stream);
 int env_reward_split_lane(rl4rs_env* e, const float* probs, const float* p_last, double* reward, void* stream);
+struct AheadPart {
+    const int32_t* rep; const int32_t* active; const int32_t* cnt;
+    int32_t* rep_out; int32_t* active_out; int32_t* cnt_out;
+};
+int env_build_ahead_rows_lane(rl4rs_env* e, int32_t c0, int32_t n, float* dense_out, int32_t* cat_out, const AheadPart* part, void* stream);
 bool dien_lane_path(const rl4rs_dien* n, int rows);
 int dien_n_cu(const rl4rs_dien* n);
 
diff --git a/rl4rs_amd/csrc/dien.hip b/rl4rs_amd/csrc/dien.hip
--- a/rl4rs_amd/csrc/dien.hip
+++ b/rl4rs_amd/csrc/dien.hip
@@ -1460,6 +1460,7 @@
     float* obs_mirror;
     bool obs_mirror_used;
     float* obs_last;
+    bool group_rows; float* head_out;
     std::vector<void*> owned;
     int profiling;
     std::vector<EvPair> pending;
@@ -2310,7 +2311,7 @@
     struct SetGuard { rl4rs_dien* n; bool on; ~SetGuard() { if (on) swap_scratch(n); } } set_guard{n, set == 1};
     if (set == 1) swap_scratch(n);
     n->last_set = set; n->last_rows = R; n->last_home = home;
-    struct MirrorOnce { rl4rs_dien* n; ~MirrorOnce() { n->obs_mirror = nullptr; n->obs_last = nullptr; n->part_rep = nullptr; } } mirror_once{n};
+    struct MirrorOnce { rl4rs_dien* n; ~MirrorOnce() { n->obs_mirror = nullptr; n->obs_last = nullptr; n->part_rep = nullptr; n->group_rows = false; n->head_out = nullptr; } } mirror_once{n};
     DienCall c{};
     c.R = R; c.group = group; c.obs = obs != nullptr; c.prob = prob != nullptr;
     c.mirror = n->obs_mirror != nullptr; c.obs_last = n->obs_last != nullptr;
@@ -2318,13 +2319,14 @@
     c.row_order = n->row_order && n->row_order_n == ngroups;
     c.augru_rows = n->augru_rows; c.distinct_hint = n->distinct_hint;
     c.dense_vec = (n->Dn & 3) == 0 && (reinterpret_cast<uintptr_t>(dense) & 15) == 0;
+    c.rows_differ = n->group_rows;
     RL4RS_REQUIRE(!c.carried || (dien_takes_partition(n) && c.part_groups == ngroups),
                   "dien_forward: the row partition set for this forward is for %d groups with the row dedup on (forward: %d groups)", n->part_groups, ngroups);
     RL4RS_REQUIRE(!c.obs_last || c.prob, "dien_forward: rl4rs_dien_set_obs_last needs a forward that returns probabilities");
     const DienPlan p = dien_plan(n->t, c);
     DienFwd f;
     f.R = R; f.group = group; f.n_groups = ngroups; f.dense = dense; f.cat = cat; f.slots = slots;
-    f.obs_out = obs ? obs : n->obs_tmp; f.prob = prob; f.st = (hipStream_t)stream;
+    f.obs_out = obs ? obs : (n->head_out ? n->head_out : n->obs_tmp); f.prob = prob; f.st = (hipStream_t)stream;
     f.set = set; f.home = home;
     f.order_in = c.row_order ? n->row_order : nullptr;
     f.rep = c.carried ? n->part_rep : n->dd_rep;
@@ -2501,6 +2503,7 @@
 }
 namespace rl4rs {
 void dien_set_obs_mirror(rl4rs_dien* n, float* host_visible) { if (n) n->obs_mirror = host_visible; }
+void dien_set_group_rows(rl4rs_dien* n, float* head_out) { if (n) { n->group_rows = true; n->head_out = head_out; } }
 void dien_last_partition(const rl4rs_dien* n, DienPartition* out) { *out = n->dd_info; }
 bool dien_takes_partition(const rl4rs_dien* n) { return n && n->t.row_dedup && !n->t.dup_store; }
 const int32_t* dien_row_order(const rl4rs_dien* n, int n_groups) { return (n->row_order && n->row_order_n == n_groups) ? n->row_order : nullptr; }
@@ -2538,6 +2541,9 @@
 }
 bool dien_augru_rows64(const rl4rs_dien* n, int B, int group) {
     return n && n->t.fp16x2 && n->t.augru_x && (int64_t)B * group <= n->c.max_rows && augru_rows64(n->augru_rows, B * group, group, n->S, n->n_cu);
+}
+bool dien_augru_rows64_auto(const rl4rs_dien* n, int B, int group) {
+    return dien_augru_rows64(n, B, group) && augru_rows64(0, B * group, group, n->S, n->n_cu);
 }
 int64_t dien_augru_rounds(const rl4rs_dien* n, int B, int live, int group) {
     if (!n || !n->t.fp16x2 || !n->t.augru_x || (int64_t)B * group > n->c.max_rows) return -1;
diff --git a/rl4rs_amd/csrc/dien_plan.hpp b/rl4rs_amd/csrc/dien_plan.hpp
--- a/rl4rs_amd/csrc/dien_plan.hpp
+++ b/rl4rs_amd/csrc/dien_plan.hpp
@@ -63,6 +63,7 @@
     int augru_rows;
     int distinct_hint;
     bool dense_vec;
+    bool rows_differ;
 };
 
 enum class PlanDedup { None, Launch, Carried };
@@ -105,7 +106,7 @@
                c.augru_rows != 64 && augru_shadow_room(c.distinct_hint, n_groups, t.S, t.n_cu) && g16_shadow_fits(c.R, t.Dn, t.Fld, t.U);
     p.cat_h16 = t.fp16x2 && t.cat16;
     if (p.shadow) p.cat = PlanCat::Shadow;
-    else if (t.cat_v2_shape() && t.cat_group && t.Cn >= 11 && (c.group == 8 || c.group == 9)) p.cat = c.group == 8 ? PlanCat::G8 : PlanCat::G9;
+    else if (t.cat_v2_shape() && t.cat_group && t.Cn >= 11 && (c.group == 8 || c.group == 9) && !c.rows_differ) p.cat = c.group == 8 ? PlanCat::G8 : PlanCat::G9;
     else if (t.cat_v2_shape()) p.cat = t.Cn == 21 ? PlanCat::V2_21 : PlanCat::V2_24;
     else p.cat = PlanCat::V1;
     p.dense_side = t.dense_fork;
diff --git a/rl4rs_amd/csrc/env.hip b/rl4rs_amd/csrc/env.hip
--- a/rl4rs_amd/csrc/env.hip
+++ b/rl4rs_amd/csrc/env.hip
@@ -149,6 +149,57 @@
 #undef ENV_ROWS_ACTED
 #undef ENV_ROWS_BUILT
 #undef ENV_ROWS_DONE
+
+template <bool USE_LDS>
+__global__ __launch_bounds__(1024) void k_env_rows_ahead(EnvDev e, int c0, int n, float* __restrict__ dense_out, int32_t* __restrict__ cat_out,
+                                                         AheadPart part) {
+    extern __shared__ __attribute__((aligned(16))) char smem[];
+    float* s_item_lds = reinterpret_cast<float*>(smem);
+    const size_t item_bytes = USE_LDS ? (((size_t)e.A * e.D * 4 + 15) & ~size_t(15)) : 0;
+    const int wave = threadIdx.x >> 6, lane = threadIdx.x & 63, nw = blockDim.x >> 6;
+    int32_t* s_prev = reinterpret_cast<int32_t*>(smem + item_bytes) + wave * e.T;
+    if (USE_LDS) {
+        stage_items(e, s_item_lds);
+        __syncthreads();
+    }
+    const float* s_item = USE_LDS ? s_item_lds : e.item_vec;
+    auto logged = [&](int b, int j) {
+        const int a = offline_action_id(e, b, j);
+        return (a < 0 || a >= e.A) ? 0 : a;
+    };
+    const int total_waves = gridDim.x * nw;
+    for (int b = blockIdx.x * nw + wave; b < e.B; b += total_waves) {
+        for (int j = lane; j < e.T; j += 64)
+            s_prev[j] = j <= c0 ? e.prev[(size_t)b * e.T + j] : (j < c0 + n ? logged(b, j) : 0);
+        if (part.rep) {
+            const int r = part.rep[b];
+            bool differs = false;
+            if (r != b)
+                for (int j = c0 + 1 + lane; j < c0 + n; j += 64) differs |= logged(b, j) != logged(r, j);
+            const bool split = __any(differs);
+            if (lane == 0) {
+                if (b < part.cnt[0]) part.active_out[b] = part.active[b];
+                if (split) {
+                    const int pos = atomicAdd(part.cnt_out, 1);
+                    if (pos < e.B) part.active_out[pos] = b;
+                }
+                part.rep_out[b] = split ? b : r;
+            }
+        }
+        __builtin_amdgcn_wave_barrier();
+        __builtin_amdgcn_fence(__ATOMIC_ACQ_REL, "wavefront");
+        for (int k = n - 1; k >= 0; --k) {
+            const int c = c0 + k;
+            const size_t r = (size_t)b * n + k;
+            build_row(e, s_item, s_prev, b, 0, e.T, 1, s_prev[c], dense_out + r * e.Dn, cat_out + r * e.Cn, lane);
+            __builtin_amdgcn_wave_barrier();
+            __builtin_amdgcn_fence(__ATOMIC_ACQ_REL, "wavefront");
+            if (lane == 0) s_prev[c] = 0;
+            __builtin_amdgcn_wave_barrier();
+            __builtin_amdgcn_fence(__ATOMIC_ACQ_REL, "wavefront");
+        }
+    }
+}
 
 template <typename TA>
 __global__ __launch_bounds__(256) void k_knn(const TA* __restrict__ actions, int n, const double* __restrict__ emb,
@@ -853,6 +904,34 @@
     int R = e->d.B * rows_per_env;
     return launch_rows<2>(e, R, nullptr, e->cur_steps, rows_per_env, jb, st);
 }
+extern "C" int rl4rs_env_build_ahead_rows(rl4rs_env* e, int32_t n, float* dense_out, int32_t* cat_out, const int32_t* rep, const int32_t* active,
+                                          const int32_t* n_active, int32_t* rep_out, int32_t* active_out, int32_t* n_active_out, void* stream) {
+    RL4RS_REQUIRE(e, "build_ahead_rows: null env");
+    ENV_JOIN(e, stream);
+    const rl4rs::AheadPart part = {rep, active, n_active, rep_out, active_out, n_active_out};
+    return rl4rs::env_build_ahead_rows_lane(e, e->cur_steps - 1, n, dense_out, cat_out, rep ? &part : nullptr, stream);
+}
+int rl4rs::env_build_ahead_rows_lane(rl4rs_env* e, int32_t c0, int32_t n, float* dense_out, int32_t* cat_out, const AheadPart* part, void* stream) {
+    RL4RS_REQUIRE(e && dense_out && cat_out, "build_ahead_rows: null argument");
+    RL4RS_REQUIRE(!e->d.is_seq, "build_ahead_rows: Slate envs only");
+    RL4RS_REQUIRE(c0 >= 0 && n >= 1 && c0 + n <= e->d.T && c0 == e->cur_steps - 1, "build_ahead_rows: steps %d..%d behind cur_steps=%d of %d",
+                  c0, c0 + n - 1, e->cur_steps, e->d.T);
+    hipStream_t st = (hipStream_t)stream;
+    AheadPart p;
+    memset(&p, 0, sizeof(p));
+    if (part) {
+        p = *part;
+        RL4RS_REQUIRE(p.rep && p.active && p.cnt && p.rep_out && p.active_out && p.cnt_out, "build_ahead_rows: incomplete partition");
+        RL4RS_HIP_TRY(hipMemcpyAsync(p.cnt_out, p.cnt, 4, hipMemcpyDeviceToDevice, st));
+    }
+    const RowsLaunch L = rows_launch(e, e->d.B * n, 2);
+    if (L.lds)
+        hipLaunchKernelGGL((k_env_rows_ahead<true>), dim3(L.grid), dim3(L.threads), L.smem, st, e->d, c0, n, dense_out, cat_out, p);
+    else
+        hipLaunchKernelGGL((k_env_rows_ahead<false>), dim3(L.grid), dim3(L.threads), L.smem, st, e->d, c0, n, dense_out, cat_out, p);
+    RL4RS_LAUNCH_CHECK();
+    return RL4RS_OK;
+}
 extern "C" {
 
 int rl4rs_env_reward_split(rl4rs_env* e, const float* probs, const float* p_last, double* reward, void* stream);
diff --git a/rl4rs_amd/csrc/step.hip b/rl4rs_amd/csrc/step.hip
--- a/rl4rs_amd/csrc/step.hip
+++ b/rl4rs_amd/csrc/step.hip
@@ -50,6 +50,14 @@
     LaneLinks links;
     int32_t* part_active_alt;
     int32_t* part_cnt_alt;
+    int replay_ahead;
+    AheadState ahead;
+    float* ah_dense;
+    int32_t* ah_cat;
+    float* ah_obs;
+    int32_t* ah_rep;
+    int32_t* ah_active;
+    int32_t* ah_cnt;
     hipStream_t copy_stream;
     hipEvent_t ev_ready, ev_copied;
 };
@@ -97,7 +105,17 @@
     if (reward_dst && i < B) reward_dst[i] = reward_src[i];
 }
 
+__global__ void k_ahead_handout(const float* __restrict__ src, const int32_t* __restrict__ rep, int n, int k, float* __restrict__ obs_dst,
+                                double* __restrict__ reward_dst, int B) {
+    const int64_t i = (int64_t)blockIdx.x * blockDim.x + threadIdx.x;
+    if (i >= (int64_t)B * 64) return;
+    const int b = (int)(i >> 6), q = (int)(i & 63);
+    reinterpret_cast<float4*>(obs_dst)[i] = reinterpret_cast<const float4*>(src + ((size_t)rep[b] * n + k) * 256)[q];
+    if (reward_dst && i < B) reward_dst[i] = 0.0;
+}
+
 int lanes_wait(rl4rs_stepper* s, void* stream, int have_stream) {
+    (void)ahead_cancel(s->ahead);
     const bool used[2] = {s->lstate.used[0], s->lstate.used[1]};
     if (!lane_join(s->lstate)) return RL4RS_OK;
     for (int i = 0; i < 2; ++i) {
@@ -313,6 +331,144 @@
     return RL4RS_OK;
 }
 
+int ensure_ahead(rl4rs_stepper* s) {
+    if (s->ah_obs) return RL4RS_OK;
+    const size_t R = (size_t)s->cfg.batch_size * 9, B = (size_t)s->cfg.batch_size;
+    float *cat = nullptr, *part = nullptr;
+    int rc;
+    if ((rc = dev_alloc(&s->ah_dense, R * (size_t)s->cfg.dense_feature_num)) || (rc = dev_alloc(&cat, R * (size_t)s->cfg.category_feature_num)) ||
+        (rc = dev_alloc(&part, 2 * B + 4)) || (rc = dev_alloc(&s->ah_obs, R * 256))) {
+        if (s->ah_dense) (void)hipFree(s->ah_dense);
+        if (cat) (void)hipFree(cat);
+        if (part) (void)hipFree(part);
+        s->ah_dense = nullptr;
+        return rc;
+    }
+    s->ah_cat = reinterpret_cast<int32_t*>(cat);
+    s->ah_rep = reinterpret_cast<int32_t*>(part);
+    s->ah_active = s->ah_rep + B;
+    s->ah_cnt = s->ah_active + B;
+    return RL4RS_OK;
+}
+
+int ahead_handout(rl4rs_stepper* s, int k, float* obs_dev, double* reward_dev, hipStream_t home) {
+    const int B = s->cfg.batch_size;
+    hipLaunchKernelGGL(k_ahead_handout, dim3((unsigned)(((int64_t)B * 64 + 255) / 256)), dim3(256), 0, home, s->ah_obs, s->ah_rep, s->ahead.n, k,
+                       obs_dev, reward_dev, B);
+    RL4RS_LAUNCH_CHECK();
+    return RL4RS_OK;
+}
+
+int ahead_start(rl4rs_stepper* s, const AheadState& was, int cur, RowRefineArgs* rf, const int32_t* actions_dev, float* obs_dev, double* reward_dev,
+                void* stream) {
+    hipStream_t home = (hipStream_t)stream;
+    const int B = s->cfg.batch_size, n = s->ahead.n;
+    const bool lanes = s->ahead.lanes;
+    const LaneState before = s->lstate;
+    hipStream_t st = home;
+    hipEvent_t before_augru = nullptr;
+    if (lanes) {
+        const LanePlan lp = lane_ahead_start(s->lstate);
+        StepLane& l = s->lane[0];
+        st = l.st;
+        hipError_t he = hipSuccess;
+        if (lp.wait_entry && (he = hipEventRecord(s->ev_entry, home)) == hipSuccess) he = hipStreamWaitEvent(st, s->ev_entry, 0);
+        if (he == hipSuccess && lp.wait_act) he = hipStreamWaitEvent(st, s->lane[1].act_done, 0);
+        if (he != hipSuccess) {
+            lane_undo(s->lstate, before);
+            s->ahead = was;
+            set_error("env_step_discrete: %s", hipGetErrorString(he));
+            return RL4RS_EHIP;
+        }
+        if (lp.wait_act) before_augru = s->lane[1].done;
+        if (!rf->active_src) { rf->active_src = s->part_active; rf->n_active_src = s->part_cnt; }
+        rf->active = s->part_active_alt;
+        rf->cnt = s->part_cnt_alt;
+        env_flip_rows(s->env);
+    } else {
+        const AheadState now = s->ahead;
+        const int rcj = lanes_wait(s, stream, 1);
+        s->ahead = now;
+        if (rcj) { s->ahead = was; return rcj; }
+    }
+    ActTail tail;
+    tail.done = nullptr; tail.done_v = 0;
+    tail.zero_reward = nullptr;
+    tail.next_action = s->next_off + (size_t)(cur + 1) * B;
+    tail.next_cur = cur + 1;
+    int rc = rl4rs::env_act_discrete_tail(s->env, actions_dev, tail, st, rf);
+    if (rc) {
+        if (lanes) { env_flip_rows(s->env); lane_undo(s->lstate, before); }
+        env_rows_current(s->env, &s->dense, &s->cat);
+        s->ahead = was;
+        return rc;
+    }
+    if (lanes) {
+        std::swap(s->part_active, s->part_active_alt);
+        std::swap(s->part_cnt, s->part_cnt_alt);
+    }
+    env_rows_current(s->env, &s->dense, &s->cat);
+    refined(s);
+    s->next_off_cur = cur + 1;
+    AheadPart part = {s->part_rep[s->part_cur], s->part_active, s->part_cnt, s->ah_rep, s->ah_active, s->ah_cnt};
+    rc = rl4rs::env_build_ahead_rows_lane(s->env, cur, n, s->ah_dense, s->ah_cat, &part, st);
+    if (lanes && hipEventRecord(s->lane[0].act_done, st) != hipSuccess && !rc) {
+        set_error("env_step_discrete: hipEventRecord failed");
+        rc = RL4RS_EHIP;
+    }
+    if (!rc) {
+        rl4rs::dien_set_group_rows(s->dien, s->ah_obs);
+        rc = rl4rs_dien_set_row_partition(s->dien, s->ah_rep, s->ah_active, s->ah_cnt, B);
+    }
+    if (!rc) rc = dien_forward_lane_full(s->dien, 0, B * n, n, s->ah_dense, s->ah_cat, s->slots, nullptr, nullptr, st, stream, nullptr, before_augru);
+    if (lanes) (void)hipEventRecord(s->lane[0].done, st);
+    if (!rc && lanes && hipStreamWaitEvent(home, s->lane[0].done, 0) != hipSuccess) {
+        set_error("env_step_discrete: hipStreamWaitEvent failed");
+        rc = RL4RS_EHIP;
+    }
+    if (rc) {
+        s->ahead.active = false;
+        s->ahead.handed -= 1;
+        s->ahead.started -= 1;
+        return rc;
+    }
+    return ahead_handout(s, 0, obs_dev, reward_dev, home);
+}
+
+int ahead_next(rl4rs_stepper* s, const AheadState& was, int cur, RowRefineArgs* rf, const int32_t* actions_dev, float* obs_dev, double* reward_dev,
+               void* stream) {
+    hipStream_t home = (hipStream_t)stream;
+    const int B = s->cfg.batch_size;
+    const bool lanes = s->ahead.lanes;
+    const LaneState before = s->lstate;
+    hipStream_t st = home;
+    if (lanes) {
+        (void)lane_ahead_next(s->lstate);
+        st = s->lane[1].st;
+        RL4RS_HIP_TRY(hipStreamWaitEvent(st, s->lane[0].act_done, 0));
+    }
+    ActTail tail;
+    tail.done = nullptr; tail.done_v = 0;
+    tail.zero_reward = nullptr;
+    tail.next_action = s->next_off + (size_t)(cur + 1) * B;
+    tail.next_cur = cur + 1;
+    const int rc = rl4rs::env_act_discrete_tail(s->env, actions_dev, tail, st, rf);
+    if (rc) {
+        if (lanes) lane_undo(s->lstate, before);
+        s->ahead = was;
+        return rc;
+    }
+    if (rf) refined(s);
+    s->next_off_cur = cur + 1;
+    if (lanes) {
+        RL4RS_HIP_TRY(hipEventRecord(s->lane[1].act_done, st));
+        RL4RS_HIP_TRY(hipEventRecord(s->lane[1].done, st));
+        RL4RS_HIP_TRY(hipStreamWaitEvent(home, s->lane[0].done, 0));
+        RL4RS_HIP_TRY(hipStreamWaitEvent(home, s->lane[1].done, 0));
+    }
+    return ahead_handout(s, cur - s->ahead.c0, obs_dev, reward_dev, home);
+}
+
 int reward_act(const rl4rs_stepper* s, int cur) {
     const int T = s->cfg.max_steps;
     if (!s->cfg.is_seq) return T - 1;
@@ -364,6 +520,7 @@
         s->overlap = s->reset_lane = s->reward_lane = s->lanes_made;
     }
     s->act_tail = true;
+    s->replay_ahead = dien != nullptr ? 1 : 0;
     s->obs_fold = true;
     s->distinct_hint = s->cfg.batch_size;
     void* p;
@@ -408,6 +565,10 @@
     }
     if (s->probs) (void)hipFree(s->probs);
     if (s->p_last) (void)hipFree(s->p_last);
+    if (s->ah_dense) (void)hipFree(s->ah_dense);
+    if (s->ah_cat) (void)hipFree(s->ah_cat);
+    if (s->ah_obs) (void)hipFree(s->ah_obs);
+    if (s->ah_rep) (void)hipFree(s->ah_rep);
     if (s->next_off) (void)hipFree(s->next_off);
     if (s->part_rep[0]) (void)hipFree(s->part_rep[0]);
     if (s->ev_ready) (void)hipEventDestroy(s->ev_ready);
@@ -440,6 +601,33 @@
         c.to_reward = (c.reward_due || !(s->reset_lane || s->reward_lane)) ? 0 : reward_act(s, cur) - cur;
         c.no_reward_lane = !s->reward_lane;
         c.reward_fold = c.reward_due && reward_dev && c.overlap && c.dien_x && refine && fold_obs(s);
+        {
+            AheadCall a;
+            memset(&a, 0, sizeof(a));
+            a.on = s->replay_ahead != 0 && s->act_tail;
+            a.own_row = own_row;
+            a.slate = !s->cfg.is_seq && !done_dev && !mask_bits_dev && (reinterpret_cast<uintptr_t>(obs_dev) & 15) == 0;
+            a.dien_x = s->dien != nullptr;
+            a.carried = refine;
+            a.cur = cur; a.T = T;
+            if (a.on && a.dien_x && (s->ahead.active || ahead_rows(cur, T) == 8 || ahead_rows(cur, T) == 9)) {
+                for (int i = 0; i < 2; ++i)
+                    a.rows64[i] = s->replay_ahead == 2 ? rl4rs::dien_augru_rows64(s->dien, s->cfg.batch_size, 8 + i)
+                                                       : rl4rs::dien_augru_rows64_auto(s->dien, s->cfg.batch_size, 8 + i);
+            }
+            a.lanes = lane_room(c);
+            if (!s->ahead.active && ahead_trigger(a) && ensure_ahead(s) != RL4RS_OK) {
+                (void)hipGetLastError();
+                s->replay_ahead = 0;
+                a.on = false;
+            }
+            const AheadState was = s->ahead;
+            bool dropped = false;
+            const AheadStep step = ahead_decide(s->ahead, a, &dropped);
+            if (dropped) { const int rcj = lanes_wait(s, stream, 1); if (rcj) return rcj; }
+            if (step == AheadStep::Start) return ahead_start(s, was, cur, &rf, actions_dev, obs_dev, reward_dev, stream);
+            if (step == AheadStep::Next) return ahead_next(s, was, cur, refine ? &rf : nullptr, actions_dev, obs_dev, reward_dev, stream);
+        }
         const LaneState before = s->lstate;
         const LanePlan lp = lane_decide(s->lstate, c);
         if (lp.lane) return lane_transition(s, lp, before, cur, &rf, actions_dev, obs_dev, reward_dev, stream);
@@ -503,6 +691,20 @@
 int rl4rs_stepper_set_reward_lane(rl4rs_stepper* s, int32_t on) {
     RL4RS_REQUIRE(s, "stepper_set_reward_lane: null argument");
     s->reward_lane = on != 0 && s->lanes_made;
+    return RL4RS_OK;
+}
+
+int rl4rs_stepper_set_replay_ahead(rl4rs_stepper* s, int32_t on) {
+    RL4RS_REQUIRE(s && on >= 0 && on <= 2, "stepper_set_replay_ahead: bad argument");
+    s->replay_ahead = s->dien != nullptr ? on : 0;
+    return RL4RS_OK;
+}
+
+int rl4rs_stepper_replay_stats(const rl4rs_stepper* s, int64_t* started, int64_t* handed, int64_t* dropped) {
+    RL4RS_REQUIRE(s, "stepper_replay_stats: null argument");
+    if (started) *started = s->ahead.started;
+    if (handed) *handed = s->ahead.handed;
+    if (dropped) *dropped = s->ahead.dropped;
     return RL4RS_OK;
 }
 
diff --git a/rl4rs_amd/csrc/step_lanes.hpp b/rl4rs_amd/csrc/step_lanes.hpp
--- a/rl4rs_amd/csrc/step_lanes.hpp
+++ b/rl4rs_amd/csrc/step_lanes.hpp
@@ -136,4 +136,79 @@
     return p;
 }
 
-}
+struct AheadCall {
+    bool on;
+    bool own_row;
+    bool slate;
+    bool dien_x;
+    bool carried;
+    bool rows64[2];
+    bool lanes;
+    int cur, T;
+};
+struct AheadState {
+    bool active;
+    bool lanes;
+    int c0, n;
+    int next;
+    int64_t started, handed, dropped;
+};
+enum class AheadStep { None, Start, Next };
+
+inline int ahead_rows(int cur, int T) { return T - 1 - cur; }
+inline bool ahead_trigger(const AheadCall& c) {
+    const int n = ahead_rows(c.cur, c.T);
+    return c.on && c.own_row && c.slate && c.dien_x && c.carried && (n == 8 || n == 9) && c.rows64[n - 8];
+}
+inline bool ahead_cancel(AheadState& s) {
+    if (!s.active) return false;
+    s.dropped += s.c0 + s.n - s.next;
+    s.active = false;
+    return true;
+}
+inline AheadStep ahead_decide(AheadState& s, const AheadCall& c, bool* dropped) {
+    *dropped = false;
+    if (s.active) {
+        if (c.on && c.own_row && c.slate && c.cur == s.next && c.cur < s.c0 + s.n) {
+            s.next += 1;
+            s.handed += 1;
+            if (s.next == s.c0 + s.n) s.active = false;
+            return AheadStep::Next;
+        }
+        *dropped = ahead_cancel(s);
+    }
+    if (!ahead_trigger(c)) return AheadStep::None;
+    s.active = true;
+    s.lanes = c.lanes;
+    s.c0 = c.cur;
+    s.n = ahead_rows(c.cur, c.T);
+    s.next = c.cur + 1;
+    s.started += 1;
+    s.handed += 1;
+    return AheadStep::Start;
+}
+inline LanePlan lane_ahead_start(LaneState& s) {
+    LanePlan p = {};
+    p.lane = true;
+    p.on = 0;
+    p.wait_entry = !s.in_flight;
+    p.wait_act = s.in_flight && s.last == 1;
+    s.in_flight = true;
+    s.used[0] = true;
+    s.last = 0;
+    s.next = 1;
+    return p;
+}
+inline LanePlan lane_ahead_next(LaneState& s) {
+    LanePlan p = {};
+    p.lane = true;
+    p.on = 1;
+    p.wait_act = true;
+    s.in_flight = true;
+    s.used[1] = true;
+    s.last = 1;
+    s.next = 0;
+    return p;
+}
+
+}
diff --git a/rl4rs_amd/device.py b/rl4rs_amd/device.py
--- a/rl4rs_amd/device.py
+++ b/rl4rs_amd/device.py
@@ -222,6 +222,20 @@
         else:
             check(self.lib.rl4rs_env_build_complete_rows(self.h, rows_per_env, _stream()))
 
+    def build_ahead_rows(self, n, partition=None):
+        dense = torch.empty((self.B * n, self.Dn), dtype=torch.float32, device=self.device)
+        cat = torch.empty((self.B * n, self.Cn), dtype=torch.int32, device=self.device)
+        if partition is None:
+            check(self.lib.rl4rs_env_build_ahead_rows(self.h, n, _ptr(dense), _ptr(cat), None, None, None, None, None, None, _stream()))
+            return dense, cat
+        rep, active, cnt = partition
+        assert all(t.dtype == torch.int32 and t.is_cuda and t.is_contiguous() for t in partition) and rep.numel() == self.B
+        out = (torch.empty(self.B, dtype=torch.int32, device=self.device), torch.full((self.B,), -1, dtype=torch.int32, device=self.device),
+               torch.zeros(1, dtype=torch.int32, device=self.device))
+        check(self.lib.rl4rs_env_build_ahead_rows(self.h, n, _ptr(dense), _ptr(cat), _ptr(rep), _ptr(active), _ptr(cnt), _ptr(out[0]),
+                                                  _ptr(out[1]), _ptr(out[2]), _stream()))
+        return dense, cat, out
+
     def reward(self, probs, p_last=None):
         out = torch.empty(self.B, dtype=torch.float64, device=self.device)
         m = self.n_complete - (1 if p_last is not None else 0)
@@ -299,7 +313,7 @@
 class DeviceStepper(object):
 
     def __init__(self, env, net, slots, act_tail=True, obs_fold=True, partition_carry=True, step_overlap=True, reset_lane=True,
-                 reward_lane=True):
+                 reward_lane=True, replay_ahead=True):
         self.lib = _lib.load()
         self.env, self.net, self.slots = env, net, slots
         assert slots.dtype == torch.int32 and slots.is_contiguous() and slots.shape[1] == env.B
@@ -320,6 +334,8 @@
             check(self.lib.rl4rs_stepper_set_reset_lane(self.h, 0))
         if not reward_lane:
             check(self.lib.rl4rs_stepper_set_reward_lane(self.h, 0))
+        if replay_ahead is not True:
+            check(self.lib.rl4rs_stepper_set_replay_ahead(self.h, 2 if replay_ahead == 'pinned' else 0))
         self.reset_lane = bool(step_overlap and reset_lane)
         self._distinct_hint = None
         self.B, self.A, self.E, self.W, self.device = env.B, env.A, env.E, env.W, env.device
@@ -351,6 +367,11 @@
         a, b = C.c_int64(0), C.c_int64(0)
         check(self.lib.rl4rs_stepper_lane_stats_ex(self.h, C.byref(a), C.byref(b)))
         return int(a.value), int(b.value)
+
+    def replay_stats(self):
+        a, b, d = C.c_int64(0), C.c_int64(0), C.c_int64(0)
+        check(self.lib.rl4rs_stepper_replay_stats(self.h, C.byref(a), C.byref(b), C.byref(d)))
+        return int(a.value), int(b.value), int(d.value)
 
     def observe(self):
         if not self.reset_lane or not self.act_tail:
diff --git a/rl4rs_amd/env/slate.py b/rl4rs_amd/env/slate.py
--- a/rl4rs_amd/env/slate.py
+++ b/rl4rs_amd/env/slate.py
@@ -562,7 +562,9 @@
             no_overlap = self.config.get('no_step_overlap', os.environ.get('RL4RS_NO_STEP_OVERLAP', '') not in ('', '0'))
             self._stepper = D.DeviceStepper(env, net, slots, act_tail=not no_tail, obs_fold=not no_fold, partition_carry=not no_carry,
                                             step_overlap=not no_overlap, reset_lane=self._lane_switch('reset_lane'),
-                                            reward_lane=self._lane_switch('reward_lane'))
+                                            reward_lane=self._lane_switch('reward_lane'),
+                                            replay_ahead=self._lane_switch('replay_ahead') and (
+                                                'pinned' if self.config.get('replay_ahead', os.environ.get('RL4RS_REPLAY_AHEAD', '')) == 'pinned' else True))
             self._stepper_key = key
         own = samples.is_seq and env.cur_steps >= samples.page_items
         self._stepper.set_distinct_hint(None if own else getattr(samples, '_n_lines', None))
```

After: 7.010 million, median of 6. 1.09x the previous value.
